# dohlee/diffab-pytorch

Hardware: AMD Instinct MI355X
Metric: CDR-residue denoise-steps/sec (K=128 patch) (higher is better)
Workload: dtype f32 (bf16x6 / fp16x3 split-precision products on the 16-bit matrix cores, fp32 accumulate; fp32-accurate, DESIGN section 4)

## Files before the change

### diffab-pytorch_amd/csrc/api.hip

```cpp
#include <atomic>
#include <cstring>
#include <mutex>
#include <vector>

#include "common.h"
#include "denoiser_internal.h"
#include "mlp_chain_tile.h"

namespace diffab {

static thread_local char g_err[512] = "";

void set_error(const char* fmt, ...) {
  va_list ap;
  va_start(ap, fmt);
  vsnprintf(g_err, sizeof(g_err), fmt, ap);
  va_end(ap);
}

namespace {
struct OrderState {
  std::recursive_mutex mu;
  hipStream_t last = nullptr;
  bool have = false;
// ... 21 lines not shown
}
StreamOrder::~StreamOrder() {
  if (dev_ < 0) return;
  OrderState& o = g_order[dev_ & 31];
  --o.depth;
  o.mu.unlock();
}
void set_stream_order(bool on) { g_order_on.store(on); }

struct KernelTimer {
  bool on = false;
  std::vector<hipEvent_t> ev;
  size_t used = 0;
};
static KernelTimer g_timer;

void timer_begin(hipStream_t st) {
  if (!g_timer.on) return;
  if (g_timer.used + 2 > g_timer.ev.size()) {
    for (int i = 0; i < 2; ++i) {
      hipEvent_t e;
      if (hipEventCreate(&e) != hipSuccess) return;
      g_timer.ev.push_back(e);
    }
  }
  (void)hipEventRecord(g_timer.ev[g_timer.used], st);
}
bool kernel_timer_enabled() { return g_timer.on; }
void timer_end(hipStream_t st) {
  if (!g_timer.on || g_timer.used + 2 > g_timer.ev.size()) return;
  (void)hipEventRecord(g_timer.ev[g_timer.used + 1], st);
  g_timer.used += 2;
}

static int check_dims(const diffab_dims* d, const char* who) {
  DIFFAB_REQUIRE(d != nullptr, DIFFAB_ERR_ARG, "%s: dims is null", who);
  DIFFAB_REQUIRE(d->B > 0 && d->K > 0 && d->D > 0 && d->C >= 0 && d->H > 0 && d->DS > 0 && d->PQ > 0 && d->PV > 0 && d->NL >= 0 && d->V > 0,
                 DIFFAB_ERR_ARG, "%s: non-positive dimension (B=%d K=%d D=%d C=%d H=%d DS=%d PQ=%d PV=%d NL=%d V=%d)", who, d->B, d->K, d->D,
                 d->C, d->H, d->DS, d->PQ, d->PV, d->NL, d->V);
  DIFFAB_REQUIRE(static_cast<int64_t>(d->B) * d->K < (1ll << 31), DIFFAB_ERR_UNSUPPORTED, "%s: B*K must be < 2^31", who);
  return DIFFAB_OK;
}

struct StepBuffers {
  float *cat2, *h1, *hA, *hB, *cat3, *t1, *t2, *vbuf, *logits, *ipa, *emb_tab, *beta_tab;
  char* planes;
  float* pair;
  size_t bytes;
};
static size_t mlp_planes_bytes() { return (rowgemm128_b6_scratch_bytes(128) + 255) & ~static_cast<size_t>(255); }

static StepBuffers carve_step(const diffab_dims* d, void* ws, int n_pair = 0) {
  Carver c(ws);
  const size_t rows = static_cast<size_t>(d->B) * d->K;
  StepBuffers b;
  b.cat2 = c.take<float>(rows * 2 * d->D);
  b.h1 = c.take<float>(rows * d->D);
  b.hA = c.take<float>(rows * d->D);
  b.hB = c.take<float>(rows * d->D);
  b.cat3 = c.take<float>(rows * (d->D + 3));
  b.t1 = c.take<float>(rows * d->D);
  b.t2 = c.take<float>(rows * d->D);
  b.vbuf = c.take<float>(rows * 3);
  b.logits = c.take<float>(rows * d->V);
  b.emb_tab = c.take<float>(static_cast<size_t>(25) * d->D);
  b.beta_tab = c.take<float>(static_cast<size_t>(3) * d->B * d->D);
  size_t ipa_floats = ipa_generic_workspace_floats(d);
  if (fast_path_supported(d)) ipa_floats = ipa_floats > ipa_fast_workspace_floats(d) ? ipa_floats : ipa_fast_workspace_floats(d);
  b.ipa = c.take<float>(ipa_floats);
  b.planes = fast_path_supported(d) ? c.take<char>(d->NL * ipa_layer_planes_bytes() + 11 * mlp_planes_bytes()) : nullptr;
  b.pair = pair_planes_supported(d) ? c.take<float>(pair_planes_floats(d, n_pair)) : nullptr;
  b.bytes = c.bytes();
  return b;
}

static bool ipa_layer_weights_ok(const diffab_dims* d, const diffab_ipa_layer_weights* w) {
  return w && w->gamma && w->wq_s && w->wk_s && w->wv_s && (w->w_bias || d->C == 0) && w->wq_p && w->wk_p && w->wv_p && w->w_out && w->b_out;
}

static int ipa_layer_dispatch(const diffab_dims* d, const diffab_ipa_layer_weights* w, const float* x, const float* e, const float* R,
                              const float* t, float* y, float* ws, uint32_t flags, hipStream_t st, float* sp_keep = nullptr,
                              float* d2_keep = nullptr, const void* planes = nullptr, const float* pair_planes = nullptr,
                              bool taped = false,
                              const unsigned char* tile_needed = nullptr, const int* ctx_of_row = nullptr, int n_ctx = 0) {
  DIFFAB_REQUIRE(ipa_layer_weights_ok(d, w), DIFFAB_ERR_ARG, "ipa layer: null weight pointer");
  if (!(flags & DIFFAB_FLAG_FORCE_GENERIC) && fast_path_supported(d))
    return ipa_layer_fast(d, w, x, e, R, t, y, ws, st, sp_keep, d2_keep, planes, pair_planes, (flags & DIFFAB_FLAG_FP32_GEMM) != 0,
                          taped, tile_needed, ctx_of_row, n_ctx);
  return ipa_layer_generic(d, w, x, e, R, t, y, ws, st, ctx_of_row);
}

static int check_denoiser_weights(const diffab_dims* d, const diffab_denoiser_weights* w) {
  DIFFAB_REQUIRE(w && w->seq_emb && w->res_w0 && w->res_b0 && w->res_w2 && w->res_b2 && (d->NL == 0 || w->layers), DIFFAB_ERR_ARG,
                 "denoiser: null weight pointer");
  DIFFAB_REQUIRE(d->C > 0, DIFFAB_ERR_ARG, "denoiser: C must be positive (the Denoiser's IPA layers use the pair bias, :478-492)");
  for (const diffab_mlp3_weights* h : {&w->coord, &w->orient, &w->seq})
    DIFFAB_REQUIRE(h->w0 && h->b0 && h->w2 && h->b2 && h->w4 && h->b4, DIFFAB_ERR_ARG, "denoiser head: null weight pointer");
  for (int l = 0; l < d->NL; ++l)
    DIFFAB_REQUIRE(ipa_layer_weights_ok(d, &w->layers[l]), DIFFAB_ERR_ARG, "denoiser: null weight pointer in IPA layer %d", l);
  return DIFFAB_OK;
}

static bool use_pair_planes(const diffab_dims* d, uint32_t flags, const float* pair_ctx, const StepBuffers& b) {
  const uint32_t other = DIFFAB_FLAG_FORCE_GENERIC | DIFFAB_FLAG_PAIR_F32;
  return (flags & DIFFAB_FLAG_PAIR_PLANES) && !(flags & other) && b.pair != nullptr && pair_planes_supported(d) &&
         (reinterpret_cast<uintptr_t>(pair_ctx) & 15) == 0;
}

static bool module_launch_fills_chip(const diffab_dims* d) {
  if (!ipa_module_persistent_supported(d)) return false;
  int dev = 0, ncu = 256;
  if (hipGetDevice(&dev) == hipSuccess) (void)hipDeviceGetAttribute(&ncu, hipDeviceAttributeMultiprocessorCount, dev);
  const int rounds = (d->B + ncu - 1) / ncu;
  return d->K == 128 && d->B >= ncu && static_cast<double>(d->B) >= 0.85 * rounds * ncu;
}

struct ForwardPlan {
  uint32_t flags;
  bool fold;
  bool b6;
  bool chain;
  bool persistent, fused_mlps;
  const float* pair_planes;
  const int* ctx_of_row;
  int n_ctx;
  const unsigned char* last_layer_tiles;
  float* res_emb;
};

static ForwardPlan plan_forward(const diffab_dims* d, uint32_t flags, const StepBuffers& b, const float* res_ctx, const float* pair_ctx,
                                float* res_emb, bool loop, const int* ctx_of_row = nullptr, int n_ctx = 0, unsigned char* tiles = nullptr) {
  const int rows = d->B * d->K, D = d->D;
  if (loop && !(flags & DIFFAB_FLAG_PAIR_F32)) flags |= DIFFAB_FLAG_PAIR_PLANES;
  ForwardPlan p{};
  p.flags = flags;
  p.fold = !(flags & DIFFAB_FLAG_FORCE_GENERIC) && fast_path_supported(d) && rowgemm128_ok(res_ctx, D, b.h1, D, rows, D);
  p.b6 = p.fold && use_b6_gemm(flags) && rowgemm128_b6_ok(res_ctx, D, b.h1, D, rows, D);
  p.chain = p.b6 && d->V <= 128;
  p.pair_planes = use_pair_planes(d, flags, pair_ctx, b) ? b.pair : nullptr;
  p.ctx_of_row = ctx_of_row;
  p.n_ctx = n_ctx;
  p.last_layer_tiles = tiles != nullptr && !(flags & DIFFAB_FLAG_ALL_ROWS) && p.fold && d->K % 16 == 0 && d->NL >= 2 ? tiles : nullptr;
  p.res_emb = res_emb;
  p.persistent = p.b6 && p.pair_planes != nullptr && ipa_module_persistent_supported(d) &&
                 ((flags & DIFFAB_FLAG_PERSISTENT_MODULE) || (loop && !(flags & DIFFAB_FLAG_MULTI_LAUNCH) && module_launch_fills_chip(d)));
  p.fused_mlps = p.persistent && p.chain && D == 128 && res_emb == nullptr;
  return p;
}

struct StepBias {
  const float* beta;
  const float* sched_beta;
  int t;
  const int* t_dev;
  float* beta_traj;
  int traj_rows;
};

static int prepare_forward(const diffab_dims* d, const diffab_denoiser_weights* w, const ForwardPlan& p, const StepBuffers& b,
                           const float* pair_ctx, const StepBias& bias, hipStream_t st) {
  if (p.fold)
    if (int rc = launch_fold_embed_table(d, w, b.emb_tab, st)) return rc;
  if (p.b6) {
    const int D = d->D;
    for (int l = 0; l < d->NL; ++l)
      if (int rc = ipa_layer_split_weights(&w->layers[l], b.planes + l * ipa_layer_planes_bytes(), st)) return rc;
    char* mlp = b.planes + d->NL * ipa_layer_planes_bytes();
    const diffab_mlp3_weights* hw[3] = {&w->coord, &w->orient, &w->seq};
    if (int rc = launch_wsplit128(w->res_w0, 2 * D, D, mlp, st)) return rc;
    if (int rc = launch_wsplit128(w->res_w2, D, D, mlp + mlp_planes_bytes(), st)) return rc;
    for (int hd = 0; hd < 3; ++hd) {
      if (int rc = launch_wsplit128(hw[hd]->w0, D + 3, D, mlp + (2 + 2 * hd) * mlp_planes_bytes(), st)) return rc;
      if (int rc = launch_wsplit128(hw[hd]->w2, D, D, mlp + (3 + 2 * hd) * mlp_planes_bytes(), st)) return rc;
      const int nout = hd == 2 ? d->V : 3;
      if (int rc = launch_wsplit128(hw[hd]->w4, D, D, mlp + (8 + hd) * mlp_planes_bytes(), st, nout)) return rc;
    }
  }
  if (p.pair_planes)
    if (int rc = launch_pair_split(d, pair_ctx, b.pair, st, p.n_ctx)) return rc;
  if (bias.beta_traj) {
    diffab_dims dt = *d;
    dt.B = bias.traj_rows;
    if (int rc = launch_fold_beta_table(&dt, w, bias.sched_beta, bias.beta_traj, st)) return rc;
  }
  return DIFFAB_OK;
}

static int denoise_step(const diffab_dims* d, const diffab_denoiser_weights* w, const ForwardPlan& p, const StepBias& bias,
                        const int64_t* seq_t, const float* x_t, const float* O_t, const float* res_ctx, const float* pair_ctx, float* out_eps,
                        float* out_O0, float* out_post, float* out_logits, const StepBuffers& b, hipStream_t st) {
  const int rows = d->B * d->K, D = d->D;
  if (p.fold && bias.beta_traj == nullptr)
    if (int rc = launch_fold_beta_table(d, w, bias.beta, b.beta_tab, st, bias.sched_beta, bias.t, bias.t_dev)) return rc;
  const char* mlp = p.b6 ? b.planes + d->NL * ipa_layer_planes_bytes() : nullptr;
  auto dense128 = [&](int slot, const float* X, const float* W, int ldw, const float* bvec, const int64_t* bias_idx, int bias_div, float* Y,
                      bool relu) -> int {
    if (p.b6) return launch_rowgemm128_b6p(X, D, mlp + slot * mlp_planes_bytes(), bvec, bias_idx, bias_div, Y, D, rows, D, relu, st);
    return launch_rowgemm128(X, D, W, ldw, bvec, bias_idx, bias_div, Y, D, rows, D, relu, st);
  };
  float* logits = out_logits ? out_logits : b.logits;
  MlpChainSet emb_set{}, head_set{};
  if (p.chain) {
    const void* pl[3] = {mlp, mlp + mlp_planes_bytes(), nullptr};
    const float* bs[3] = {b.emb_tab, w->res_b2, nullptr};
    float* ys[1] = {b.hA};
    const int nout1[1] = {D};
    if (int rc = make_mlp_chain_set(&emb_set, 1, pl, bs, seq_t, 0, 2, nout1, ys, nout1)) return rc;
    if (!p.fused_mlps)
      if (int rc = launch_mlp_chain_b6(res_ctx, D, pl, bs, seq_t, 0, 2, D, b.hA, D, rows, st)) return rc;
  } else if (p.fold) {
    if (int rc = dense128(0, res_ctx, w->res_w0, 2 * D, b.emb_tab, seq_t, 0, b.h1, true)) return rc;
    if (int rc = dense128(1, b.h1, w->res_w2, D, w->res_b2, nullptr, 0, b.hA, false)) return rc;
  } else {
    if (int rc = launch_embed_concat(res_ctx, w->seq_emb, seq_t, D, rows, b.cat2, st)) return rc;
    if (int rc = launch_linear(b.cat2, 2 * D, w->res_w0, w->res_b0, b.h1, D, rows, D, 2 * D, true, st)) return rc;
    if (int rc = launch_linear(b.h1, D, w->res_w2, w->res_b2, b.hA, D, rows, D, D, false, st)) return rc;
  }
  float *cur = b.hA, *nxt = b.hB;
  const diffab_mlp3_weights* hw[3] = {&w->coord, &w->orient, &w->seq};
  float* outs[3] = {out_eps, b.vbuf, logits};
  const int nout[3] = {3, 3, d->V};
  const void* hpl[9];
  const float* hbs[9];
  const int head_div = bias.beta_traj ? rows : d->K;
  if (p.chain) {
    for (int hd = 0; hd < 3; ++hd) {
      hpl[3 * hd] = mlp + (2 + 2 * hd) * mlp_planes_bytes();
      hpl[3 * hd + 1] = mlp + (3 + 2 * hd) * mlp_planes_bytes();
      hpl[3 * hd + 2] = mlp + (8 + hd) * mlp_planes_bytes();
      hbs[3 * hd] = bias.beta_traj ? bias.beta_traj + (static_cast<size_t>(hd) * bias.traj_rows + bias.t) * D
                                   : b.beta_tab + static_cast<size_t>(hd) * d->B * D;
      hbs[3 * hd + 1] = hw[hd]->b2;
      hbs[3 * hd + 2] = hw[hd]->b4;
    }
    if (int rc = make_mlp_chain_set(&head_set, 3, hpl, hbs, nullptr, head_div, 3, nout, outs, nout)) return rc;
  }
  if (p.persistent) {
    if (int rc = launch_ipa_module_persistent(d, b.hA, b.hB, O_t, x_t, b.ipa, b.planes, p.pair_planes, st, p.fused_mlps ? res_ctx : nullptr,
                                              &emb_set, &head_set, p.ctx_of_row, p.n_ctx, p.last_layer_tiles))
      return rc;
    cur = (d->NL & 1) ? b.hB : b.hA;
  }
  for (int l = 0; l < d->NL && !p.persistent; ++l) {
    const void* planes = p.b6 ? b.planes + l * ipa_layer_planes_bytes() : nullptr;
    if (int rc = ipa_layer_dispatch(d, &w->layers[l], cur, pair_ctx, O_t, x_t, nxt, b.ipa, p.flags, st, nullptr, nullptr, planes, p.pair_planes,
                                    false, l == d->NL - 1 ? p.last_layer_tiles : nullptr, p.ctx_of_row, p.n_ctx))
      return rc;
    float* tmp = cur; cur = nxt; nxt = tmp;
  }
  if (p.res_emb) DIFFAB_HIP_CHECK(hipMemcpyAsync(p.res_emb, cur, sizeof(float) * rows * D, hipMemcpyDeviceToDevice, st));
  if (p.chain) {
    if (!p.fused_mlps)
      if (int rc = launch_mlp_chains_b6(cur, D, 3, hpl, hbs, nullptr, head_div, 3, nout, outs, nout, rows, st)) return rc;
  } else if (p.fold) {
    for (int hd = 0; hd < 3; ++hd) {
      if (int rc = dense128(2 + 2 * hd, cur, hw[hd]->w0, D + 3, b.beta_tab + static_cast<size_t>(hd) * d->B * D, nullptr, d->K, b.t1, true))
        return rc;
      if (int rc = dense128(3 + 2 * hd, b.t1, hw[hd]->w2, D, hw[hd]->b2, nullptr, 0, b.t2, true)) return rc;
      if (int rc = launch_linear(b.t2, D, hw[hd]->w4, hw[hd]->b4, outs[hd], nout[hd], rows, nout[hd], D, false, st)) return rc;
    }
  } else {
    if (int rc = launch_beta_concat(cur, bias.beta, D, d->K, rows, b.cat3, st)) return rc;
    for (int hd = 0; hd < 3; ++hd) {
      if (int rc = launch_linear(b.cat3, D + 3, hw[hd]->w0, hw[hd]->b0, b.t1, D, rows, D, D + 3, true, st)) return rc;
      if (int rc = launch_linear(b.t1, D, hw[hd]->w2, hw[hd]->b2, b.t2, D, rows, D, D, true, st)) return rc;
      if (int rc = launch_linear(b.t2, D, hw[hd]->w4, hw[hd]->b4, outs[hd], nout[hd], rows, nout[hd], D, false, st)) return rc;
    }
  }
  if (out_O0 == nullptr) return DIFFAB_OK;
  return launch_heads_finish(b.vbuf, O_t, logits, d->V, rows, out_O0, out_post, st);
}

static uint32_t taped_flags(uint32_t flags) { return flags & ~(DIFFAB_FLAG_FORCE_GENERIC | DIFFAB_FLAG_PAIR_PLANES); }

static int denoise_step_taped(const diffab_dims* d, const diffab_denoiser_weights* w, const int64_t* seq_t, const float* x_t,
                              const float* O_t, const float* res_ctx, const float* pair_ctx, const float* beta, float* out_eps,
                              float* out_O0, float* out_post, const TrainTape& tp, uint32_t flags, hipStream_t st) {
  const int rows = d->B * d->K, D = d->D;
  if (int rc = launch_embed_concat(res_ctx, w->seq_emb, seq_t, D, rows, tp.cat2, st)) return rc;
  if (int rc = launch_linear(tp.cat2, 2 * D, w->res_w0, w->res_b0, tp.h1, D, rows, D, 2 * D, true, st)) return rc;
  if (int rc = launch_linear(tp.h1, D, w->res_w2, w->res_b2, tp.x[0], D, rows, D, D, false, st)) return rc;
  const bool b6 = tp.planes && use_b6_gemm(flags) && fast_path_supported(d);
  for (int l = 0; l < d->NL; ++l) {
    if (b6)
      if (int rc = ipa_layer_split_weights(&w->layers[l], tp.planes, st)) return rc;
    if (int rc = ipa_layer_dispatch(d, &w->layers[l], tp.x[l], pair_ctx, O_t, x_t, tp.x[l + 1], tp.ipa_ws[l], flags, st, tp.sp[l], tp.d2[l],
                                    b6 ? tp.planes : nullptr, nullptr, true))
      return rc;
  }
  if (int rc = launch_beta_concat(tp.x[d->NL], beta, D, d->K, rows, tp.cat3, st)) return rc;
  const diffab_mlp3_weights* hw[3] = {&w->coord, &w->orient, &w->seq};
  float* outs[3] = {out_eps, tp.vbuf, tp.logits};
  const int nout[3] = {3, 3, d->V};
  for (int hd = 0; hd < 3; ++hd) {
    if (int rc = launch_linear(tp.cat3, D + 3, hw[hd]->w0, hw[hd]->b0, tp.t1[hd], D, rows, D, D + 3, true, st)) return rc;
    if (int rc = launch_linear(tp.t1[hd], D, hw[hd]->w2, hw[hd]->b2, tp.t2[hd], D, rows, D, D, true, st)) return rc;
    if (int rc = launch_linear(tp.t2[hd], D, hw[hd]->w4, hw[hd]->b4, outs[hd], nout[hd], rows, nout[hd], D, false, st)) return rc;
  }
  return launch_heads_finish(tp.vbuf, O_t, tp.logits, d->V, rows, out_O0, out_post, st);
}

constexpr int kTrajRows = 1025;
struct SampleBuffers {
  float *beta, *eps, *O0, *post;
  int* t_dev;
  unsigned char* tiles;
  float* beta_traj;
  int* ctx_of_row;
  float* res_ctx;
  void* step;
  size_t bytes;
};

static SampleBuffers carve_sample(const diffab_dims* d, void* ws, int n_pair = 0, bool mapped = false) {
  Carver c(ws);
  const size_t rows = static_cast<size_t>(d->B) * d->K;
  SampleBuffers s;
  s.beta = c.take<float>(d->B);
  s.eps = c.take<float>(rows * 3);
  s.O0 = c.take<float>(rows * 9);
  s.post = c.take<float>(rows * d->V);
  s.t_dev = c.take<int>(64);
  s.tiles = c.take<unsigned char>(static_cast<size_t>(d->B) * ((d->K + 15) / 16));
  s.beta_traj = c.take<float>(static_cast<size_t>(3) * kTrajRows * d->D);
  s.ctx_of_row = mapped ? c.take<int>(d->B) : nullptr;
  s.res_ctx = mapped ? c.take<float>(rows * d->D) : nullptr;
  const size_t step_bytes = carve_step(d, nullptr, n_pair).bytes;
  s.step = c.take<char>(step_bytes);
  s.bytes = c.bytes();
  return s;
}

struct ScoreBuffers {
  int* t_list;
  float* beta;
  int* ctx_of_row;
  int64_t* seq_t;
  float *x_t, *O_t, *eps, *eps_hat;
  float* res_ctx;
  void* step;
  size_t bytes;
};
static ScoreBuffers carve_score(const diffab_dims* d, void* ws, int n_ctx) {
  Carver c(ws);
  const size_t rows = static_cast<size_t>(d->B) * d->K;
  ScoreBuffers s;
  s.t_list = c.take<int>(kTrajRows);
  s.beta = c.take<float>(d->B);
  s.ctx_of_row = c.take<int>(d->B);
  s.seq_t = c.take<int64_t>(rows);
  s.x_t = c.take<float>(rows * 3);
  s.O_t = c.take<float>(rows * 9);
  s.eps = c.take<float>(rows * 3);
  s.eps_hat = c.take<float>(rows * 3);
  s.res_ctx = c.take<float>(rows * d->D);
  s.step = c.take<char>(carve_step(d, nullptr, n_ctx).bytes);
  s.bytes = c.bytes();
  return s;
}

}

using namespace diffab;

extern "C" {

const char* diffab_version(void) { return "diffab_hip 0.1.0 (gfx950)"; }
const char* diffab_last_error(void) { return g_err; }

int diffab_device_ok(void) {
  int n = 0;
  if (hipGetDeviceCount(&n) != hipSuccess || n <= 0) return 0;
  hipDeviceProp_t p;
  int dev = 0;
  if (hipGetDevice(&dev) != hipSuccess || hipGetDeviceProperties(&p, dev) != hipSuccess) return 0;
  return std::strncmp(p.gcnArchName, "gfx950", 6) == 0 ? 1 : 0;
}

int diffab_debug_linear128(const float* X, const float* W, const float* bias, float* Y, int64_t M, int32_t Kd, int32_t mode, void* scratch,
                           size_t scratch_bytes, void* stream) {
  StreamOrder order_(stream);
  DIFFAB_REQUIRE(X && W && Y && M >= 1 && M < (1LL << 31) && Kd >= 32 && Kd % 32 == 0, DIFFAB_ERR_ARG, "debug_linear128: bad operands");
  hipStream_t st = as_stream(stream);
  if (mode == 0) return launch_linear(X, Kd, W, bias, Y, 128, static_cast<int>(M), 128, Kd, false, st);
  if (mode == 2) {
    const size_t pb = (rowgemm128_h3_planes_bytes(Kd) + 255) & ~static_cast<size_t>(255);
    DIFFAB_REQUIRE(Kd % 64 == 0, DIFFAB_ERR_ARG, "debug_linear128: mode 2 (fp16 x 3) needs Kd %% 64 == 0 (its chunks of 32 k are joined in pairs)");
    DIFFAB_REQUIRE(scratch && scratch_bytes >= pb + 512 && rowgemm128_b6_ok(X, Kd, Y, 128, static_cast<int>(M), Kd) &&
                       (reinterpret_cast<uintptr_t>(scratch) & 15) == 0,
                   DIFFAB_ERR_ARG, "debug_linear128: mode 2 needs 16-byte aligned operands and %zu bytes of scratch", pb + 512);
    float* wis = reinterpret_cast<float*>(static_cast<char*>(scratch) + pb);
    if (int rc = launch_wsplit128_h3(W, Kd, Kd, scratch, wis, st)) return rc;
    return launch_rowgemm128_h3p(X, Kd, scratch, wis, bias, nullptr, 0, Y, 128, static_cast<int>(M), Kd, false, st, nullptr);
  }
  DIFFAB_REQUIRE(mode == 1 && scratch && scratch_bytes >= rowgemm128_b6_scratch_bytes(Kd) && rowgemm128_b6_ok(X, Kd, Y, 128, static_cast<int>(M), Kd),
                 DIFFAB_ERR_ARG, "debug_linear128: mode 1 needs 16-byte aligned operands and %zu bytes of scratch", rowgemm128_b6_scratch_bytes(Kd));
  return launch_rowgemm128_b6(X, Kd, W, Kd, bias, nullptr, 0, Y, 128, static_cast<int>(M), Kd, false, scratch, st);
}

int diffab_debug_xstat128(const float* X, const float* W, float* Y, int64_t M, int32_t N, int32_t mode, void* scratch, size_t scratch_bytes,
                          void* stream) {
  StreamOrder order_(stream);
  DIFFAB_REQUIRE(X && W && Y && scratch && M >= 1 && M < (1LL << 31) && N >= 1 && (mode == 1 || mode == 2), DIFFAB_ERR_ARG,
                 "debug_xstat128: bad operands");
  const size_t need = mode == 1 ? xstat_b6_scratch_bytes(N) : xstat_h3_scratch_bytes(N);
  DIFFAB_REQUIRE(scratch_bytes >= need && (reinterpret_cast<uintptr_t>(scratch) & 15) == 0 && (reinterpret_cast<uintptr_t>(X) & 15) == 0,
                 DIFFAB_ERR_ARG, "debug_xstat128: needs 16-byte aligned X / scratch and %zu bytes of scratch", need);
  hipStream_t st = as_stream(stream);
  if (mode == 1) return launch_xstat_b6(X, W, 1, N, Y, N, static_cast<int>(M), N, scratch, st);
  return launch_xstat_h3(X, W, 1, N, Y, N, static_cast<int>(M), N, scratch, st);
}

int diffab_debug_gemm_tn(const float* A, const float* B, float* C, float* db, int64_t M, int32_t N1, int32_t N2, int32_t mode, void* stream) {
  StreamOrder order_(stream);
  DIFFAB_REQUIRE(A && B && C && M >= 1 && M < (1LL << 31) && N1 >= 1 && N2 >= 1 && (mode == 1 || mode == 2), DIFFAB_ERR_ARG,
                 "debug_gemm_tn: bad operands");
  hipStream_t st = as_stream(stream);
  if (mode == 1) return launch_gemm_tn_b6(A, N1, B, N2, C, N2, static_cast<int>(M), N1, N2, db, nullptr, nullptr, 0, st);
  return launch_gemm_tn_h3(A, N1, B, N2, C, N2, static_cast<int>(M), N1, N2, db, nullptr, nullptr, 0, st);
}

int diffab_set_stream_guard(int on) {
  set_stream_order(on != 0);
  return DIFFAB_OK;
}

int diffab_debug_set_module_stagger(int32_t ticks_10ns, int32_t classes) {
  set_module_stagger(ticks_10ns, classes);
  return DIFFAB_OK;
}

int diffab_debug_set_module_stamps(void* device_buffer) {
  set_module_stamps(device_buffer);
  return DIFFAB_OK;
}

int diffab_debug_row_tiles(const uint8_t* gen_mask, int32_t B, int32_t K, uint8_t* tiles, void* stream) {
  StreamOrder order_(stream);
  DIFFAB_REQUIRE(gen_mask && tiles && B >= 1 && K >= 16 && K % 16 == 0, DIFFAB_ERR_ARG, "debug_row_tiles: need B >= 1 and K a multiple of 16");
  return launch_tiles_needed(gen_mask, B, K, tiles, as_stream(stream));
}

int diffab_debug_set_attn_variant(int32_t v) { return set_attn_variant(v); }

int diffab_debug_set_attn_stamps(void* device_buffer) {
  set_attn_stamps(device_buffer);
  return DIFFAB_OK;
}

int diffab_kernel_timer_enable(int on) {
  g_timer.on = on != 0;
  g_timer.used = 0;
  return DIFFAB_OK;
}

int diffab_kernel_timer_read(int64_t* launches, double* total_ms) {
  DIFFAB_REQUIRE(launches && total_ms, DIFFAB_ERR_ARG, "kernel_timer_read: null pointer");
  double tot = 0.0;
  for (size_t i = 0; i + 1 < g_timer.used; i += 2) {
    DIFFAB_HIP_CHECK(hipEventSynchronize(g_timer.ev[i + 1]));
    float ms = 0.f;
    DIFFAB_HIP_CHECK(hipEventElapsedTime(&ms, g_timer.ev[i], g_timer.ev[i + 1]));
    tot += ms;
  }
  *launches = static_cast<int64_t>(g_timer.used / 2);
  *total_ms = tot;
  g_timer.used = 0;
  return DIFFAB_OK;
}

size_t diffab_denoise_workspace_bytes(const diffab_dims* d) {
  if (check_dims(d, "denoise_workspace_bytes")) return 0;
  return carve_step(d, nullptr).bytes;
}

size_t diffab_sample_workspace_bytes(const diffab_dims* d) {
  if (check_dims(d, "sample_workspace_bytes")) return 0;
  return carve_sample(d, nullptr).bytes;
}

size_t diffab_sample_shared_workspace_bytes(const diffab_dims* d, int32_t n_ctx) {
  if (check_dims(d, "sample_shared_workspace_bytes")) return 0;
  if (n_ctx < 1 || static_cast<int64_t>(n_ctx) * d->K >= (1ll << 31)) {
    set_error("sample_shared_workspace_bytes: need 1 <= n_ctx and n_ctx*K < 2^31 (n_ctx=%d)", n_ctx);
    return 0;
  }
  return carve_sample(d, nullptr, n_ctx, true).bytes;
}

int diffab_ipa_layer_fwd(const diffab_dims* d, const diffab_ipa_layer_weights* w, const float* x, const float* e, const float* R,
                         const float* t, float* y, void* workspace, size_t workspace_bytes, uint32_t flags, void* stream) {
  StreamOrder order_(stream);
  if (int rc = check_dims(d, "ipa_layer_fwd")) return rc;
  DIFFAB_REQUIRE(x && (e || d->C == 0) && R && t && y && workspace, DIFFAB_ERR_ARG, "ipa_layer_fwd: null pointer");
  const StepBuffers b = carve_step(d, workspace);
  DIFFAB_REQUIRE(workspace_bytes >= b.bytes, DIFFAB_ERR_WORKSPACE, "ipa_layer_fwd: workspace %zu < %zu bytes", workspace_bytes, b.bytes);
  const float* pair_planes = nullptr;
  if (use_pair_planes(d, flags, e, b)) {
    if (int rc = launch_pair_split(d, e, b.pair, as_stream(stream))) return rc;
    pair_planes = b.pair;
  }
  return ipa_layer_dispatch(d, w, x, e, R, t, y, b.ipa, flags, as_stream(stream), nullptr, nullptr, nullptr, pair_planes);
}

int diffab_denoise_step_fwd(const diffab_dims* d, const diffab_denoiser_weights* w, const int64_t* seq_t, const float* x_t, const float* O_t,
                            const float* res_ctx, const float* pair_ctx, const float* beta, float* out_eps, float* out_O0,
                            float* out_posterior, float* out_logits, float* out_res_emb, void* workspace, size_t workspace_bytes,
                            uint32_t flags, void* stream) {
  StreamOrder order_(stream);
  if (int rc = check_dims(d, "denoise_step_fwd")) return rc;
  if (int rc = check_denoiser_weights(d, w)) return rc;
  DIFFAB_REQUIRE(seq_t && x_t && O_t && res_ctx && pair_ctx && beta && out_eps && out_O0 && out_posterior && workspace, DIFFAB_ERR_ARG,
                 "denoise_step_fwd: null pointer");
  const StepBuffers b = carve_step(d, workspace);
  DIFFAB_REQUIRE(workspace_bytes >= b.bytes, DIFFAB_ERR_WORKSPACE, "denoise_step_fwd: workspace %zu < %zu bytes", workspace_bytes, b.bytes);
  hipStream_t st = as_stream(stream);
  const ForwardPlan p = plan_forward(d, flags, b, res_ctx, pair_ctx, out_res_emb, false);
  const StepBias bias{beta};
  if (int rc = prepare_forward(d, w, p, b, pair_ctx, bias, st)) return rc;
  return denoise_step(d, w, p, bias, seq_t, x_t, O_t, res_ctx, pair_ctx, out_eps, out_O0, out_posterior, out_logits, b, st);
}

static int check_attn_bwd_lds(const diffab_dims* d, const char* who) {
  DIFFAB_REQUIRE(attn_bwd_lds_ok(d), DIFFAB_ERR_UNSUPPORTED,
                 "%s: H*K = %d too large for the attention backward's LDS (%zu > %zu bytes; the forward alone reaches further)", who,
                 d->H * d->K, attn_bwd_lds_bytes(d), kAttnBwdLdsMax);
// ... 248 lines not shown
  std::vector<int32_t> plan_host;
  if (steps != nullptr) {
    const int T = s->T;
    DIFFAB_REQUIRE(steps->n_steps >= 1, DIFFAB_ERR_ARG, "sample_loop: steps n_steps = %d < 1", steps->n_steps);
    DIFFAB_REQUIRE(steps->steps && steps->beta_jump && steps->alpha_jump && steps->plan_dev, DIFFAB_ERR_ARG,
                   "sample_loop: steps needs steps, beta_jump, alpha_jump and plan_dev");
    DIFFAB_REQUIRE(s->alpha_bar, DIFFAB_ERR_ARG, "sample_loop: steps need the schedule's alpha_bar");
    DIFFAB_REQUIRE(steps->steps[0] == t_start, DIFFAB_ERR_ARG, "sample_loop: steps[0] = %d, t_start = %d", steps->steps[0], t_start);
    std::vector<char> listed(T + 1, 0);
    for (int j = 0; j < steps->n_steps; ++j) {
      const int t = steps->steps[j];
      DIFFAB_REQUIRE(t > t_stop && t <= T, DIFFAB_ERR_ARG, "sample_loop: steps[%d] = %d outside [t_stop + 1, T] = [%d, %d]", j, t, t_stop + 1, T);
      DIFFAB_REQUIRE(j == 0 || t < steps->steps[j - 1], DIFFAB_ERR_ARG, "sample_loop: steps are not strictly descending at %d (%d after %d)", j,
                     t, steps->steps[j - 1]);
      const float bj = steps->beta_jump[t], aj = steps->alpha_jump[t];
      DIFFAB_REQUIRE(bj > 0.0f && bj < 1.0f && aj > 0.0f && aj < 1.0f, DIFFAB_ERR_ARG,
                     "sample_loop: jump coefficients at step %d outside (0, 1): beta' = %g, alpha' = %g", t, bj, aj);
      listed[t] = 1;
    }
    if (rec != nullptr)
      for (int t = 0; t <= T; ++t)
        DIFFAB_REQUIRE(rec->slot_of_step[t] == -1 || listed[t], DIFFAB_ERR_ARG,
                       "sample_loop: record slot_of_step[%d] = %d, but the step list does not run step %d", t, rec->slot_of_step[t], t);
    plan_host.resize(3 * static_cast<size_t>(T + 1));
    for (int t = 0; t <= T; ++t) plan_host[t] = t > 0 ? t - 1 : 0;
    for (int j = 0; j < steps->n_steps; ++j) plan_host[steps->steps[j]] = j + 1 < steps->n_steps ? steps->steps[j + 1] : t_stop;
    std::memcpy(plan_host.data() + (T + 1), steps->beta_jump, sizeof(float) * (T + 1));
    std::memcpy(plan_host.data() + 2 * (T + 1), steps->alpha_jump, sizeof(float) * (T + 1));
    const int32_t* pd = static_cast<const int32_t*>(steps->plan_dev);
    pdev = StepPlanDev{pd, reinterpret_cast<const float*>(pd + (T + 1)), reinterpret_cast<const float*>(pd + 2 * (T + 1)), s->alpha_bar};
  }
  GuidanceDev gdev;
  if (guidance != nullptr) {
    if (int rc = check_guidance_terms(guidance, "sample_loop")) return rc;
    DIFFAB_REQUIRE(guidance->max_shift > 0.0f, DIFFAB_ERR_ARG, "sample_loop: guidance max_shift = %g must be > 0 (INFINITY: no cap)",
                   guidance->max_shift);
    DIFFAB_REQUIRE(guidance->t_max >= 0 && guidance->t_max <= s->T, DIFFAB_ERR_ARG, "sample_loop: guidance t_max = %d outside [0, T = %d]",
                   guidance->t_max, s->T);
    DIFFAB_REQUIRE(guidance->shift_dev != nullptr, DIFFAB_ERR_ARG, "sample_loop: guidance needs shift_dev");
    DIFFAB_REQUIRE(!(keep & DIFFAB_FLAG_KEEP_STRUCTURE), DIFFAB_ERR_ARG,
                   "sample_loop: guidance moves the structure, which DIFFAB_FLAG_KEEP_STRUCTURE does not sample");
    DIFFAB_REQUIRE(s->alpha_bar_sqrt, DIFFAB_ERR_ARG, "sample_loop: guidance needs the schedule's alpha_bar_sqrt");
    gdev.shift = guidance->shift_dev;
    gdev.chain = guidance->chain;
    gdev.residue_idx = guidance->residue_idx;
    gdev.residue_mask = guidance->residue_mask;
    gdev.w_clash = guidance->w_clash;
    gdev.clash_distance = guidance->clash_distance;
    gdev.w_bond = guidance->w_bond;
    gdev.bond_length = guidance->bond_length;
    gdev.max_shift = guidance->max_shift;
    gdev.t_max = guidance->t_max;
  }
  TemperatureDev tdev;
  if (temperature != nullptr) {
    DIFFAB_REQUIRE(!temperature->rot_scale || temperature->rot_row, DIFFAB_ERR_ARG,
                   "sample_loop: temperature rot_scale needs rot_row (its rows of the stacked reverse table)");
    DIFFAB_REQUIRE(!((temperature->trans_scale || temperature->rot_scale) && (keep & DIFFAB_FLAG_KEEP_STRUCTURE)), DIFFAB_ERR_ARG,
                   "sample_loop: noise scales act on the structure, which DIFFAB_FLAG_KEEP_STRUCTURE does not sample");
    DIFFAB_REQUIRE(!(temperature->seq_temp && (keep & DIFFAB_FLAG_KEEP_SEQUENCE)), DIFFAB_ERR_ARG,
                   "sample_loop: a sequence temperature acts on the sequence, which DIFFAB_FLAG_KEEP_SEQUENCE does not sample");
    tdev = TemperatureDev{temperature->trans_scale, temperature->rot_scale, temperature->seq_temp, temperature->rot_row};
  }
  const bool mapped = ctx_of_row != nullptr;
  DIFFAB_REQUIRE(mapped || n_ctx == d->B, DIFFAB_ERR_ARG, "sample_loop: without ctx_of_row n_ctx must equal B (%d != %d)", n_ctx, d->B);
  DIFFAB_REQUIRE(n_ctx >= 1 && static_cast<int64_t>(n_ctx) * d->K < (1ll << 31), DIFFAB_ERR_ARG, "sample_loop: need 1 <= n_ctx, n_ctx*K < 2^31");
  bool identity = n_ctx == d->B;
  for (int b = 0; mapped && b < d->B; ++b) {
    DIFFAB_REQUIRE(ctx_of_row[b] >= 0 && ctx_of_row[b] < n_ctx, DIFFAB_ERR_ARG, "sample_loop: ctx_of_row[%d] = %d outside [0, %d)", b,
                   ctx_of_row[b], n_ctx);
    identity = identity && ctx_of_row[b] == b;
  }
  const SampleBuffers sb = carve_sample(d, workspace, n_ctx, mapped);
  DIFFAB_REQUIRE(workspace_bytes >= sb.bytes, DIFFAB_ERR_WORKSPACE, "sample_loop: workspace %zu < %zu bytes", workspace_bytes, sb.bytes);
  hipStream_t st = as_stream(stream);
  const int* ctx_dev = nullptr;
  if (!identity) {
    DIFFAB_HIP_CHECK(hipMemcpyAsync(sb.ctx_of_row, ctx_of_row, sizeof(int32_t) * d->B, hipMemcpyHostToDevice, st));
    if (int rc = launch_gather_rows(res_ctx, sb.ctx_of_row, d->B, static_cast<int64_t>(d->K) * d->D, sb.res_ctx, st)) return rc;
    ctx_dev = sb.ctx_of_row;
    res_ctx = sb.res_ctx;
  }
  const StepBuffers b0 = carve_step(d, sb.step, n_ctx);
  const ForwardPlan plan = plan_forward(d, flags, b0, res_ctx, pair_ctx, nullptr, true, ctx_dev, n_ctx, sb.tiles);
  StepBias bias{sb.beta, plan.fold ? s->beta : nullptr, 0, nullptr, nullptr, s->T + 1};
  if (plan.chain && s->T + 1 <= kTrajRows && !(flags & DIFFAB_FLAG_GRAPH_SAMPLER)) bias.beta_traj = sb.beta_traj;
  if (int rc = prepare_forward(d, w, plan, b0, pair_ctx, bias, st)) return rc;
  if (plan.last_layer_tiles)
    if (int rc = launch_tiles_needed(gen_mask, d->B, d->K, sb.tiles, st)) return rc;
  if (rec != nullptr) {
    DIFFAB_HIP_CHECK(hipMemcpyAsync(rec->slot_dev, rec->slot_of_step, sizeof(int32_t) * (s->T + 1), hipMemcpyHostToDevice, st));
    if (int rc = launch_record_fixed(rdev, seq, x, O, gen_mask, d->B, d->K, d->V, st)) return rc;
  }
  if (steps != nullptr)
    DIFFAB_HIP_CHECK(hipMemcpyAsync(steps->plan_dev, plan_host.data(), sizeof(int32_t) * plan_host.size(), hipMemcpyHostToDevice, st));
  auto one_step = [&](int t, const int* t_dev) -> int {
    if (!plan.fold)
      if (int rc = launch_fill_beta(s, t, d->B, sb.beta, st, t_dev)) return rc;
    StepBias step = bias;
    step.t = t;
    step.t_dev = t_dev;
    if (int rc = denoise_step(d, w, plan, step, seq, x, O, res_ctx, pair_ctx, sb.eps, nullptr, nullptr, nullptr, b0, st)) return rc;
    return launch_reverse_update_philox(s, rev_tab, t, seq, x, O, sb.eps, sb.O0, sb.post, gen_mask, seed, first_patch, d->B, d->K, d->V, st,
                                        t_dev, b0.vbuf, b0.logits, keep, allowed, rdev, pdev, gdev, tdev);
  };
  const int n_steps = steps != nullptr ? steps->n_steps : t_start - t_stop;
  const bool graph = (flags & DIFFAB_FLAG_GRAPH_SAMPLER) && n_steps >= 3 && !kernel_timer_enabled();
  if (!graph) {
    if (steps != nullptr) {
      for (int j = 0; j < n_steps; ++j)
        if (int rc = one_step(steps->steps[j], nullptr)) return rc;
      return DIFFAB_OK;
    }
    for (int t = t_start; t > t_stop; --t)
      if (int rc = one_step(t, nullptr)) return rc;
    return DIFFAB_OK;
  }
  const int t_second = steps != nullptr ? steps->steps[1] : t_start - 1;
  if (int rc = one_step(t_start, nullptr)) return rc;
  if (int rc = launch_set_int(sb.t_dev, t_second, st)) return rc;
  hipStream_t side = nullptr;
  hipEvent_t ev = nullptr;
  hipGraph_t g = nullptr;
  hipGraphExec_t ge = nullptr;
  DIFFAB_HIP_CHECK(hipStreamCreateWithFlags(&side, hipStreamNonBlocking));
  hipError_t ei = hipEventCreateWithFlags(&ev, hipEventDisableTiming);
  if (ei == hipSuccess) ei = hipEventRecord(ev, st);
  if (ei == hipSuccess) ei = hipStreamWaitEvent(side, ev, 0);
  int rc = DIFFAB_OK;
  if (ei == hipSuccess) {
    hipStream_t caller = st;
    st = side;
    ei = hipStreamBeginCapture(side, hipStreamCaptureModeThreadLocal);
    if (ei == hipSuccess) {
      rc = one_step(t_second, sb.t_dev);
      if (rc == DIFFAB_OK) rc = steps != nullptr ? launch_advance_step(sb.t_dev, pdev.next, side) : launch_dec_int(sb.t_dev, side);
      ei = hipStreamEndCapture(side, &g);
    }
    st = caller;
  }
  if (ei == hipSuccess && rc == DIFFAB_OK) ei = hipGraphInstantiate(&ge, g, nullptr, nullptr, 0);
  if (ei == hipSuccess && rc == DIFFAB_OK)
    for (int j = 1; j < n_steps && ei == hipSuccess; ++j) ei = hipGraphLaunch(ge, side);
  if (ei == hipSuccess) ei = hipStreamSynchronize(side);
  if (ge) (void)hipGraphExecDestroy(ge);
  if (g) (void)hipGraphDestroy(g);
  if (ev) (void)hipEventDestroy(ev);
  (void)hipStreamDestroy(side);
  if (rc != DIFFAB_OK) return rc;
  if (ei != hipSuccess) {
    set_error("sample_loop: graph capture / replay failed: %s", hipGetErrorString(ei));
    return DIFFAB_ERR_HIP;
  }
  return DIFFAB_OK;
}

size_t diffab_score_workspace_bytes(const diffab_dims* d, int32_t n_ctx) {
  if (check_dims(d, "score_workspace_bytes")) return 0;
  if (n_ctx < 1 || static_cast<int64_t>(n_ctx) * d->K >= (1ll << 31)) {
    set_error("score_workspace_bytes: need 1 <= n_ctx and n_ctx*K < 2^31 (n_ctx=%d)", n_ctx);
    return 0;
  }
  return carve_score(d, nullptr, n_ctx).bytes;
}

int diffab_score_designs(const diffab_dims* d, const diffab_denoiser_weights* w, const diffab_sched* s, const diffab_igso3* fwd_tab,
                         const int64_t* seq, const float* x, const float* O, const uint8_t* gen_mask, const uint8_t* res_mask,
// ... 61 lines not shown
```

### diffab-pytorch_amd/csrc/denoiser_fast.hip

```cpp
#include <cstdlib>
#include <type_traits>

#include "common.h"
#include "denoiser_internal.h"
#include "rowgemm_b6_tile.h"
#include "ipa_attn_tile.h"

namespace diffab {


constexpr int LBM = 128, LBK = 32, LLD = LBK + 4;

struct LinearSegs {
  const float* W[6];
  int n_end[6];
  int nseg;
};

template <int BN, bool RELU, bool VEC>
__global__ __launch_bounds__(256) void linear_mfma_kernel(const float* __restrict__ X, int ldx, LinearSegs segs,
                                                          const float* __restrict__ bias, float* __restrict__ Y, int ldy, int M, int N,
                                                          int Kd) {
  __shared__ __attribute__((aligned(16))) float As[LBM * LLD];
  __shared__ __attribute__((aligned(16))) float Bs[BN * LLD];
// ... 189 lines not shown
#pragma unroll
      for (int s = 0; s < 4; ++s)
#pragma unroll
        for (int mt = 0; mt < MT; ++mt)
#pragma unroll
          for (int tt = 0; tt < 4; ++tt)
            acc[mt][tt] = __builtin_amdgcn_mfma_f32_16x16x4f32(a[mt][4 * part + kq][s], b[kq & 1][tt][s], acc[mt][tt], 0, 0, 0);
    }
  };

  load_w(0);
  load_a(aA, 0);
  store_w(0);
  __syncthreads();
  for (int ch = 0; ch < nchunk; ch += 2 * AW) {
    load_a(aB, ch / AW + 1);
#pragma unroll
    for (int p = 0; p < AW; ++p) {
      load_w(ch + p + 1);
      MEM_FENCE();
      compute(aA, p, p & 1);
      store_w((p + 1) & 1);
      __syncthreads();
    }
    load_a(aA, ch / AW + 2);
#pragma unroll
    for (int p = 0; p < AW; ++p) {
      load_w(ch + AW + p + 1);
      MEM_FENCE();
      compute(aB, p, (AW + p) & 1);
      store_w((AW + p + 1) & 1);
      __syncthreads();
    }
  }
  const int col = 64 * cw + 4 * l15;
  const bool table = bias_idx != nullptr || bias_div > 0;
  f32x4 bv = {0.f, 0.f, 0.f, 0.f};
  if (bias && !table) bv = *reinterpret_cast<const f32x4*>(bias + col);
#pragma unroll
  for (int mt = 0; mt < MT; ++mt)
#pragma unroll
    for (int r = 0; r < 4; ++r) {
      const int row = m0 + 16 * MT * rw + 16 * mt + 4 * g + r;
      if (row >= M) continue;
      if (table) {
        const int64_t bi = bias_idx ? bias_idx[row] : row / bias_div;
        bv = *reinterpret_cast<const f32x4*>(bias + bi * 128 + col);
      }
      f32x4 o = {acc[mt][0][r] + bv[0], acc[mt][1][r] + bv[1], acc[mt][2][r] + bv[2], acc[mt][3][r] + bv[3]};
      if (RELU) { o[0] = fmaxf(o[0], 0.f); o[1] = fmaxf(o[1], 0.f); o[2] = fmaxf(o[2], 0.f); o[3] = fmaxf(o[3], 0.f); }
      *reinterpret_cast<f32x4*>(Y + static_cast<int64_t>(row) * ldy + col) = o;
    }
}

bool rowgemm128_ok(const float* X, int ldx, const float* Y, int ldy, int M, int Kd) {
  return Kd % (2 * RG_KC) == 0 && ldx % 4 == 0 && ldy % 4 == 0 && aligned16(X) && aligned16(Y) && M >= RG_ROWS;
}
int launch_rowgemm128(const float* X, int ldx, const float* W, int ldw, const float* bias, const int64_t* bias_idx, int bias_div, float* Y,
                      int ldy, int M, int Kd, bool relu, hipStream_t st) {
  DIFFAB_REQUIRE(rowgemm128_ok(X, ldx, Y, ldy, M, Kd) && (!bias || aligned16(bias)), DIFFAB_ERR_ARG, "rowgemm128: unsupported operands");
  const dim3 grid((M + RG_ROWS - 1) / RG_ROWS);
#define RG_LAUNCH(R, AW_) \
  hipLaunchKernelGGL((rowgemm128_kernel<R, AW_>), grid, dim3(512), 0, st, X, ldx, W, ldw, bias, bias_idx, bias_div, Y, ldy, M, Kd)
  if (RG_DEEP_A && Kd % (4 * RG_KC) == 0) { if (relu) RG_LAUNCH(true, 2); else RG_LAUNCH(false, 2); }
  else                                    { if (relu) RG_LAUNCH(true, 1); else RG_LAUNCH(false, 1); }
#undef RG_LAUNCH
  DIFFAB_LAUNCH_CHECK();
  return DIFFAB_OK;
}

int launch_linear(const float* X, int ldx, const float* W, const float* bias, float* Y, int ldy, int M, int N, int Kd, bool relu,
                  hipStream_t st) {
  LinearSegs segs{};
  segs.W[0] = W;
  segs.n_end[0] = N;
  segs.nseg = 1;
  const bool vec = (ldx % 4 == 0) && (Kd % 4 == 0) && aligned16(X) && aligned16(W);
  if (N == 128 && vec && rowgemm128_ok(X, ldx, Y, ldy, M, Kd) && (!bias || aligned16(bias)))
    return launch_rowgemm128(X, ldx, W, Kd, bias, nullptr, 0, Y, ldy, M, Kd, relu, st);
  if (N > 64) return launch_linear_bn<128>(X, ldx, segs, bias, Y, ldy, M, N, Kd, relu, vec, st);
  return launch_linear_bn<64>(X, ldx, segs, bias, Y, ldy, M, N, Kd, relu, vec, st);
}

template <int NT, bool MULTI, bool PLANES = false, bool TAPE = false>
__global__ __launch_bounds__(512) void ipa_attn_fast_kernel(const float* __restrict__ proj, const float* __restrict__ e,
                                                            const float* __restrict__ R, const float* __restrict__ t,
                                                            const float* __restrict__ Wb, const float* __restrict__ gamma,
                                                            float* __restrict__ feat, int B, int NC_arg,
                                                            unsigned long long* __restrict__ stamps, const float* __restrict__ esc = nullptr,
                                                            float* __restrict__ tape_p = nullptr, float* __restrict__ tape_d2 = nullptr,
                                                            const unsigned char* __restrict__ tile_needed = nullptr,
                                                            const int* __restrict__ ctx_of_row = nullptr) {
  extern __shared__ __attribute__((aligned(16))) float S[];
  const int ntile = (MULTI ? NC_arg : 1) * NT;
  int b, tile;
  const unsigned bid = blockIdx.x;
  if ((B & 7) == 0) {
    const int xcd = bid & 7, slot = bid >> 3;
    b = (slot / ntile) * 8 + xcd;
    tile = slot % ntile;
  } else {
    b = bid / ntile;
    tile = bid % ntile;
  }
  if (tile_needed != nullptr && !tile_needed[b * ntile + tile]) return;
  ipa_attn_tile<NT, MULTI, PLANES, TAPE>(S, b, tile, bid, proj, e, R, t, Wb, gamma, feat, NC_arg, stamps, esc, tape_p, tape_d2, ctx_of_row);
}

static unsigned long long* g_attn_stamps = nullptr;
static bool g_pair_chain_off = false;
void set_pair_embed_fused(bool on);
int set_attn_variant(int v) {
  DIFFAB_REQUIRE((v & ~(4 | 64)) == 0, DIFFAB_ERR_ARG, "debug_set_attn_variant: %d has bits other than 4 and 64", v);
  set_pair_embed_fused(!(v & 4));
  g_pair_chain_off = (v & 64) != 0;
  return DIFFAB_OK;
}
bool pair_chain_bwd_enabled() { return !g_pair_chain_off; }
void set_attn_stamps(void* p) {
  g_attn_stamps = static_cast<unsigned long long*>(p);
}

__global__ void points_to_global_fast_kernel(float* __restrict__ proj, const float* __restrict__ R, const float* __restrict__ t, int rows) {
  const int gid = blockIdx.x * blockDim.x + threadIdx.x;
  if (gid >= rows * 192) return;
  const int r = gid / 192, p = gid % 192;
  float* qv = proj + static_cast<int64_t>(r) * ANP + OFF_GQ + p * 3;
  const float* Rr = R + static_cast<int64_t>(r) * 9;
  const float x = qv[0], y = qv[1], z = qv[2];
  qv[0] = (x * Rr[0] + y * Rr[3] + z * Rr[6]) + t[r * 3 + 0];
  qv[1] = (x * Rr[1] + y * Rr[4] + z * Rr[7]) + t[r * 3 + 1];
  qv[2] = (x * Rr[2] + y * Rr[5] + z * Rr[8]) + t[r * 3 + 2];
}

__global__ __launch_bounds__(64) void fold_embed_table_kernel(const float* __restrict__ emb, const float* __restrict__ W0,
                                                              const float* __restrict__ b0, int D, int n_types, float* __restrict__ tab) {
  const int s_ = blockIdx.x, n0 = blockIdx.y * 8, lane = threadIdx.x;
  if (s_ >= n_types) return;
  float acc[8];
#pragma unroll
  for (int i = 0; i < 8; ++i) {
    acc[i] = 0.f;
    const int n = n0 + i;
    if (n < D)
      for (int k = lane; k < D; k += 64) acc[i] += emb[s_ * D + k] * W0[n * 2 * D + D + k];
  }
#pragma unroll
  for (int i = 0; i < 8; ++i) {
    for (int o = 32; o > 0; o >>= 1) acc[i] += __shfl_xor(acc[i], o);
    if (lane == 0 && n0 + i < D) tab[s_ * D + n0 + i] = acc[i] + b0[n0 + i];
  }
}
__global__ void fold_beta_table_kernel(const float* __restrict__ beta, const float* __restrict__ Wa, const float* __restrict__ ba,
                                       const float* __restrict__ Wb_, const float* __restrict__ bb, const float* __restrict__ Wc,
                                       const float* __restrict__ bc, int D, int B, float* __restrict__ tab,
                                       const float* __restrict__ sched_beta, int t, const int* __restrict__ t_dev) {
  const int b = blockIdx.x, hd = blockIdx.y, n = threadIdx.x;
  if (b >= B || n >= D) return;
  const float* W = hd == 0 ? Wa : (hd == 1 ? Wb_ : Wc);
  const float* bias = hd == 0 ? ba : (hd == 1 ? bb : bc);
  const float be = sched_beta ? sched_beta[t_dev ? *t_dev : t] : beta[b];
  const float* wr = W + n * (D + 3) + D;
  tab[(static_cast<int64_t>(hd) * B + b) * D + n] = ((be * wr[0] + sinf(be) * wr[1]) + cosf(be) * wr[2]) + bias[n];
}
int launch_fold_embed_table(const diffab_dims* d, const diffab_denoiser_weights* w, float* emb_tab, hipStream_t st) {
  hipLaunchKernelGGL(fold_embed_table_kernel, dim3(25, (d->D + 7) / 8), dim3(64), 0, st, w->seq_emb, w->res_w0, w->res_b0, d->D, 25, emb_tab);
  DIFFAB_LAUNCH_CHECK();
  return DIFFAB_OK;
}
int launch_fold_beta_table(const diffab_dims* d, const diffab_denoiser_weights* w, const float* beta, float* beta_tab, hipStream_t st,
                           const float* sched_beta, int t, const int* t_dev) {
  hipLaunchKernelGGL(fold_beta_table_kernel, dim3(d->B, 3), dim3(d->D), 0, st, beta, w->coord.w0, w->coord.b0, w->orient.w0, w->orient.b0,
                     w->seq.w0, w->seq.b0, d->D, d->B, beta_tab, sched_beta, t, t_dev);
  DIFFAB_LAUNCH_CHECK();
  return DIFFAB_OK;
}

bool fast_path_supported(const diffab_dims* d) {
  return d->D == 128 && d->C == AC && d->H == AH && d->DS == ADS && d->PQ == AP && d->PV == AP && d->K % 64 == 0 && d->K >= 64 &&
         d->K <= 1024;
}

__global__ __launch_bounds__(256) void pair_rowscale_kernel(const float* __restrict__ e, int row_f4, float* __restrict__ rs) {
  const int64_t row = blockIdx.x;
  const f32x4* p = reinterpret_cast<const f32x4*>(e) + row * row_f4;
  float m = 0.f;
  for (int i = threadIdx.x; i < row_f4; i += 256) {
    const f32x4 v = p[i];
    m = fmaxf(fmaxf(m, fmaxf(fabsf(v[0]), fabsf(v[1]))), fmaxf(fabsf(v[2]), fabsf(v[3])));
  }
#pragma unroll
  for (int o = 1; o < 64; o <<= 1) m = fmaxf(m, __shfl_xor(m, o));
  __shared__ float wm[4];
  if ((threadIdx.x & 63) == 0) wm[threadIdx.x >> 6] = m;
  __syncthreads();
  if (threadIdx.x == 0) {
    const unsigned b = __float_as_uint(fmaxf(fmaxf(wm[0], wm[1]), fmaxf(wm[2], wm[3])));
    const int ex = static_cast<int>((b >> 23) & 255u);
    const bool ok = ex >= 8 && ex < 231 && b < 0x7f800000u;
    rs[2 * row] = ok ? __uint_as_float(static_cast<unsigned>(127 + 7 + 127 - ex) << 23) : 1.0f;
    rs[2 * row + 1] = ok ? __uint_as_float(static_cast<unsigned>(ex - 7) << 23) : 1.0f;
  }
}
__global__ void pair_split_kernel(const float* __restrict__ e, const float* __restrict__ rs, int K, int64_t n_groups,
                                  _Float16* __restrict__ out) {
  const int64_t gid = blockIdx.x * static_cast<int64_t>(blockDim.x) + threadIdx.x;
  if (gid >= n_groups) return;
  const int cg = static_cast<int>(gid & 7);
  const int64_t rj = gid >> 3;
  const int j = static_cast<int>(rj % K);
  const int64_t row = rj / K;
  const float s = rs[2 * row];
  const f32x4 v0 = reinterpret_cast<const f32x4*>(e)[gid * 2], v1 = reinterpret_cast<const f32x4*>(e)[gid * 2 + 1];
  f16x8 h1, h2;
#pragma unroll
  for (int c = 0; c < 8; ++c) {
    const float x = (c < 4 ? v0[c & 3] : v1[c & 3]) * s;
    const _Float16 a = static_cast<_Float16>(x);
    h1[c] = a;
    h2[c] = static_cast<_Float16>(x - static_cast<float>(a));
  }
  const int jt = j >> 4, l15 = j & 15, ks = cg >> 2, g = cg & 3;
  _Float16* base = out + (row * K) * 128 + static_cast<int64_t>(jt) * 2048 + ks * 512 + (l15 + 16 * g) * 8;
  *reinterpret_cast<f16x8*>(base) = h1;
  *reinterpret_cast<f16x8*>(base + 1024) = h2;
}
bool pair_planes_supported(const diffab_dims* d) { return fast_path_supported(d); }
static size_t pair_patches(const diffab_dims* d, int n_pair) { return static_cast<size_t>(n_pair > 0 ? n_pair : d->B); }
size_t pair_planes_floats(const diffab_dims* d, int n_pair) {
  const size_t np = pair_patches(d, n_pair);
  return pair_planes_supported(d) ? np * d->K * d->K * AC + 64 + 2 * np * d->K + 64 : 0;
}
const float* pair_row_scales(const diffab_dims* d, const float* planes, int n_pair) {
  return planes + 64 + pair_patches(d, n_pair) * d->K * d->K * AC;
}
int launch_pair_split(const diffab_dims* d, const float* e, float* planes, hipStream_t st, int n_pair) {
  DIFFAB_REQUIRE(pair_planes_supported(d) && e && planes && (reinterpret_cast<uintptr_t>(planes) & 15) == 0 &&
                     (reinterpret_cast<uintptr_t>(e) & 15) == 0,
                 DIFFAB_ERR_ARG, "pair_split: unsupported operands");
  const int64_t np = static_cast<int64_t>(pair_patches(d, n_pair));
  const int64_t n = np * d->K * d->K * AC;
  float* rs = const_cast<float*>(pair_row_scales(d, planes, n_pair));
  hipLaunchKernelGGL(pair_rowscale_kernel, dim3(static_cast<unsigned>(np * d->K)), dim3(256), 0, st, e, d->K * AC / 4, rs);
  hipLaunchKernelGGL(pair_split_kernel, dim3(static_cast<unsigned>((n / 8 + 255) / 256)), dim3(256), 0, st, e, rs, d->K, n / 8,
                     reinterpret_cast<_Float16*>(planes + 64));
  DIFFAB_LAUNCH_CHECK();
  return DIFFAB_OK;
}


bool use_b6_gemm(uint32_t flags) { return !(flags & DIFFAB_FLAG_FP32_GEMM); }
static size_t round256(size_t b) { return (b + 255) & ~static_cast<size_t>(255); }
constexpr size_t kLayerSmallFloats = AH * AC + 64 + 128;
size_t ipa_layer_small_offset() { return 0; }
size_t ipa_layer_h3_pj_offset() { return ipa_layer_small_offset() + round256(kLayerSmallFloats * sizeof(float)); }
size_t ipa_layer_h3_out_offset() { return ipa_layer_h3_pj_offset() + round256(proj_frames_h3_planes_bytes()); }
size_t ipa_layer_h3_wis_offset() { return ipa_layer_h3_out_offset() + round256(rowgemm128_h3_planes_bytes(AF)); }
size_t ipa_layer_planes_bytes() { return ipa_layer_h3_wis_offset() + round256((ANP + 128) * sizeof(float)); }
__global__ void layer_small_copy_kernel(const float* __restrict__ w_bias, const float* __restrict__ gamma, const float* __restrict__ b_out,
                                        float* __restrict__ out) {
  const int i = blockIdx.x * blockDim.x + threadIdx.x;
  if (i < AH * AC) out[i] = w_bias[i];
  else if (i < AH * AC + 64) out[i] = i - AH * AC < AH ? gamma[i - AH * AC] : 0.0f;
  else if (i < static_cast<int>(kLayerSmallFloats)) out[i] = b_out[i - AH * AC - 64];
}
int ipa_layer_split_weights(const diffab_ipa_layer_weights* w, void* planes, hipStream_t st) {
  DIFFAB_REQUIRE(w && w->wq_s && w->wk_s && w->wv_s && w->wq_p && w->wk_p && w->wv_p && w->w_out, DIFFAB_ERR_ARG, "ipa layer: null weight pointer");
  const float* W6[6] = {w->wq_s, w->wk_s, w->wv_s, w->wq_p, w->wk_p, w->wv_p};
  if (w->w_bias && w->gamma && w->b_out) {
    hipLaunchKernelGGL(layer_small_copy_kernel, dim3((kLayerSmallFloats + 255) / 256), dim3(256), 0, st, w->w_bias, w->gamma, w->b_out,
                       reinterpret_cast<float*>(static_cast<char*>(planes) + ipa_layer_small_offset()));
    DIFFAB_LAUNCH_CHECK();
  }
  char* pl = static_cast<char*>(planes);
  float* wis = reinterpret_cast<float*>(pl + ipa_layer_h3_wis_offset());
  if (int rc = launch_pjsplit_h3(W6, pl + ipa_layer_h3_pj_offset(), wis, st)) return rc;
  return launch_wsplit128_h3(w->w_out, AF, AF, pl + ipa_layer_h3_out_offset(), wis + ANP, st);
}
static size_t b6_scratch_floats() { return (ipa_layer_planes_bytes() + 256) / sizeof(float); }

static size_t ipa_ws_parts_offset(const diffab_dims* d) {
  const size_t rows = static_cast<size_t>(d->B) * d->K;
  const size_t o = rows * (ANP + AF) + 128 + (attention_split_supported(d) ? attention_split_workspace_floats(d) : 0) + b6_scratch_floats();
  return (o + 63) & ~static_cast<size_t>(63);
}
size_t ipa_fast_workspace_floats(const diffab_dims* d) { return ipa_ws_parts_offset(d) + rowgemm128_h3_parts_floats(d->B * d->K, AF) + 64; }

int ipa_layer_fast(const diffab_dims* d, const diffab_ipa_layer_weights* w, const float* x, const float* e, const float* R, const float* t,
                   float* y, float* ws, hipStream_t st, float* sp_keep, float* d2_keep, const void* planes, const float* pair_planes,
                   bool fp32_gemm, bool taped, const unsigned char* tile_needed, const int* ctx_of_row, int n_ctx) {
  const int rows = d->B * d->K, D = d->D;
  DIFFAB_REQUIRE(ctx_of_row == nullptr || sp_keep == nullptr, DIFFAB_ERR_ARG, "ipa_layer_fast: shared contexts are an inference form");
  float* proj = ws;
  float* feat = ws + static_cast<size_t>(rows) * ANP;
  const bool h3 = use_b6_gemm(fp32_gemm ? DIFFAB_FLAG_FP32_GEMM : 0u) && (planes != nullptr || sp_keep == nullptr);
  if (h3 && planes == nullptr) {
    float* tail = ws + static_cast<size_t>(rows) * (ANP + AF) + 128 + (attention_split_supported(d) ? attention_split_workspace_floats(d) : 0);
    void* own = reinterpret_cast<void*>((reinterpret_cast<uintptr_t>(tail) + 255) & ~static_cast<uintptr_t>(255));
    if (int rc = ipa_layer_split_weights(w, own, st)) return rc;
    planes = own;
  }
  const char* plc = static_cast<const char*>(planes);
  const float* wis = h3 ? reinterpret_cast<const float*>(plc + ipa_layer_h3_wis_offset()) : nullptr;
  auto to_out = [&]() -> int {
    if (h3 && rowgemm128_b6_ok(feat, AF, y, D, rows, AF))
      return launch_rowgemm128_h3p(feat, AF, plc + ipa_layer_h3_out_offset(), wis + ANP, w->b_out, nullptr, 0, y, D, rows, AF, false, st,
                                   taped ? nullptr : ws + ipa_ws_parts_offset(d));
    return launch_linear(feat, AF, w->w_out, w->b_out, y, D, rows, D, AF, false, st);
  };
  LinearSegs segs{};
  segs.W[0] = w->wq_s; segs.W[1] = w->wk_s; segs.W[2] = w->wv_s; segs.W[3] = w->wq_p; segs.W[4] = w->wk_p; segs.W[5] = w->wv_p;
  segs.n_end[0] = 256; segs.n_end[1] = 512; segs.n_end[2] = 768; segs.n_end[3] = 960; segs.n_end[4] = 1152; segs.n_end[5] = 1344;
  segs.nseg = 6;
  bool vec = aligned16(x);
  for (int s = 0; s < 6; ++s) vec = vec && aligned16(segs.W[s]);
  DIFFAB_REQUIRE(vec, DIFFAB_ERR_ARG, "ipa_layer_fast: x and the projection weights must be 16-byte aligned");
  if (h3) {
    if (int rc = launch_proj_frames_h3p(x, plc + ipa_layer_h3_pj_offset(), wis, R, t, proj, rows, st)) return rc;
  } else {
    if (int rc = launch_proj_frames_f32(x, segs.W, R, t, proj, rows, st)) return rc;
  }
  if (sp_keep != nullptr && attention_split_supported(d) && !(d->K == 128 && d2_keep != nullptr)) {
    if (int rc = launch_attention_split(d, proj, e, R, t, w->w_bias, w->gamma, feat, sp_keep, st, d2_keep)) return rc;
    return to_out();
  }
  const bool tape = sp_keep != nullptr && attention_split_supported(d);
  const int nt = (d->K % 128 == 0) ? 8 : 4;
  const int nc = d->K / (16 * nt);
  const size_t lds = ipa_attn_lds_bytes(nt);
  const dim3 grid(d->B * (d->K / TI));
  const bool use_planes = pair_planes != nullptr && pair_planes_supported(d);
  const float* e_arg = use_planes ? pair_planes + 64 : e;
  const float* esc = use_planes ? pair_row_scales(d, pair_planes, n_ctx) : nullptr;
#define ATTN_LAUNCH(NT_, MULTI_, PLANES_)                                                                                             \
  do {                                                                                                                                \
    DIFFAB_HIP_CHECK(hipFuncSetAttribute(reinterpret_cast<const void*>(ipa_attn_fast_kernel<NT_, MULTI_, PLANES_>),                   \
                                         hipFuncAttributeMaxDynamicSharedMemorySize, static_cast<int>(lds)));                         \
    timer_begin(st);                                                                                                                  \
    hipLaunchKernelGGL((ipa_attn_fast_kernel<NT_, MULTI_, PLANES_>), grid, dim3(512), lds, st, proj, e_arg, R, t, w->w_bias, w->gamma, \
                       feat, d->B, nc, g_attn_stamps, esc, nullptr, nullptr, tile_needed, ctx_of_row);                                \
    timer_end(st);                                                                                                                    \
  } while (0)
  if (tape) {
    DIFFAB_HIP_CHECK(hipFuncSetAttribute(reinterpret_cast<const void*>(ipa_attn_fast_kernel<8, false, false, true>),
                                         hipFuncAttributeMaxDynamicSharedMemorySize, static_cast<int>(lds)));
    hipLaunchKernelGGL((ipa_attn_fast_kernel<8, false, false, true>), grid, dim3(512), lds, st, proj, e, R, t, w->w_bias, w->gamma, feat,
                       d->B, nc, nullptr, nullptr, sp_keep, d2_keep);
  } else if (use_planes) {
    if (nt == 8 && nc == 1) ATTN_LAUNCH(8, false, true);
    else if (nt == 8) ATTN_LAUNCH(8, true, true);
    else if (nc == 1) ATTN_LAUNCH(4, false, true);
    else ATTN_LAUNCH(4, true, true);
  } else if (nt == 8 && nc == 1) ATTN_LAUNCH(8, false, false);
  else if (nt == 8) ATTN_LAUNCH(8, true, false);
  else if (nc == 1) ATTN_LAUNCH(4, false, false);
  else ATTN_LAUNCH(4, true, false);
#undef ATTN_LAUNCH
  DIFFAB_LAUNCH_CHECK();
  return to_out();
}

}
```

### diffab-pytorch_amd/csrc/denoiser_internal.h

```cpp
#pragma once
#include "common.h"

namespace diffab {

int launch_linear_generic(const float* X, int ldx, const float* W, const float* bias, float* Y, int ldy, int M, int N, int Kd, bool relu,
                          hipStream_t st);
size_t ipa_generic_workspace_floats(const diffab_dims* d);
int ipa_layer_generic(const diffab_dims* d, const diffab_ipa_layer_weights* w, const float* x, const float* e, const float* R, const float* t,
                      float* y, float* ws, hipStream_t st, const int* ctx_of_row = nullptr);
int launch_embed_concat(const float* res_ctx, const float* emb, const int64_t* seq, int D, int64_t rows, float* out, hipStream_t st);
int launch_beta_concat(const float* h, const float* beta, int D, int K, int64_t rows, float* out, hipStream_t st);
int launch_heads_finish(const float* v, const float* O_t, const float* logits, int V, int64_t rows, float* O0, float* post, hipStream_t st);
int launch_proj_frames_f32(const float* x, const float* const* W6, const float* R, const float* t, float* proj, int rows, hipStream_t st);
int launch_losses_bwd(const float* post, const float* tpost, const float* eps, const float* teps, const float* O0, const float* tO,
                      const float* O_t, const float* v, const uint8_t* gm, const uint8_t* rm, const float* count, const float* up, int V,
                      int64_t rows, float* d_logits, float* d_eps, float* d_v, hipStream_t st);
int launch_heads_cotangent(const float* post, const float* c_post, const float* c_eps, const float* c_O0, const float* O_t, const float* v,
                           int V, int64_t rows, float* d_logits, float* d_eps, float* d_v, float* d_Ot, hipStream_t st);
int launch_ipa_frames_bwd(const float* proj, const float* dproj, int NP, int pt_col0, int n_pts, const float* feat, const float* dfeat, int F,
                          int ol_col0, int on_col0, int n_vpts, const float* R, const float* t, float* dR, float* dt, int rows,
                          hipStream_t st);

bool fast_path_supported(const diffab_dims* d);
size_t ipa_fast_workspace_floats(const diffab_dims* d);
int ipa_layer_fast(const diffab_dims* d, const diffab_ipa_layer_weights* w, const float* x, const float* e, const float* R, const float* t,
                   float* y, float* ws, hipStream_t st,
                   float* sp_keep = nullptr, float* d2_keep = nullptr,
                   const void* planes = nullptr,
                   const float* pair_planes = nullptr,
                   bool fp32_gemm = false,
                   bool taped = false,
                   const unsigned char* tile_needed = nullptr,
                   const int* ctx_of_row = nullptr, int n_ctx = 0);
bool pair_planes_supported(const diffab_dims* d);
size_t pair_planes_floats(const diffab_dims* d, int n_pair = 0);
int launch_pair_split(const diffab_dims* d, const float* e, float* planes, hipStream_t st, int n_pair = 0);
const float* pair_row_scales(const diffab_dims* d, const float* planes, int n_pair = 0);
int launch_linear(const float* X, int ldx, const float* W, const float* bias, float* Y, int ldy, int M, int N, int Kd, bool relu,
                  hipStream_t st);

bool rowgemm128_ok(const float* X, int ldx, const float* Y, int ldy, int M, int Kd);
int launch_rowgemm128(const float* X, int ldx, const float* W, int ldw, const float* bias, const int64_t* bias_idx, int bias_div, float* Y,
                      int ldy, int M, int Kd, bool relu, hipStream_t st);
size_t rowgemm128_b6_scratch_bytes(int Kd);
bool rowgemm128_b6_ok(const float* X, int ldx, const float* Y, int ldy, int M, int Kd);
int launch_wsplit128(const float* W, int ldw, int Kd, void* planes, hipStream_t st, int nrows = 128);
int launch_mlp_chains_b6(const float* X, int ldx, int nchains, const void* const* planes, const float* const* bias, const int64_t* bias_idx0,
                         int bias_div0, int nlayers, const int* n_out, float* const* Y, const int* ldy, int M, hipStream_t st);
struct MlpChainSet;
int make_mlp_chain_set(MlpChainSet* out, int nchains, const void* const* planes, const float* const* bias, const int64_t* bias_idx0,
                       int bias_div0, int nlayers, const int* n_out, float* const* Y, const int* ldy);
int launch_mlp_chain_b6(const float* X, int ldx, const void* const* planes, const float* const* bias, const int64_t* bias_idx0, int bias_div0,
                        int nlayers, int n_out, float* Y, int ldy, int M, hipStream_t st);
int launch_wsplit128_strided(const float* W, int64_t sn, int64_t sk, int kseg, int k0, void* planes, hipStream_t st);
int launch_wsplit128_segs(const float* const* W, const int* k_end, int nseg, void* planes, hipStream_t st);
int launch_rowgemm128_b6p(const float* X, int ldx, const void* planes, const float* bias, const int64_t* bias_idx, int bias_div, float* Y,
                          int ldy, int M, int Kd, bool relu, hipStream_t st, float* parts = nullptr);
size_t rowgemm128_b6_parts_floats(int M, int Kd);
size_t rowgemm128_h3_parts_floats(int M, int Kd);
int launch_rowgemm128_b6(const float* X, int ldx, const float* W, int ldw, const float* bias, const int64_t* bias_idx, int bias_div, float* Y,
                         int ldy, int M, int Kd, bool relu, void* scratch, hipStream_t st);
bool use_b6_gemm(uint32_t flags = 0);
size_t xstat_b6_scratch_bytes(int N);
int launch_gemm_tn_h3(const float* A, int lda, const float* B, int ldb, float* C, int ldc, int M, int N1, int N2, float* db,
                      float* const* seg_ptrs, const int* seg_ends, int nseg, hipStream_t st);
size_t xstat_h3_scratch_bytes(int N);
int launch_xstat_h3(const float* X, const float* W, int64_t sn, int64_t sk, float* Y, int ldy, int rows, int N, void* scratch, hipStream_t st);
int launch_xstat_b6(const float* X, const float* W, int64_t sn, int64_t sk, float* Y, int ldy, int rows, int N, void* scratch, hipStream_t st);
bool gemm_tn_b6_ok(const float* A, int lda, const float* B, int ldb, int M, int N1, int N2);
int launch_gemm_tn_b6(const float* A, int lda, const float* B, int ldb, float* C, int ldc, int M, int N1, int N2, float* db,
                      float* const* seg_ptrs, const int* seg_ends, int nseg, hipStream_t st);
size_t ipa_layer_planes_bytes();
size_t ipa_layer_small_offset();
size_t ipa_layer_h3_pj_offset();
size_t ipa_layer_h3_out_offset();
size_t ipa_layer_h3_wis_offset();
size_t rowgemm128_h3_planes_bytes(int Kd);
size_t proj_frames_h3_planes_bytes();
int launch_wsplit128_h3(const float* W, int ldw, int Kd, void* planes, float* wis, hipStream_t st, int nrows = 128);
int launch_pjsplit_h3(const float* const* W6, void* planes, float* wis, hipStream_t st);
int launch_rowgemm128_h3p(const float* X, int ldx, const void* planes, const float* wis, const float* bias, const int64_t* bias_idx, int bias_div,
                          float* Y, int ldy, int M, int Kd, bool relu, hipStream_t st, float* parts = nullptr);
int launch_proj_frames_h3p(const float* x, const void* planes, const float* wis, const float* R, const float* t, float* proj, int rows,
                           hipStream_t st);
int ipa_layer_split_weights(const diffab_ipa_layer_weights* w, void* planes, hipStream_t st);
bool ipa_module_persistent_supported(const diffab_dims* d);
int launch_ipa_module_persistent(const diffab_dims* d, float* xa, float* xb, const float* R, const float* t, float* ws, const void* planes,
                                 const float* pair_planes, hipStream_t st, const float* emb_X = nullptr, const MlpChainSet* emb = nullptr,
                                 const MlpChainSet* heads = nullptr, const int* ctx_of_row = nullptr, int n_ctx = 0,
                                 const unsigned char* last_layer_tiles = nullptr);
void set_module_stagger(int ticks, int classes);
void set_module_stamps(void* device_buffer);
int launch_fold_embed_table(const diffab_dims* d, const diffab_denoiser_weights* w, float* emb_tab, hipStream_t st);
int launch_fold_beta_table(const diffab_dims* d, const diffab_denoiser_weights* w, const float* beta, float* beta_tab, hipStream_t st,
                           const float* sched_beta = nullptr, int t = 0, const int* t_dev = nullptr);

bool pair_embed_fused_supported(const diffab_ctx_dims* d);
size_t pair_embed_fused_prep_floats(const diffab_ctx_dims* d);
int launch_pair_embed_fused(const diffab_ctx_dims* d, const diffab_pair_emb_weights* w, const int64_t* seq_idx, const float* distmat,
                            const float* xyz, const float* pairwise_dihedrals, const int64_t* residue_idx, int32_t residue_idx_batch_stride,
                            const int64_t* chain_idx, const float* atom_mask, const uint8_t* sequence_context_mask, float* out, float* prep,
                            float* tape_h1, float* tape_df, float* tape_m1, float* tape_m2, int64_t row0, int64_t nrows, hipStream_t st,
                            const float** coef_sp_out = nullptr);
int launch_softplus_table(const float* coefw, int n, float* out, hipStream_t st);

bool attention_split_supported(const diffab_dims* d);
size_t attention_split_workspace_floats(const diffab_dims* d);
int launch_ipa_logits(const diffab_dims* d, const float* proj, const float* gamma, float* SP, hipStream_t st);
int launch_attention_probs(const diffab_dims* d, const float* proj, const float* e, const float* Wb, const float* gamma, float* P,
                           float* D2, hipStream_t st);
constexpr int kDeLayersMax = 6;
int launch_pair_de_layers(const diffab_dims* d, int nl, const float* const* P, const float* const* G, const float* const* doe,
                          const float* const* Wb, float* de, hipStream_t st);
int launch_pair_stream_bwd(const diffab_dims* d, const float* e, const float* P, float* G , const float* D2,
                           const float* dfeat, float* wb_part, const float* Wb, float* de ,
                           hipStream_t st);
int launch_attention_split(const diffab_dims* d, const float* proj, const float* e, const float* R, const float* t, const float* Wb,
                           const float* gamma, float* feat, float* SP, hipStream_t st, float* D2 = nullptr);

void set_stream_order(bool on);
int set_attn_variant(int v);
void set_attn_stamps(void* device_buffer);

void timer_begin(hipStream_t st);
void timer_end(hipStream_t st);
bool kernel_timer_enabled();

constexpr int kMaxLayers = 16;
struct TrainTape {
  float *cat2, *h1, *x[kMaxLayers + 1], *ipa_ws[kMaxLayers], *cat3, *t1[3], *t2[3], *vbuf, *logits;
  float* scratch;
  void* planes;
  float *sp[kMaxLayers], *d2[kMaxLayers];
};
size_t train_tape_floats(const diffab_dims* d);
TrainTape carve_tape(const diffab_dims* d, float* base);
constexpr size_t kAttnBwdLdsMax = 160 * 1024;
size_t attn_bwd_lds_bytes(const diffab_dims* d);
inline bool attn_bwd_lds_ok(const diffab_dims* d) { return attn_bwd_lds_bytes(d) <= kAttnBwdLdsMax; }
size_t train_bwd_workspace_floats(const diffab_dims* d);
int train_step_bwd(const diffab_dims* d, const diffab_denoiser_weights* w, const diffab_denoiser_weights* g, const TrainTape& tp,
                   const int64_t* seq_t, const float* x_t, const float* O_t, const float* pair_ctx, const float* eps_hat,
                   const float* O0_hat, const float* post_hat, const float* true_post, const float* true_eps, const float* true_O0,
                   const uint8_t* gm, const uint8_t* rm, const float* upstream3, float* d_res_ctx, float* d_pair_ctx, float* ws,
                   hipStream_t st);
int denoise_step_bwd(const diffab_dims* d, const diffab_denoiser_weights* w, const diffab_denoiser_weights* g, const TrainTape& tp,
                     const int64_t* seq_t, const float* x_t, const float* O_t, const float* pair_ctx, const float* post_hat,
                     const float* cot_eps, const float* cot_O0, const float* cot_post, float* d_res_ctx, float* d_pair_ctx, float* ws,
                     hipStream_t st, float* d_x_t = nullptr, float* d_O_t = nullptr);
int ipa_layer_bwd(const diffab_dims* d1, const diffab_ipa_layer_weights* lw, const diffab_ipa_layer_weights* lg, const TrainTape& tp,
                  const float* R, const float* t, const float* pair_ctx, const float* dy, float* dx, float* d_pair_ctx, float* ws,
                  hipStream_t st, float* d_R = nullptr, float* d_t = nullptr);
int bwd_linear(const float* dY, int ldy, const float* X, int ldx, const float* W, float* dW, float* db, float* dX, int lddx, int M, int N,
               int Kd, bool acc_dx, hipStream_t st);
int bwd_relu_mask(float* dY, const float* act, int64_t n, hipStream_t st);
int bwd_linear_masked(const float* dY, int ldy, const float* X, int ldx, const float* W, float* dW, float* db, float* dX, int lddx, int M,
                      int N, int Kd, const float* relu_act, hipStream_t st);
size_t pair_chain_bwd_prep_floats();
size_t pair_chain_bwd_part_floats();
int launch_pair_dist_bwd_fused(const int64_t* seq, const uint8_t* seq_m, const float* distmat, const float* xyz, const float* din, const float* dh1,
                               const float* W, int ld_w, int K, int A, int n_aa, int unk, int64_t row0, int64_t nrows, int ld, float* g_sp,
                               float* prep, hipStream_t st);
bool pair_dist_bwd_mfma_supported(int K, int A, int64_t row0, int64_t nrows, int ld, int n_aa);
int launch_pair_dist_bwd_mfma(const int64_t* seq, const uint8_t* seq_m, const float* distmat, const float* xyz, const float* din, const float* ddin,
                              int K, int A, int n_aa, int unk, int64_t row0, int64_t nrows, int ld, float* g_sp, hipStream_t st);
bool pair_table_mfma_supported(int C, int K, int64_t row0, int64_t nrows, int n_aa, int max_dist);
int launch_pair_table_mfma(const float* g, const int64_t* seq, const uint8_t* seq_m, const int64_t* resid, int resid_bstride, const int64_t* chain,
                           int K, int max_dist, int n_aa, int unk, int64_t row0, int64_t nrows, float* G1, float* part, hipStream_t st);
struct PartsSegs { int nseg; int off[8]; int n[8]; int cols[8]; int ld[8]; float* out[8]; };
int launch_parts_reduce(const float* parts, int nparts, int64_t stride, const PartsSegs& sg, hipStream_t st);
bool pair_chain_bwd_supported(int C, int K, int64_t row0, int64_t nrows);
bool pair_chain_bwd_enabled();
int launch_pair_chain_bwd(const float* d_out, const float* amask, int K, int A, int ca, int64_t row0, int64_t nrows, const float* const* X,
// ... 83 lines not shown
```

### diffab-pytorch_amd/csrc/ipa_attn_tile.h

```cpp
#pragma once
#include <hip/hip_runtime.h>
#include <cmath>
#include <cstdint>

namespace diffab {

typedef float f32x4 __attribute__((ext_vector_type(4)));
typedef float f32x16 __attribute__((ext_vector_type(16)));
typedef float f32x2 __attribute__((ext_vector_type(2)));

#ifndef MEM_FENCE
#define MEM_FENCE() asm volatile("" ::: "memory")
#endif

constexpr int AH = 8, ADS = 32, AP = 8, AC = 64;
constexpr int ANP = 3 * AH * ADS + 3 * AH * AP * 3;
constexpr int AF = AH * ADS + AH * AC + AH * AP * 3 + AH * AP;
constexpr int OFF_QS = 0, OFF_KS = 256, OFF_VS = 512, OFF_GQ = 768, OFF_GK = 960, OFF_GV = 1152;
constexpr int FOFF_OS = 0, FOFF_OE = 256, FOFF_OL = 768, FOFF_ON = 960;
constexpr int TI = 16;


#define FAST_EXP(x) __expf(x)

typedef _Float16 f16x8 __attribute__((ext_vector_type(8)));
typedef short s16x4_t __attribute__((ext_vector_type(4)));
typedef short s16x8_t __attribute__((ext_vector_type(8)));
template <int SD>
struct AttnP1Pre {
  f32x4 st[SD][4];
  f32x4 qa[2];
  f32x4 gqr[2];
};
struct AttnLaneOff { int s, p0, p1; };
__device__ __forceinline__ AttnLaneOff attn_lane_off(const int lane) {
  const int g0 = lane, g1 = lane + 64 < 96 ? lane + 64 : 95;
  return AttnLaneOff{(lane >> 3) * ANP + 4 * (lane & 7), (g0 / 6) * ANP + 4 * (g0 % 6), (g1 / 6) * ANP + 4 * (g1 % 6)};
}
__device__ __forceinline__ void attn_tile_request(f32x4 (&dst)[4], const float* __restrict__ proj, const int64_t row0, const int off_s,
                                                  const int off_p, const AttnLaneOff lo, const int h) {
  const float* us = proj + row0 * ANP + (off_s + h * ADS);
  const float* up = proj + row0 * ANP + (off_p + h * 24);
  dst[0] = *reinterpret_cast<const f32x4*>(us + lo.s);
  dst[1] = *reinterpret_cast<const f32x4*>(us + 8 * ANP + lo.s);
  dst[2] = *reinterpret_cast<const f32x4*>(up + lo.p0);
  dst[3] = *reinterpret_cast<const f32x4*>(up + lo.p1);
}
template <int SD>
__device__ __forceinline__ void attn_p1_request(AttnP1Pre<SD>& pre, const int piece, const float* __restrict__ proj, const int64_t prow0,
                                                const int64_t krow0, const int i0, const int lane, const AttnLaneOff lo, const int h) {
  if (piece < SD) {
    attn_tile_request(pre.st[piece], proj, krow0 + 16 * piece, OFF_KS, OFF_GK, lo, h);
    return;
  }
  const int l15 = lane & 15, q = lane >> 4;
  const float* uq = proj + (prow0 + i0) * ANP + h * ADS;
  pre.qa[0] = *reinterpret_cast<const f32x4*>(uq + OFF_QS + l15 * ANP + 4 * q);
  pre.qa[1] = *reinterpret_cast<const f32x4*>(uq + OFF_QS + 16 + l15 * ANP + 4 * q);
  const float* ug = proj + (prow0 + i0) * ANP + (OFF_GQ + h * 24);
  pre.gqr[0] = *reinterpret_cast<const f32x4*>(ug + lo.p0);
  pre.gqr[1] = *reinterpret_cast<const f32x4*>(ug + lo.p1);
}

template <bool PLANES, typename FP>
__device__ __forceinline__ void attn_shift_pair_rows(FP& e, FP& esc, const int* __restrict__ ctx_of_row, const int b, const int K) {
  if (ctx_of_row == nullptr) return;
  int c;
  asm volatile("s_load_dword %0, %1, 0x0\n\ts_waitcnt lgkmcnt(0)" : "=s"(c) : "s"(ctx_of_row + b) : "memory");
  const int64_t shift = static_cast<int64_t>(c - b) * K;
  e += shift * K * AC;
  if constexpr (PLANES) esc += 2 * shift;
}

template <int NT, bool MULTI, bool PLANES = false, bool TAPE = false>
__device__ __forceinline__ void ipa_attn_tile(float* __restrict__ S, const int b, const int tile, const unsigned stamp_id,
                                              const float* __restrict__ proj, const float* __restrict__ e,
                                              const float* __restrict__ R, const float* __restrict__ t,
                                              const float* __restrict__ Wb, const float* __restrict__ gamma,
                                              float* __restrict__ feat, int NC_arg,
                                              unsigned long long* __restrict__ stamps, const float* __restrict__ esc = nullptr,
                                              float* __restrict__ tape_p = nullptr, float* __restrict__ tape_d2 = nullptr,
                                              const int* __restrict__ ctx_of_row = nullptr) {
  static_assert(!PLANES || NT % 2 == 0, "the o_e product takes key tiles in pairs");
  static_assert(!TAPE || (!MULTI && !PLANES), "the tape form is the single-chunk fp32-pair kernel");
  const int NC = MULTI ? NC_arg : 1;
  constexpr int KC = NT * 16;
  const int K = NC * KC;
  auto stamp = [&](int k) {
    if (stamps != nullptr) {
      __builtin_amdgcn_sched_barrier(0);
#ifdef AT_STAMP_REALTIME
      const unsigned long long tnow = __builtin_amdgcn_s_memrealtime();
#else
      const unsigned long long tnow = __builtin_amdgcn_s_memtime();
#endif
      if ((threadIdx.x & 63) == 0) stamps[(static_cast<size_t>(stamp_id) * 8 + (threadIdx.x >> 6)) * 8 + k] = tnow;
      __builtin_amdgcn_sched_barrier(0);
    }
  };
  stamp(0);
  const int i0 = tile * TI;
  const int tid = threadIdx.x, lane0 = tid & 63, wv = __builtin_amdgcn_readfirstlane(tid >> 6);
  constexpr int HS = KC + 8, IS = AH * (KC + 8) + 8;
  const int64_t prow0 = static_cast<int64_t>(b) * K;
  attn_shift_pair_rows<PLANES>(e, esc, ctx_of_row, b, K);
  const float scale_t = 0.57735026918962576f;

  constexpr int KLD = 40, GLD = 28;
  constexpr int P1_TILE = 16 * KLD + 16 * GLD;
  constexpr int ELD = 72;
  constexpr int SCR_FLOATS = 2 * 16 * ELD;
  constexpr int E_LAG = MULTI ? 2 : 0;
  constexpr int E_EARLY = MULTI ? 1 : 2;
  float* scr = S + TI * IS + wv * SCR_FLOATS;
  float* st_fac = S + TI * IS + 8 * SCR_FLOATS;
  float* st_inv = st_fac + TI * AH;
  float* wb_lds = st_inv + TI * AH;
  float* gq_lds = wb_lds + (PLANES ? 0 : 4 * 64 * 4) + wv * (TI * 24);
  if (wv == 0 && !PLANES) {
    const int l15_ = lane0 & 15, q_ = lane0 >> 4;
#pragma unroll
    for (int sg = 0; sg < 4; ++sg) {
      f32x4 v = *reinterpret_cast<const f32x4*>(Wb + (l15_ & 7) * AC + 16 * sg + 4 * q_);
#pragma unroll
      for (int s_ = 0; s_ < 4; ++s_) v[s_] = l15_ < 8 ? v[s_] : 0.0f;
      *reinterpret_cast<f32x4*>(wb_lds + (sg * 64 + lane0) * 4) = v;
    }
  }

  const float* erow[2];
  float Mrun[2], Lrun[2];
#pragma unroll
  for (int ii = 0; ii < 2; ++ii) {
    erow[ii] = e + ((prow0 + i0 + 2 * wv + ii) * K) * AC;
    Mrun[ii] = -INFINITY;
    Lrun[ii] = 0.f;
  }
  float inv_s2[2];
#pragma unroll
  for (int ii = 0; ii < 2; ++ii) inv_s2[ii] = 1.0f;
  if constexpr (PLANES) {
    const float* ep = esc + 2 * (prow0 + i0 + 2 * __builtin_amdgcn_readfirstlane(static_cast<int>(threadIdx.x >> 6)));
#pragma unroll
    for (int ii = 0; ii < 2; ++ii) inv_s2[ii] = ep[2 * ii + 1];
  }

#pragma unroll 1
  for (int c = 0; c < NC; ++c) {
    const bool last = c == NC - 1;
    const int64_t krow0 = prow0 + c * KC;
    int lane = lane0;
    asm volatile("" : "+v"(lane));
    const int l15 = lane & 15, q = lane >> 4;
    f32x4 ev[2][NT][4];
    f32x4 wv4[2][2];
    auto load_e_tile = [&](int ii, int cc_, int jt) {
      if constexpr (PLANES) {
        const f32x4* ep = reinterpret_cast<const f32x4*>(erow[ii]) + (cc_ * NT + jt) * 256 + lane;
#pragma unroll
        for (int r = 0; r < 4; ++r) ev[ii][jt][r] = __builtin_nontemporal_load(ep + r * 64);
      } else {
        const f32x4* ep = reinterpret_cast<const f32x4*>(erow[ii] + (cc_ * KC + jt * 16 + 4 * q) * AC + 4 * l15);
#pragma unroll
        for (int r = 0; r < 4; ++r) ev[ii][jt][r] = __builtin_nontemporal_load(ep + r * (AC / 4));
      }
    };
    {
      const int h = wv;
      const float scale_s = 0.17677669529663687f;
      const float coef_p = -0.5f * 0.16666666666666666f * gamma[h];
      const int ks_dst = (lane >> 3) * KLD + 4 * (lane & 7);
      const int g0 = lane, g1 = lane + 64;
      const int gk_dst0 = 16 * KLD + (g0 / 6) * GLD + 4 * (g0 % 6), gk_dst1 = 16 * KLD + (g1 / 6) * GLD + 4 * (g1 % 6);
      constexpr int SD = MULTI ? 3 : 4;
      static_assert(E_EARLY <= SD, "the early pair tiles are requested in the last E_EARLY iterations, which must not request key tiles any more");
      AttnP1Pre<SD> pre;
      f32x4 (&st)[SD][4] = pre.st;
      const AttnLaneOff lo = attn_lane_off(lane);
      auto load_keys = [&](int sb, int jt) { attn_tile_request(st[sb], proj, krow0 + 16 * jt, OFF_KS, OFF_GK, lo, h); };
      auto stage_keys = [&](int sb, int lb) {
        float* t_ = scr + lb * P1_TILE;
        *reinterpret_cast<f32x4*>(t_ + ks_dst) = st[sb][0];
        *reinterpret_cast<f32x4*>(t_ + ks_dst + 8 * KLD) = st[sb][1];
        *reinterpret_cast<f32x4*>(t_ + gk_dst0) = st[sb][2];
        if (g1 < 96) *reinterpret_cast<f32x4*>(t_ + gk_dst1) = st[sb][3];
      };
      attn_p1_request<SD>(pre, SD, proj, prow0, krow0, i0, lane, lo, h);
#pragma unroll
      for (int piece = 0; piece < SD && piece < NT; ++piece) attn_p1_request<SD>(pre, piece, proj, prow0, krow0, i0, lane, lo, h);
      f32x4 (&qa)[2] = pre.qa;
      MEM_FENCE();
      *reinterpret_cast<f32x4*>(gq_lds + 4 * g0) = pre.gqr[0];
      if (g1 < 96) *reinterpret_cast<f32x4*>(gq_lds + 4 * g1) = pre.gqr[1];
      f32x4 gq[4][6];
#pragma unroll
      for (int r = 0; r < 4; ++r)
#pragma unroll
        for (int cc = 0; cc < 6; ++cc) gq[r][cc] = *reinterpret_cast<const f32x4*>(gq_lds + (4 * q + r) * 24 + 4 * cc);
      struct KeyFrag { f32x4 kb0, kb1, gk[6]; };
      auto read_frags = [&](int jt) {
        KeyFrag f;
        const float* t_ = scr + (jt & 1) * P1_TILE;
        f.kb0 = *reinterpret_cast<const f32x4*>(t_ + l15 * KLD + 4 * q);
        f.kb1 = *reinterpret_cast<const f32x4*>(t_ + l15 * KLD + 16 + 4 * q);
#pragma unroll
        for (int cc = 0; cc < 6; ++cc) f.gk[cc] = *reinterpret_cast<const f32x4*>(t_ + 16 * KLD + l15 * GLD + 4 * cc);
        return f;
      };
      stage_keys(0, 0);
      KeyFrag cur = read_frags(0);
      if (NT > 1) stage_keys(1 % SD, 1);
#pragma unroll
      for (int jt = 0; jt < NT; ++jt) {
        if (jt + 2 < NT) stage_keys((jt + 2) % SD, jt & 1);
        KeyFrag nxt = cur;
        if (jt + 1 < NT) nxt = read_frags(jt + 1);
        if (jt + SD < NT) {
          load_keys(jt % SD, jt + SD);
        } else if (jt + E_EARLY >= NT) {
          if constexpr (PLANES) {
            if (jt + E_EARLY == NT) {
              const int hh = lane & 7, qq = lane >> 4;
#pragma unroll
              for (int ks = 0; ks < 2; ++ks)
#pragma unroll
                for (int hf = 0; hf < 2; ++hf) wv4[ks][hf] = *reinterpret_cast<const f32x4*>(Wb + hh * AC + 32 * ks + 8 * qq + 4 * hf);
            }
          }
          load_e_tile(0, c, jt + E_EARLY - NT);
        }
        MEM_FENCE();
        const f32x4 kb0 = cur.kb0, kb1 = cur.kb1;
        f32x4 gk[6];
#pragma unroll
        for (int cc = 0; cc < 6; ++cc) gk[cc] = cur.gk[cc];
        cur = nxt;
        f32x4 acc = {0.f, 0.f, 0.f, 0.f};
#pragma unroll
        for (int s = 0; s < 4; ++s) acc = __builtin_amdgcn_mfma_f32_16x16x4f32(qa[0][s], kb0[s], acc, 0, 0, 0);
#pragma unroll
        for (int s = 0; s < 4; ++s) acc = __builtin_amdgcn_mfma_f32_16x16x4f32(qa[1][s], kb1[s], acc, 0, 0, 0);
#pragma unroll
        for (int r = 0; r < 4; ++r) {
          f32x2 d2v = {0.f, 0.f};
#pragma unroll
          for (int cc = 0; cc < 6; ++cc) {
            f32x2 dlo, dhi;
            asm("v_pk_add_f32 %0, %1, %2 neg_lo:[0,1] neg_hi:[0,1]"
                : "=v"(dlo)
                : "v"(__builtin_shufflevector(gq[r][cc], gq[r][cc], 0, 1)), "v"(__builtin_shufflevector(gk[cc], gk[cc], 0, 1)));
            asm("v_pk_add_f32 %0, %1, %2 neg_lo:[0,1] neg_hi:[0,1]"
                : "=v"(dhi)
                : "v"(__builtin_shufflevector(gq[r][cc], gq[r][cc], 2, 3)), "v"(__builtin_shufflevector(gk[cc], gk[cc], 2, 3)));
            d2v = __builtin_elementwise_fma(dlo, dlo, d2v);
            d2v = __builtin_elementwise_fma(dhi, dhi, d2v);
          }
          const float d2 = d2v[0] + d2v[1];
          S[(4 * q + r) * IS + h * HS + jt * 16 + l15] = scale_t * (acc[r] * scale_s + coef_p * d2);
          if constexpr (TAPE) tape_d2[((static_cast<int64_t>(b) * AH + h) * K + i0 + 4 * q + r) * K + jt * 16 + l15] = d2;
        }
        if (c == 0 && jt == 0) stamp(6);
        if (c == 0 && jt == 3) stamp(7);
      }
    }
    if (c == 0) stamp(1);
    {
      const int h = l15 & 7;
      constexpr int E_DEPTH_FP32 = 3;
      constexpr int RT = NT / 2;
      constexpr int E_DEPTH0 = PLANES ? RT : (E_DEPTH_FP32 < NT ? (E_DEPTH_FP32 > E_EARLY ? E_DEPTH_FP32 : E_EARLY) : NT);
      if constexpr (!PLANES) {
#pragma unroll
        for (int jt = E_EARLY; jt < E_DEPTH0; ++jt) load_e_tile(0, c, jt);
      }
      f32x4 wb[4];
      f16x8 wp[2][2];
      float bscale = scale_t, oscale = 1.0f;
      if constexpr (PLANES) {
        float wmax = 0.f;
#pragma unroll
        for (int ks = 0; ks < 2; ++ks)
#pragma unroll
          for (int hf = 0; hf < 2; ++hf)
#pragma unroll
            for (int s = 0; s < 4; ++s) wmax = fmaxf(wmax, fabsf(wv4[ks][hf][s]));
#pragma unroll
        for (int o = 1; o < 64; o <<= 1) wmax = fmaxf(wmax, __shfl_xor(wmax, o));
        const int ew = static_cast<int>((__float_as_uint(wmax) >> 23) & 255u);
        const float sw = (ew == 0 || ew > 230) ? 1.0f : __uint_as_float(static_cast<unsigned>(127 + 7 + 127 - ew) << 23);
        const float isw = (ew == 0 || ew > 230) ? 1.0f : __uint_as_float(static_cast<unsigned>(ew - 7) << 23);
#pragma unroll
        for (int ks = 0; ks < 2; ++ks)
#pragma unroll
          for (int c8 = 0; c8 < 8; ++c8) {
            const float x = l15 < 8 ? wv4[ks][c8 >> 2][c8 & 3] * sw : 0.0f;
            const _Float16 h1 = static_cast<_Float16>(x);
            wp[0][ks][c8] = h1;
            wp[1][ks][c8] = static_cast<_Float16>(x - static_cast<float>(h1));
          }
        bscale = scale_t * isw;
        oscale = 1.0f / 256.0f;
        asm volatile("" ::"v"(wp[0][0]), "v"(wp[1][0]), "v"(wp[0][1]), "v"(wp[1][1]));
#pragma unroll
        for (int jt = E_EARLY; jt < E_DEPTH0; ++jt) load_e_tile(0, c, jt);
      } else if constexpr (!MULTI) {
#pragma unroll
        for (int sg = 0; sg < 4; ++sg) {
          wb[sg] = *reinterpret_cast<const f32x4*>(Wb + h * AC + 16 * sg + 4 * q);
#pragma unroll
          for (int s = 0; s < 4; ++s) wb[sg][s] = l15 < 8 ? wb[sg][s] : 0.0f;
        }
      }
      MEM_FENCE();
      __syncthreads();
      if (c == 0) stamp(2);
      auto stage_e = [&](int ii, int jt) {
        float* t_ = scr + (jt & 1) * (16 * ELD) + 4 * q * ELD + 4 * l15;
#pragma unroll
        for (int r = 0; r < 4; ++r) *reinterpret_cast<f32x4*>(t_ + r * ELD) = ev[ii][jt][r];
      };

      if constexpr (PLANES) {
        char* trt = reinterpret_cast<char*>(scr);
        const int wr_off = l15 * 128 + 8 * ((2 * q) ^ (4 * ((l15 >> 1) & 3)) ^ (2 * (l15 & 1)));
        const int rrow = 4 * q + (l15 >> 2);
        const int rd_off = rrow * 128 + 8 * ((l15 & 3) ^ (4 * ((rrow >> 1) & 3)) ^ (2 * (rrow & 1)));
#pragma unroll
        for (int ii = 0; ii < 2; ++ii) {
          const int il = 2 * wv + ii;
          float* Srow = S + il * IS + h * HS;
          const float inv_s = inv_s2[ii];
          const float bscale_r = bscale * inv_s, oscale_r = oscale * inv_s;
          float m_run = -INFINITY, l_run = 0.f, m_hist[NT / 2];
          f32x4 oe[4];
#pragma unroll
          for (int ct = 0; ct < 4; ++ct) oe[ct] = f32x4{0.f, 0.f, 0.f, 0.f};
#pragma unroll
          for (int T = 0; T < NT / 2; ++T) {
            f32x4 acc[2][2];
#pragma unroll
            for (int tl = 0; tl < 2; ++tl)
#pragma unroll
              for (int ks = 0; ks < 2; ++ks) {
                const f16x8 a1 = __builtin_bit_cast(f16x8, ev[ii][2 * T + tl][ks]), a2 = __builtin_bit_cast(f16x8, ev[ii][2 * T + tl][2 + ks]);
                f32x4 a_ = {0.f, 0.f, 0.f, 0.f};
                a_ = __builtin_amdgcn_mfma_f32_16x16x32_f16(a2, wp[0][ks], a_, 0, 0, 0);
                a_ = __builtin_amdgcn_mfma_f32_16x16x32_f16(a1, wp[1][ks], a_, 0, 0, 0);
                a_ = __builtin_amdgcn_mfma_f32_16x16x32_f16(a1, wp[0][ks], a_, 0, 0, 0);
                acc[tl][ks] = a_;
              }
            float v[8], smax = -INFINITY;
#pragma unroll
            for (int tl = 0; tl < 2; ++tl) {
              const f32x4 sv = *reinterpret_cast<const f32x4*>(Srow + (2 * T + tl) * 16 + 4 * q);
#pragma unroll
              for (int r = 0; r < 4; ++r) {
                v[4 * tl + r] = sv[r] + bscale_r * (acc[tl][0][r] + acc[tl][1][r]);
                smax = fmaxf(smax, v[4 * tl + r]);
              }
            }
            smax = fmaxf(smax, __shfl_xor(smax, 16));
            smax = fmaxf(smax, __shfl_xor(smax, 32));
            const float m_new = fmaxf(m_run, smax);
            const float alpha = T == 0 ? 0.0f : FAST_EXP(m_run - m_new);
            m_run = m_new;
            m_hist[T] = m_new;
            float psum = 0.f;
#pragma unroll
            for (int tt = 0; tt < 8; ++tt) {
              v[tt] = FAST_EXP(v[tt] - m_new);
              psum += v[tt];
            }
            l_run = l_run * alpha + psum;
            if (T > 0) {
#pragma unroll
              for (int ct = 0; ct < 4; ++ct)
#pragma unroll
                for (int r = 0; r < 4; ++r) oe[ct][r] *= alpha;
            }
            f16x8 p1, p2;
#pragma unroll
            for (int tt = 0; tt < 8; ++tt) {
              const float x = 256.0f * v[tt];
              const _Float16 hh = static_cast<_Float16>(x);
              p1[tt] = hh;
              p2[tt] = static_cast<_Float16>(x - static_cast<float>(hh));
            }
#pragma unroll
            for (int tl = 0; tl < 2; ++tl) {
              if (l15 < 8) *reinterpret_cast<f32x4*>(Srow + (2 * T + tl) * 16 + 4 * q) = f32x4{v[4 * tl], v[4 * tl + 1], v[4 * tl + 2], v[4 * tl + 3]};
#pragma unroll
              for (int pl = 0; pl < 2; ++pl)
#pragma unroll
                for (int ks = 0; ks < 2; ++ks)
                  *reinterpret_cast<f32x4*>(trt + (tl * 2 + pl) * 2048 + (wr_off ^ (64 * ks))) = ev[ii][2 * T + tl][2 * pl + ks];
            }
            {
              constexpr int dummy_ = 0;
              (void)dummy_;
              const int nx = ii * NT + 2 * T + RT;
              if (nx < 2 * NT) {
                load_e_tile(nx / NT, c, nx % NT);
                load_e_tile((nx + 1) / NT, c, (nx + 1) % NT);
                MEM_FENCE();
              }
            }
            f16x8 a[2][4];
#pragma unroll
            for (int pl = 0; pl < 2; ++pl)
#pragma unroll
              for (int ct = 0; ct < 4; ++ct) {
                const int ro = rd_off ^ (32 * ct);
                const s16x4_t lo = __builtin_amdgcn_ds_read_tr16_b64_v4i16((s16x4_t __attribute__((address_space(3)))*)(trt + (0 * 2 + pl) * 2048 + ro));
                const s16x4_t hi = __builtin_amdgcn_ds_read_tr16_b64_v4i16((s16x4_t __attribute__((address_space(3)))*)(trt + (1 * 2 + pl) * 2048 + ro));
                const s16x8_t v8 = {lo[0], lo[1], lo[2], lo[3], hi[0], hi[1], hi[2], hi[3]};
                a[pl][ct] = __builtin_bit_cast(f16x8, v8);
              }
#pragma unroll
            for (int ct = 0; ct < 4; ++ct) oe[ct] = __builtin_amdgcn_mfma_f32_16x16x32_f16(a[1][ct], p1, oe[ct], 0, 0, 0);
#pragma unroll
            for (int ct = 0; ct < 4; ++ct) oe[ct] = __builtin_amdgcn_mfma_f32_16x16x32_f16(a[0][ct], p2, oe[ct], 0, 0, 0);
#pragma unroll
            for (int ct = 0; ct < 4; ++ct) oe[ct] = __builtin_amdgcn_mfma_f32_16x16x32_f16(a[0][ct], p1, oe[ct], 0, 0, 0);
          }
          l_run += __shfl_xor(l_run, 16);
          l_run += __shfl_xor(l_run, 32);
          const float Mnew = MULTI ? fmaxf(Mrun[ii], m_run) : m_run;
          const float fac = (!MULTI || c == 0) ? 0.0f : expf(Mrun[ii] - Mnew);
          const float cf = MULTI ? expf(m_run - Mnew) : 1.0f;
          Mrun[ii] = Mnew;
          Lrun[ii] = Lrun[ii] * fac + l_run * cf;
          const float inv = last ? 1.0f / Lrun[ii] : 1.0f;
#pragma unroll
          for (int T = 0; T < NT / 2 - (MULTI ? 0 : 1); ++T) {
            const float f = FAST_EXP(m_hist[T] - Mnew);
            if (l15 < 8) {
#pragma unroll
              for (int tl = 0; tl < 2; ++tl) {
                f32x4* sp = reinterpret_cast<f32x4*>(Srow + (2 * T + tl) * 16 + 4 * q);
                f32x4 pv = *sp;
#pragma unroll
                for (int r = 0; r < 4; ++r) pv[r] *= f;
                *sp = pv;
              }
            }
          }
          if (l15 < 8) {
            float* fo = feat + (prow0 + i0 + il) * AF + FOFF_OE + h * AC + 4 * q;
            const float sc = cf * oscale_r;
#pragma unroll
            for (int ct = 0; ct < 4; ++ct) {
              f32x4 o = oe[ct];
#pragma unroll
              for (int r = 0; r < 4; ++r) o[r] *= sc;
              if (MULTI && c > 0) {
                const f32x4 old = *reinterpret_cast<const f32x4*>(fo + 16 * ct);
#pragma unroll
                for (int r = 0; r < 4; ++r) o[r] += old[r] * fac;
              }
#pragma unroll
              for (int r = 0; r < 4; ++r) o[r] *= inv;
              *reinterpret_cast<f32x4*>(fo + 16 * ct) = o;
            }
            if (q == 0) {
              st_fac[il * AH + h] = fac;
              st_inv[il * AH + h] = inv;
            }
          }
        }
      } else {
#pragma unroll
      for (int ii = 0; ii < 2; ++ii) {
        const int il = 2 * wv + ii;
        float* Srow = S + il * IS + h * HS;
        float lg[NT][4];
        float mx = -INFINITY;
        stage_e(ii, 0);
#pragma unroll
        for (int jt = 0; jt < NT; ++jt) {
          f32x4 acc = {0.f, 0.f, 0.f, 0.f}, acc2 = {0.f, 0.f, 0.f, 0.f};
          {
            if (jt + 1 < NT) stage_e(ii, jt + 1);
            const float* t_ = scr + (jt & 1) * (16 * ELD) + l15 * ELD + 4 * q;
#pragma unroll
            for (int sg = 0; sg < 4; ++sg) {
              const f32x4 ea = *reinterpret_cast<const f32x4*>(t_ + 16 * sg);
              const f32x4 wbf = MULTI ? *reinterpret_cast<const f32x4*>(wb_lds + (sg * 64 + lane) * 4) : wb[sg];
#pragma unroll
              for (int s = 0; s < 4; ++s) {
                if (sg & 1) acc2 = __builtin_amdgcn_mfma_f32_16x16x4f32(ea[s], wbf[s], acc2, 0, 0, 0);
                else acc = __builtin_amdgcn_mfma_f32_16x16x4f32(ea[s], wbf[s], acc, 0, 0, 0);
              }
            }
          }
          if (ii == 0 && jt + E_DEPTH0 < NT) {
            load_e_tile(0, c, jt + E_DEPTH0);
            MEM_FENCE();
          }
          const f32x4 sv = *reinterpret_cast<const f32x4*>(Srow + jt * 16 + 4 * q);
// ... 191 lines not shown
```

### diffab-pytorch_amd/csrc/ipa_persistent.hip

```cpp
#include "common.h"
#include "denoiser_internal.h"
#define AT_STAMP_REALTIME 1
#include "ipa_attn_tile.h"
#include "proj_frames_h3_tile.h"
#include "rowgemm_h3_tile.h"
#include "mlp_chain_tile.h"

namespace diffab {

namespace {
constexpr size_t cmax(size_t a, size_t b) { return a > b ? a : b; }
constexpr size_t kModuleLdsBytes = cmax(cmax(ipa_attn_lds_bytes(8), static_cast<size_t>(kChainLdsBytes)),
                                        cmax(static_cast<size_t>(pjh3::PJ_LDS_BYTES), static_cast<size_t>(h3tile::lds_bytes<128>())));
constexpr size_t kXImageOffset = cmax(static_cast<size_t>(pjh3::PJ_LDS_BYTES), static_cast<size_t>(h3tile::lds_bytes<128>())) / 4;
static_assert(kXImageOffset * 4 + h3tile::y_lds_bytes<128>() <= kModuleLdsBytes, "module LDS: no room for the x image of the dense phases");
static_assert(kModuleLdsBytes <= 160 * 1024, "module LDS: one work-group per CU within gfx950's 160 KiB");
static_assert(kXImageOffset % 4 == 0, "x image: 16-byte aligned rows");

struct ModuleArgs {
  float* xa;
  float* xb;
  float* proj;
  float* feat;
  const float* pair;
  const float* esc;
  const int* ctx_of_row;
  const unsigned char* last_layer_tiles;
  const float* R;
  const float* t;
  const char* planes;
  size_t layer_stride, pj_off, out_off, wis_off, small_off;
  unsigned long long* stamps;
  const float* emb_X;
  MlpChainSet emb, heads;
  int B, NL;
  int stagger_ticks, stagger_classes;
};
}

__device__ __forceinline__ bool module_tile_needed(const unsigned char* __restrict__ map, const int idx) {
  unsigned w;
  asm volatile("s_load_dword %0, %1, 0x0\n\ts_waitcnt lgkmcnt(0)" : "=s"(w) : "s"(map + (idx & ~3)) : "memory");
  return ((w >> (8 * (idx & 3))) & 0xffu) != 0;
}

template <int KRES>
__global__ __launch_bounds__(512) void ipa_module_persistent_kernel(const ModuleArgs a) {
  extern __shared__ __attribute__((aligned(16))) float lds[];
  constexpr int K = KRES, NTILE = K / TI, DT = K / 128;
  static_assert(KRES == 128 || KRES == 256, "patch-resident module: K = 128 or 256");
  const int M = a.B * K;
  if (a.stagger_ticks > 0 && a.stagger_classes > 1) {
    const unsigned long long t0 = __builtin_amdgcn_s_memrealtime();
    const unsigned long long wait = static_cast<unsigned long long>((blockIdx.x >> 3) % a.stagger_classes) * a.stagger_ticks;
    while (__builtin_amdgcn_s_memrealtime() - t0 < wait) __builtin_amdgcn_s_sleep(32);
  }
  unsigned long long* pstamps = a.stamps ? a.stamps + static_cast<size_t>(a.B) * a.NL * NTILE * 64 : nullptr;
  auto pstamp = [&](int b, int l, int k) {
    if (pstamps != nullptr && threadIdx.x == 0) pstamps[(static_cast<size_t>(b) * a.NL + l) * 4 + k] = __builtin_amdgcn_s_memrealtime();
  };
#pragma unroll 1
  for (int b = blockIdx.x; b < a.B; b += gridDim.x) {
    if (a.emb_X != nullptr) {
#pragma unroll 1
      for (int dt = 0; dt < DT; ++dt) {
        int tid = threadIdx.x;
        asm volatile("" : "+v"(tid));
        chaintile::mlp_chain_tile(reinterpret_cast<__bf16*>(lds), tid, b * DT + dt, a.emb_X, 128, a.emb.c[0].planes[0], a.emb.c[0].planes[1],
                                  nullptr, a.emb.c[0].bias[0], a.emb.c[0].bias[1], nullptr, a.emb.c[0].bias_idx0, a.emb.c[0].bias_div0, 2, 128,
                                  a.xa, 128, M);
        asm volatile("s_waitcnt vmcnt(0)" ::: "memory");
        __syncthreads();
      }
    }
#pragma unroll 1
    for (int l = 0; l < a.NL; ++l) {
      const char* lp = a.planes + static_cast<size_t>(l) * a.layer_stride;
      const float* small = reinterpret_cast<const float*>(lp + a.small_off);
      const float* xin = (l & 1) ? a.xb : a.xa;
      float* xout = (l & 1) ? a.xa : a.xb;
      pstamp(b, l, 0);
#pragma unroll 1
      for (int dt = 0; dt < DT; ++dt) {
        int tid = threadIdx.x;
        asm volatile("" : "+v"(tid));
        if (KRES == 128) {
          if (l == 0) {
            float* xl = lds + kXImageOffset;
            for (int i = tid; i < 128 * 32; i += 512) {
              const int row = i >> 5, c4 = 4 * (i & 31);
              *reinterpret_cast<float4*>(xl + row * h3tile::Y_LDS_LD + c4) =
                  *reinterpret_cast<const float4*>(xin + (static_cast<int64_t>(b) * 128 + row) * 128 + c4);
            }
            __syncthreads();
          }
          pjh3::proj_frames_h3_tile<true, false, true, true>(reinterpret_cast<_Float16*>(lds), tid, b, 0, 1, nullptr,
                                                             reinterpret_cast<const _Float16*>(lp + a.pj_off),
                                                             reinterpret_cast<const float*>(lp + a.wis_off), a.R, a.t, a.proj, M, 0, 0, 0,
                                                             lds + kXImageOffset);
        } else {
          pjh3::proj_frames_h3_tile<true, false>(reinterpret_cast<_Float16*>(lds), tid, b * DT + dt, 0, 1, xin,
                                                 reinterpret_cast<const _Float16*>(lp + a.pj_off), reinterpret_cast<const float*>(lp + a.wis_off),
                                                 a.R, a.t, a.proj, M);
        }
        if (dt + 1 < DT) {
          asm volatile("s_waitcnt vmcnt(0)" ::: "memory");
          __syncthreads();
        }
      }
      asm volatile("s_waitcnt vmcnt(0)" ::: "memory");
      __syncthreads();
      pstamp(b, l, 1);
      const unsigned char* needed = l + 1 == a.NL ? a.last_layer_tiles : nullptr;
#pragma unroll 1
      for (int tile = 0; tile < NTILE; ++tile) {
        if (needed != nullptr && !module_tile_needed(needed, b * NTILE + tile)) continue;
        ipa_attn_tile<8, (KRES > 128), true>(lds, b, tile, static_cast<unsigned>((b * a.NL + l) * NTILE + tile), a.proj, a.pair, a.R, a.t, small,
                                             small + 512, a.feat, K / 128, a.stamps, a.esc, nullptr, nullptr, a.ctx_of_row);
        asm volatile("s_waitcnt vmcnt(0)" ::: "memory");
        __syncthreads();
      }
      pstamp(b, l, 2);
#pragma unroll 1
      for (int dt = 0; dt < DT; ++dt) {
        int tid = threadIdx.x;
        asm volatile("" : "+v"(tid));
        if (KRES == 128)
          h3tile::rowgemm128_h3_tile<false, 128, false, true>(reinterpret_cast<_Float16*>(lds), tid, b, a.feat, AF,
                                                              reinterpret_cast<const _Float16*>(lp + a.out_off),
                                                              reinterpret_cast<const float*>(lp + a.wis_off) + ANP, small + 576, nullptr, 0,
                                                              l + 1 == a.NL ? xout : nullptr, 128, M, AF, 0, nullptr, lds + kXImageOffset);
        else
          h3tile::rowgemm128_h3_tile<false, 128>(reinterpret_cast<_Float16*>(lds), tid, b * DT + dt, a.feat, AF,
                                                 reinterpret_cast<const _Float16*>(lp + a.out_off),
                                                 reinterpret_cast<const float*>(lp + a.wis_off) + ANP, small + 576, nullptr, 0, xout, 128, M, AF);
        if (dt + 1 < DT) {
          asm volatile("s_waitcnt vmcnt(0)" ::: "memory");
          __syncthreads();
        }
      }
      asm volatile("s_waitcnt vmcnt(0)" ::: "memory");
      __syncthreads();
      pstamp(b, l, 3);
    }
    if (a.emb_X != nullptr) {
      const float* xfin = (a.NL & 1) ? a.xb : a.xa;
#pragma unroll 1
      for (int hdt = 0; hdt < 3 * DT; ++hdt) {
        const int hd = hdt / DT, dt = hdt % DT;
        int tid = threadIdx.x;
        asm volatile("" : "+v"(tid));
#define HSEL(f) (hd == 0 ? a.heads.c[0].f : hd == 1 ? a.heads.c[1].f : a.heads.c[2].f)
        chaintile::mlp_chain_tile(reinterpret_cast<__bf16*>(lds), tid, b * DT + dt, xfin, 128, HSEL(planes[0]), HSEL(planes[1]), HSEL(planes[2]),
                                  HSEL(bias[0]), HSEL(bias[1]), HSEL(bias[2]), HSEL(bias_idx0), HSEL(bias_div0), 3, HSEL(n_out),
                                  hd == 0 ? a.heads.Y[0] : hd == 1 ? a.heads.Y[1] : a.heads.Y[2],
                                  hd == 0 ? a.heads.ldy[0] : hd == 1 ? a.heads.ldy[1] : a.heads.ldy[2], M);
#undef HSEL
        asm volatile("s_waitcnt vmcnt(0)" ::: "memory");
        __syncthreads();
      }
    }
  }
}

namespace {
int g_stagger_ticks = 1000, g_stagger_classes = 8;
unsigned long long* g_module_stamps = nullptr;
}
void set_module_stagger(int ticks, int classes) {
  g_stagger_ticks = ticks;
  g_stagger_classes = classes;
}
void set_module_stamps(void* p) { g_module_stamps = static_cast<unsigned long long*>(p); }

bool ipa_module_persistent_supported(const diffab_dims* d) {
  return fast_path_supported(d) && (d->K == 128 || d->K == 256) && d->NL >= 1;
}

int launch_ipa_module_persistent(const diffab_dims* d, float* xa, float* xb, const float* R, const float* t, float* ws, const void* planes,
                                 const float* pair_planes, hipStream_t st, const float* emb_X, const MlpChainSet* emb,
                                 const MlpChainSet* heads, const int* ctx_of_row, int n_ctx, const unsigned char* last_layer_tiles) {
  DIFFAB_REQUIRE(ipa_module_persistent_supported(d) && xa && xb && R && t && ws && planes && pair_planes, DIFFAB_ERR_ARG,
                 "ipa_module_persistent: unsupported operands");
  DIFFAB_REQUIRE((reinterpret_cast<uintptr_t>(last_layer_tiles) & 3) == 0, DIFFAB_ERR_ARG,
                 "ipa_module_persistent: the row-tile map must be 4-byte aligned");
  const size_t rows = static_cast<size_t>(d->B) * d->K;
  ModuleArgs a{};
  a.xa = xa;
  a.xb = xb;
  a.proj = ws;
  a.feat = ws + rows * ANP;
  a.pair = pair_planes + 64;
  a.esc = pair_row_scales(d, pair_planes, n_ctx);
  a.ctx_of_row = ctx_of_row;
  a.last_layer_tiles = last_layer_tiles;
  a.R = R;
  a.t = t;
  a.planes = static_cast<const char*>(planes);
  a.layer_stride = ipa_layer_planes_bytes();
  a.pj_off = ipa_layer_h3_pj_offset();
  a.out_off = ipa_layer_h3_out_offset();
  a.wis_off = ipa_layer_h3_wis_offset();
  a.small_off = ipa_layer_small_offset();
  a.stamps = g_module_stamps;
  if (emb_X != nullptr) {
    DIFFAB_REQUIRE(emb && heads && d->D == 128 && (reinterpret_cast<uintptr_t>(emb_X) & 15) == 0, DIFFAB_ERR_ARG,
                   "ipa_module_persistent: the fused MLP phases need both chain sets");
    a.emb_X = emb_X;
    a.emb = *emb;
    a.heads = *heads;
  }
  a.B = d->B;
  a.NL = d->NL;
  a.stagger_ticks = g_stagger_ticks;
  a.stagger_classes = g_stagger_classes;
  int dev = 0, ncu = 256;
  if (hipGetDevice(&dev) == hipSuccess) (void)hipDeviceGetAttribute(&ncu, hipDeviceAttributeMultiprocessorCount, dev);
  const int grid = d->B < ncu ? d->B : ncu;
#define MODULE_LAUNCH(K_)                                                                                                       \
  do {                                                                                                                            \
    DIFFAB_HIP_CHECK(hipFuncSetAttribute(reinterpret_cast<const void*>(ipa_module_persistent_kernel<K_>),                         \
                                         hipFuncAttributeMaxDynamicSharedMemorySize, static_cast<int>(kModuleLdsBytes)));        \
    timer_begin(st);                                                                                                              \
    hipLaunchKernelGGL((ipa_module_persistent_kernel<K_>), dim3(grid), dim3(512), kModuleLdsBytes, st, a);                        \
    timer_end(st);                                                                                                                \
  } while (0)
  if (d->K == 128) MODULE_LAUNCH(128);
  else MODULE_LAUNCH(256);
#undef MODULE_LAUNCH
  DIFFAB_LAUNCH_CHECK();
  return DIFFAB_OK;
}

}
```

### diffab-pytorch_amd/diffab_pytorch/_hip.py

```python
from __future__ import annotations

import ctypes as C
import os
from typing import Dict, Optional, Sequence

import torch

_HERE = os.path.dirname(os.path.abspath(__file__))
LIB_PATH = os.environ.get("DIFFAB_HIP_LIB") or os.path.join(os.path.dirname(_HERE), "lib", "libdiffab_hip.so")

FLAG_FORCE_GENERIC = 1
FLAG_PAIR_F32 = 64
FLAG_FP32_GEMM = 128
FLAG_PAIR_PLANES = 32
FLAG_GRAPH_SAMPLER = 16
FLAG_PERSISTENT_MODULE = 512
FLAG_MULTI_LAUNCH = 1024
FLAG_SKIP_UNUSED_ROWS = 256
FLAG_ALL_ROWS = 8192
FLAG_KEEP_STRUCTURE = 2048
FLAG_KEEP_SEQUENCE = 4096


class HipUnavailable(RuntimeError):
    pass


class DiffabHipError(RuntimeError):
    pass


class Dims(C.Structure):
    _fields_ = [(n, C.c_int32) for n in ("B", "K", "D", "C", "H", "DS", "PQ", "PV", "NL", "V")]


_fp = C.c_void_p


class IpaLayerWeights(C.Structure):
    _fields_ = [(n, _fp) for n in ("gamma", "wq_s", "wk_s", "wv_s", "w_bias", "wq_p", "wk_p", "wv_p", "w_out", "b_out")]


class Mlp3Weights(C.Structure):
    _fields_ = [(n, _fp) for n in ("w0", "b0", "w2", "b2", "w4", "b4")]


class DenoiserWeights(C.Structure):
    _fields_ = [
        ("seq_emb", _fp), ("res_w0", _fp), ("res_b0", _fp), ("res_w2", _fp), ("res_b2", _fp),
        ("layers", C.POINTER(IpaLayerWeights)),
        ("coord", Mlp3Weights), ("orient", Mlp3Weights), ("seq", Mlp3Weights),
    ]


class CtxDims(C.Structure):
    _fields_ = [(n, C.c_int32) for n in ("B", "K", "A", "D", "C", "max_dist")]


class ResidueEmbWeights(C.Structure):
    _fields_ = [(n, _fp) for n in ("aa_emb", "chain_emb", "w0", "b0", "w2", "b2", "w4", "b4", "w6", "b6")]


class PairEmbWeights(C.Structure):
    _fields_ = [(n, _fp) for n in ("aa_pair_emb", "relpos_emb", "pair2distcoef", "dw0", "db0", "dw2", "db2", "mw0", "mb0", "mw2", "mb2",
                                   "mw4", "mb4")]


class Sched(C.Structure):
    _fields_ = [("T", C.c_int32), ("alpha", _fp), ("alpha_bar", _fp), ("alpha_bar_sqrt", _fp),
                ("one_minus_alpha_bar_sqrt", _fp), ("beta", _fp)]


class Igso3(C.Structure):
    _fields_ = [("n_sigmas", C.c_int32), ("n_bins", C.c_int32), ("sigmas", _fp), ("cdf", _fp), ("sigma_threshold", C.c_float)]


class ScoreNoised(C.Structure):
    _fields_ = [(n, _fp) for n in ("seq_t", "x_t", "O_t", "eps")]


class SampleRecord(C.Structure):
    _fields_ = [("n_slots", C.c_int32), ("slot_of_step", C.POINTER(C.c_int32)), ("slot_dev", _fp)] + \
        [(n, _fp) for n in ("seq", "x", "O", "pred_x", "pred_O", "seq_probs")]


class SampleSteps(C.Structure):
    _fields_ = [("n_steps", C.c_int32), ("steps", C.POINTER(C.c_int32)), ("beta_jump", C.POINTER(C.c_float)),
                ("alpha_jump", C.POINTER(C.c_float)), ("plan_dev", _fp)]


class SampleGuidance(C.Structure):
    _fields_ = [(n, C.c_float) for n in ("w_clash", "clash_distance", "w_bond", "bond_length", "max_shift")] + \
        [("t_max", C.c_int32)] + [(n, _fp) for n in ("chain", "residue_idx", "residue_mask", "shift_dev")]


class SampleTemperature(C.Structure):
    _fields_ = [(n, _fp) for n in ("trans_scale", "rot_scale", "seq_temp", "rot_row")]


_i32, _i64, _u32, _u64, _sz = C.c_int32, C.c_int64, C.c_uint32, C.c_uint64, C.c_size_t
_PD, _PS, _PI = C.POINTER(Dims), C.POINTER(Sched), C.POINTER(Igso3)
SYMBOLS = {
    "diffab_version": (C.c_char_p, []),
    "diffab_last_error": (C.c_char_p, []),
    "diffab_device_ok": (C.c_int, []),
    "diffab_kernel_timer_enable": (C.c_int, [C.c_int]),
    "diffab_debug_set_attn_stamps": (C.c_int, [_fp]),
    "diffab_debug_set_attn_variant": (C.c_int, [_i32]),
    "diffab_debug_set_module_stagger": (C.c_int, [_i32, _i32]),
    "diffab_debug_set_module_stamps": (C.c_int, [_fp]),
    "diffab_debug_row_tiles": (C.c_int, [_fp, _i32, _i32, _fp, _fp]),
    "diffab_set_stream_guard": (C.c_int, [C.c_int]),
    "diffab_debug_linear128": (C.c_int, [_fp, _fp, _fp, _fp, C.c_int64, C.c_int32, C.c_int32, _fp, C.c_size_t, _fp]),
    "diffab_debug_gemm_tn": (C.c_int, [_fp, _fp, _fp, _fp, C.c_int64, C.c_int32, C.c_int32, C.c_int32, _fp]),
    "diffab_debug_xstat128": (C.c_int, [_fp, _fp, _fp, C.c_int64, C.c_int32, C.c_int32, _fp, C.c_size_t, _fp]),
    "diffab_kernel_timer_read": (C.c_int, [C.POINTER(C.c_int64), C.POINTER(C.c_double)]),
    "diffab_so3_log": (C.c_int, [_fp, _fp, _i64, _fp]),
    "diffab_so3_exp": (C.c_int, [_fp, _fp, _i64, _fp]),
    "diffab_so3_matrix_to_rotvec": (C.c_int, [_fp, _fp, _i64, _fp]),
    "diffab_so3_rotvec_to_matrix": (C.c_int, [_fp, _fp, _i64, _fp]),
    "diffab_so3_scale_rot": (C.c_int, [_fp, _fp, _fp, _i64, _i64, _fp]),
    "diffab_igso3_table_build": (C.c_int, [_fp, _i32, _i32, _i32, _fp, _fp]),
    "diffab_igso3_table_build_accurate": (C.c_int, [_fp, _i32, _i32, _i32, _fp, _fp]),
    "diffab_igso3_cdf_build": (C.c_int, [_fp, _i32, _i32, _fp, _fp]),
    "diffab_igso3_sample": (C.c_int, [_PI, _fp, _i32, _i32, _fp, _fp, _fp, _fp, _fp, _fp]),
    "diffab_igso3_bins_without_replacement": (C.c_int, [_fp, _i32, _i32, _fp, _i32, _i32, _fp, _fp, _fp, C.c_float, _fp]),
    "diffab_igso3_sample_bins": (C.c_int, [_PI, _fp, _i32, _i32, _fp, _fp, _fp, _fp, _fp, _fp]),
    "diffab_weighted_multinomial": (C.c_int, [_fp, _fp, _fp, _fp, _i64, _i64, _fp, _fp]),
    "diffab_seq_forward_prob": (C.c_int, [_PS, C.c_int, _fp, _fp, _fp, _i32, _i32, _fp, _fp]),
    "diffab_seq_posterior": (C.c_int, [_PS, _fp, _fp, _fp, _fp, _i32, _i32, _fp, _fp]),
    "diffab_categorical_sample": (C.c_int, [_fp, _fp, _i64, _i32, _fp, _fp]),
    "diffab_coord_forward": (C.c_int, [_PS, _fp, _fp, _fp, _fp, _i32, _i32, _fp, _fp]),
    "diffab_orient_forward": (C.c_int, [_PS, _fp, _fp, _fp, _fp, _i32, _i32, _fp, _fp]),
    "diffab_philox_fill": (C.c_int, [_u64, _i64, _i32, _i32, _i32, _i32, C.c_int, _fp, _fp]),
    "diffab_denoise_workspace_bytes": (_sz, [_PD]),
    "diffab_sample_workspace_bytes": (_sz, [_PD]),
    "diffab_sample_shared_workspace_bytes": (_sz, [_PD, _i32]),
    "diffab_ipa_layer_fwd": (C.c_int, [_PD, C.POINTER(IpaLayerWeights), _fp, _fp, _fp, _fp, _fp, _fp, _sz, _u32, _fp]),
    "diffab_denoise_step_fwd": (C.c_int, [_PD, C.POINTER(DenoiserWeights), _fp, _fp, _fp, _fp, _fp, _fp, _fp, _fp, _fp, _fp, _fp,
                                          _fp, _sz, _u32, _fp]),
    "diffab_losses_fwd": (C.c_int, [_fp, _fp, _fp, _fp, _fp, _fp, _fp, _fp, _i32, _i32, _i32, _fp, _fp]),
    "diffab_train_tape_bytes": (_sz, [_PD]),
    "diffab_train_workspace_bytes": (_sz, [_PD]),
    "diffab_train_step_fwd": (C.c_int, [_PD, C.POINTER(DenoiserWeights)] + [_fp] * 16 + [_sz, _u32, _fp]),
    "diffab_train_step_bwd": (C.c_int, [_PD, C.POINTER(DenoiserWeights), C.POINTER(DenoiserWeights)] + [_fp] * 16 + [_sz, _fp, _sz, _fp]),
    "diffab_residue_embedding_workspace_bytes": (_sz, [C.POINTER(CtxDims)]),
    "diffab_residue_embedding_fwd": (C.c_int, [C.POINTER(CtxDims), C.POINTER(ResidueEmbWeights)] + [_fp] * 10 + [_sz, _fp]),
    "diffab_pair_embedding_workspace_bytes": (_sz, [C.POINTER(CtxDims)]),
    "diffab_pair_embedding_fwd": (C.c_int, [C.POINTER(CtxDims), C.POINTER(PairEmbWeights), _fp, _fp, _fp, _fp, _i32, _fp, _fp, _fp, _fp,
                                            _fp, _sz, _fp]),
    "diffab_pair_embedding_xyz_fwd": (C.c_int, [C.POINTER(CtxDims), C.POINTER(PairEmbWeights), _fp, _fp, _fp, _fp, _i32, _fp, _fp, _fp, _fp,
                                                _fp, _sz, _fp]),
    "diffab_residue_embedding_bwd_workspace_bytes": (_sz, [C.POINTER(CtxDims)]),
    "diffab_residue_embedding_bwd": (C.c_int, [C.POINTER(CtxDims), C.POINTER(ResidueEmbWeights), C.POINTER(ResidueEmbWeights)] + [_fp] * 10
                                     + [_sz, _fp]),
    "diffab_pair_embedding_bwd_workspace_bytes": (_sz, [C.POINTER(CtxDims)]),
    "diffab_pair_embedding_bwd": (C.c_int, [C.POINTER(CtxDims), C.POINTER(PairEmbWeights), C.POINTER(PairEmbWeights), _fp, _fp, _fp, _fp, _fp,
                                            _i32, _fp, _fp, _fp, _fp, _fp, _sz, _fp]),
    "diffab_pair_embedding_tape_bytes": (_sz, [C.POINTER(CtxDims)]),
    "diffab_pair_embedding_fwd_taped": (C.c_int, [C.POINTER(CtxDims), C.POINTER(PairEmbWeights), _fp, _fp, _fp, _fp, _fp, _i32, _fp, _fp, _fp,
                                                  _fp, _fp, _sz, _fp, _sz, _fp]),
    "diffab_pair_embedding_bwd_taped": (C.c_int, [C.POINTER(CtxDims), C.POINTER(PairEmbWeights), C.POINTER(PairEmbWeights), _fp, _fp, _fp, _fp,
                                                  _fp, _i32, _fp, _fp, _fp, _fp, _fp, _sz, _fp, _sz, _fp]),
    "diffab_featurize_xyz": (C.c_int, [_fp, _fp, _fp, _i32, _i32, _i32, _fp, _fp, _fp, _fp, _fp]),
    "diffab_patch_select": (C.c_int, [_fp, _i32, _fp, _fp, _fp, _fp, _fp, _i32, _i32, _i32, _i32, _i32, _fp, _fp, _fp, _fp]),
    "diffab_patch_gather": (C.c_int, [_fp, _fp, C.POINTER(_i32), _i32, _i32, _i32, _i32, _i64, _fp, _fp]),
    "diffab_patch_scatter": (C.c_int, [_fp, _fp, _fp, _i32, _i32, _i32, _i64, _fp, _fp]),
    "diffab_metrics_vs_native": (C.c_int, [_fp] * 7 + [_i32] * 5 + [_fp] * 7),
    "diffab_metrics_pairwise": (C.c_int, [_fp] * 4 + [_i32] * 5 + [_fp, _fp, _fp, _sz, _fp]),
    "diffab_metrics_select_diverse": (C.c_int, [_fp, _fp, _fp, _i32, _i32, _i32, _fp, _fp, _fp, _fp]),
    "diffab_orientation_loss": (C.c_int, [_fp, _fp, _i64, _fp, _fp, _fp]),
    "diffab_orientation_loss_bwd": (C.c_int, [_fp, _fp, _i64, _fp, _fp, _fp, _fp, _fp]),
    "diffab_frames_apply": (C.c_int, [_fp, _fp, _fp, _fp, _i32, _i32, _i32, _i32, _fp]),
    "diffab_frames_invert": (C.c_int, [_fp, _fp, _fp, _fp, _i32, _i32, _i32, _i32, _fp]),
    "diffab_frames_bwd": (C.c_int, [_fp, _fp, _fp, _fp, _i32, _fp, _fp, _i32, _i32, _i32, _i32, _fp]),
    "diffab_angular_encoding": (C.c_int, [_fp, _i64, _i32, _fp, _fp]),
    "diffab_angular_encoding_bwd": (C.c_int, [_fp, _fp, _i64, _i32, _fp, _fp]),
    "diffab_denoise_step_fwd_taped": (C.c_int, [_PD, C.POINTER(DenoiserWeights)] + [_fp] * 10 + [_sz, _u32, _fp]),
    "diffab_denoise_step_bwd": (C.c_int, [_PD, C.POINTER(DenoiserWeights), C.POINTER(DenoiserWeights)] + [_fp] * 13 + [_sz, _fp, _sz, _fp]),
    "diffab_ipa_layer_tape_bytes": (_sz, [_PD]),
    "diffab_ipa_layer_bwd_workspace_bytes": (_sz, [_PD]),
    "diffab_ipa_layer_fwd_taped": (C.c_int, [_PD, C.POINTER(IpaLayerWeights), _fp, _fp, _fp, _fp, _fp, _fp, _sz, _u32, _fp]),
    "diffab_ipa_layer_bwd": (C.c_int, [_PD, C.POINTER(IpaLayerWeights), C.POINTER(IpaLayerWeights), _fp, _fp, _fp, _fp, _fp, _fp, _fp, _fp, _fp,
                                       _sz, _fp, _sz, _fp]),
    "diffab_reverse_update": (C.c_int, [_PS, _i32, _fp, _fp, _fp, _fp, _fp, _fp, _fp, _fp, _fp, _fp, _i32, _i32, _i32, _fp]),
    "diffab_sample_loop": (C.c_int, [_PD, C.POINTER(DenoiserWeights), _PS, _PI, _fp, _fp, _fp, _fp, _fp, _fp, _u64, _i64, _i32,
                                     _i32, _fp, _sz, _u32, _fp]),
    "diffab_sample_loop_shared": (C.c_int, [_PD, C.POINTER(DenoiserWeights), _PS, _PI, _fp, _fp, _fp, _fp, _fp, _i32, C.POINTER(_i32), _fp,
                                            _u64, _i64, _i32, _i32, _fp, _sz, _u32, _fp]),
    "diffab_sample_init": (C.c_int, [_fp, _fp, _fp, _fp, _u64, _i64, _i32, _i32, _i32, _fp]),
    "diffab_sample_init_ex": (C.c_int, [_fp, _fp, _fp, _fp, _u64, _i64, _i32, _i32, _i32, _u32, _fp]),
    "diffab_sample_init_noised": (C.c_int, [_PS, _PI, _fp, _fp, _fp, _fp, _u64, _i64, _i32, _i32, _i32, _u32, _fp]),
    "diffab_sample_loop_aa": (C.c_int, [_PD, C.POINTER(DenoiserWeights), _PS, _PI, _fp, _fp, _fp, _fp, _fp, _i32, C.POINTER(_i32), _fp,
                                        _u64, _i64, _i32, _i32, _fp, _sz, _u32, _fp, _fp]),
# ... 134 lines not shown
```

### include/diffab_hip.h

```cpp
#ifndef DIFFAB_HIP_H
#define DIFFAB_HIP_H

#include <stddef.h>
#include <stdint.h>

#ifdef __cplusplus
extern "C" {
#endif

#define DIFFAB_OK 0
#define DIFFAB_ERR_ARG (-1)
#define DIFFAB_ERR_UNSUPPORTED (-2)
#define DIFFAB_ERR_HIP (-3)
#define DIFFAB_ERR_WORKSPACE (-4)

#define DIFFAB_FLAG_FORCE_GENERIC 1u

#define DIFFAB_FLAG_PAIR_PLANES 32u

#define DIFFAB_FLAG_PAIR_F32 64u
#define DIFFAB_FLAG_FP32_GEMM 128u

#define DIFFAB_FLAG_GRAPH_SAMPLER 16u
#define DIFFAB_FLAG_PERSISTENT_MODULE 512u
#define DIFFAB_FLAG_MULTI_LAUNCH 1024u
#define DIFFAB_FLAG_ALL_ROWS 8192u
#define DIFFAB_FLAG_SKIP_UNUSED_ROWS 256u
#define DIFFAB_FLAG_KEEP_STRUCTURE 2048u
#define DIFFAB_FLAG_KEEP_SEQUENCE 4096u

typedef struct {
  int32_t B;
  int32_t K;
  int32_t D;
  int32_t C;
  int32_t H;
  int32_t DS;
  int32_t PQ;
  int32_t PV;
  int32_t NL;
  int32_t V;
} diffab_dims;

typedef struct {
  const float* gamma;
  const float* wq_s;
  const float* wk_s;
  const float* wv_s;
  const float* w_bias;
  const float* wq_p;
  const float* wk_p;
  const float* wv_p;
  const float* w_out;
  const float* b_out;
} diffab_ipa_layer_weights;

typedef struct {
  const float *w0, *b0;
  const float *w2, *b2;
  const float *w4, *b4;
} diffab_mlp3_weights;

typedef struct {
  const float* seq_emb;
  const float *res_w0, *res_b0;
  const float *res_w2, *res_b2;
  const diffab_ipa_layer_weights* layers;
  diffab_mlp3_weights coord;
  diffab_mlp3_weights orient;
  diffab_mlp3_weights seq;
} diffab_denoiser_weights;

typedef struct {
  int32_t T;
  const float* alpha;
  const float* alpha_bar;
  const float* alpha_bar_sqrt;
  const float* one_minus_alpha_bar_sqrt;
  const float* beta;
} diffab_sched;

typedef struct {
  int32_t n_sigmas;
  int32_t n_bins;
  const float* sigmas;
  const float* cdf;
  float sigma_threshold;
} diffab_igso3;

const char* diffab_version(void);
const char* diffab_last_error(void);
int diffab_device_ok(void);

int diffab_kernel_timer_enable(int on);
int diffab_debug_set_attn_stamps(void* device_buffer);
int diffab_debug_set_attn_variant(int32_t v);
int diffab_debug_set_module_stagger(int32_t ticks_10ns, int32_t classes);
int diffab_debug_set_module_stamps(void* device_buffer);
int diffab_debug_row_tiles(const uint8_t* gen_mask, int32_t B, int32_t K, uint8_t* tiles, void* stream);
int diffab_set_stream_guard(int on);
int diffab_debug_linear128(const float* X, const float* W, const float* bias, float* Y, int64_t M, int32_t Kd, int32_t mode, void* scratch,
                           size_t scratch_bytes, void* stream);
int diffab_debug_xstat128(const float* X, const float* W, float* Y, int64_t M, int32_t N, int32_t mode, void* scratch, size_t scratch_bytes,
                          void* stream);
int diffab_debug_gemm_tn(const float* A, const float* B, float* C, float* db, int64_t M, int32_t N1, int32_t N2, int32_t mode, void* stream);
int diffab_kernel_timer_read(int64_t* launches, double* total_ms);
int diffab_so3_log(const float* R, float* S, int64_t n, void* stream);
int diffab_so3_exp(const float* S, float* R, int64_t n, void* stream);
int diffab_so3_matrix_to_rotvec(const float* R, float* v, int64_t n, void* stream);
int diffab_so3_rotvec_to_matrix(const float* v, float* R, int64_t n, void* stream);
int diffab_so3_scale_rot(const float* R, const float* k, float* out, int64_t n, int64_t per_k, void* stream);

int diffab_igso3_table_build(const float* sigmas, int32_t n_sigmas, int32_t n_bins, int32_t num_iters, float* pdf, void* stream);
int diffab_igso3_table_build_accurate(const float* sigmas, int32_t n_sigmas, int32_t n_bins, int32_t num_iters, float* pdf,
                                      void* stream);
int diffab_igso3_cdf_build(const float* pdf, int32_t n_sigmas, int32_t n_bins, float* cdf, void* stream);
int diffab_igso3_sample(const diffab_igso3* tab, const int64_t* sigma_idx, int32_t B, int32_t K, const float* axis_raw,
                        const float* u_bin, const float* u_in, const float* z, float* rotvec, void* stream);

int diffab_igso3_bins_without_replacement(const float* pdf, int32_t n_sigmas, int32_t n_bins, const int64_t* sigma_idx, int32_t B,
                                          int32_t K, const float* race, int32_t* bins, const float* sigmas, float sigma_threshold,
                                          void* stream);
int diffab_igso3_sample_bins(const diffab_igso3* tab, const int64_t* sigma_idx, int32_t B, int32_t K, const float* axis_raw,
                             const int32_t* bins, const float* u_in, const float* z, float* rotvec, void* stream);

int diffab_weighted_multinomial(const float* p1, const float* p2, const float* w1, const float* w2, int64_t n, int64_t per_b,
                                float* out, void* stream);
int diffab_seq_forward_prob(const diffab_sched* s, int mode, const int64_t* seq, const int64_t* t, const uint8_t* mask,
                            int32_t B, int32_t K, float* prob , void* stream);
int diffab_seq_posterior(const diffab_sched* s, const int64_t* seq_t, const int64_t* seq_0, const int64_t* t,
                         const uint8_t* mask, int32_t B, int32_t K, float* post , void* stream);
int diffab_categorical_sample(const float* prob, const float* u, int64_t n_rows, int32_t V, int64_t* out, void* stream);
int diffab_coord_forward(const diffab_sched* s, const float* x0, const int64_t* t, const uint8_t* mask, const float* eps,
                         int32_t B, int32_t K, float* xt, void* stream);
int diffab_orient_forward(const diffab_sched* s, const float* O0, const uint8_t* mask, const int64_t* t,
                          const float* rotvec, int32_t B, int32_t K, float* Ot, void* stream);

int diffab_philox_fill(uint64_t seed, int64_t first_patch, int32_t B, int32_t K, int32_t step, int32_t stream_id, int kind,
                       float* out, void* stream);

size_t diffab_denoise_workspace_bytes(const diffab_dims* d);
size_t diffab_sample_workspace_bytes(const diffab_dims* d);
size_t diffab_sample_shared_workspace_bytes(const diffab_dims* d, int32_t n_ctx);
int diffab_ipa_layer_fwd(const diffab_dims* d, const diffab_ipa_layer_weights* w, const float* x ,
                         const float* e , const float* R , const float* t ,
                         float* y , void* workspace, size_t workspace_bytes, uint32_t flags, void* stream);
int diffab_denoise_step_fwd(const diffab_dims* d, const diffab_denoiser_weights* w, const int64_t* seq_t, const float* x_t,
                            const float* O_t, const float* res_ctx, const float* pair_ctx, const float* beta ,
                            float* out_eps, float* out_O0, float* out_posterior, float* out_logits, float* out_res_emb,
                            void* workspace, size_t workspace_bytes, uint32_t flags, void* stream);

int diffab_losses_fwd(const float* pred_post, const float* true_post, const float* pred_eps, const float* true_eps,
                      const float* pred_O0, const float* true_O0, const uint8_t* gen_mask, const uint8_t* res_mask,
                      int32_t B, int32_t K, int32_t V, float* losses3, void* stream);

size_t diffab_train_tape_bytes(const diffab_dims* d);
size_t diffab_train_workspace_bytes(const diffab_dims* d);
int diffab_train_step_fwd(const diffab_dims* d, const diffab_denoiser_weights* w, const int64_t* seq_t, const float* x_t,
                          const float* O_t, const float* res_ctx, const float* pair_ctx, const float* beta, const float* true_post,
                          const float* true_eps, const float* true_O0, const uint8_t* gen_mask, const uint8_t* res_mask,
                          float* out_eps, float* out_O0, float* out_posterior, float* losses3, void* tape, size_t tape_bytes,
                          uint32_t flags, void* stream);
int diffab_train_step_bwd(const diffab_dims* d, const diffab_denoiser_weights* w, const diffab_denoiser_weights* grads,
                          const int64_t* seq_t, const float* x_t, const float* O_t, const float* pair_ctx, const float* out_eps,
                          const float* out_O0, const float* out_posterior, const float* true_post, const float* true_eps,
                          const float* true_O0, const uint8_t* gen_mask, const uint8_t* res_mask, const float* upstream3,
                          float* d_res_ctx, float* d_pair_ctx, const void* tape, size_t tape_bytes, void* workspace,
                          size_t workspace_bytes, void* stream);

int diffab_orientation_loss(const float* pred, const float* target, int64_t n, float* elems, float* sum1, void* stream);
int diffab_orientation_loss_bwd(const float* pred, const float* target, int64_t n, const float* g_elems, const float* g_total,
                                float* d_pred, float* d_target, void* stream);

int diffab_frames_apply(const float* x, const float* R, const float* t, float* out, int32_t B, int32_t N, int32_t L, int32_t P, void* stream);
int diffab_frames_invert(const float* x, const float* R, const float* t, float* out, int32_t B, int32_t N, int32_t L, int32_t P, void* stream);
int diffab_frames_bwd(const float* x, const float* R, const float* t, const float* g_out, int32_t invert, float* dR, float* dt, int32_t B,
                      int32_t N, int32_t L, int32_t P, void* stream);
int diffab_angular_encoding(const float* x, int64_t n, int32_t num_funcs, float* out, void* stream);
int diffab_angular_encoding_bwd(const float* enc, const float* g_out, int64_t n, int32_t num_funcs, float* dx, void* stream);

int diffab_denoise_step_fwd_taped(const diffab_dims* d, const diffab_denoiser_weights* w, const int64_t* seq_t, const float* x_t,
                                  const float* O_t, const float* res_ctx, const float* pair_ctx, const float* beta, float* out_eps,
                                  float* out_O0, float* out_posterior, void* tape, size_t tape_bytes, uint32_t flags, void* stream);
int diffab_denoise_step_bwd(const diffab_dims* d, const diffab_denoiser_weights* w, const diffab_denoiser_weights* grads,
                            const int64_t* seq_t, const float* x_t, const float* O_t, const float* pair_ctx, const float* out_posterior,
                            const float* d_eps, const float* d_O0, const float* d_posterior, float* d_res_ctx, float* d_pair_ctx,
                            float* d_x_t, float* d_O_t, const void* tape, size_t tape_bytes, void* workspace, size_t workspace_bytes,
                            void* stream);
size_t diffab_ipa_layer_tape_bytes(const diffab_dims* d);
size_t diffab_ipa_layer_bwd_workspace_bytes(const diffab_dims* d);
int diffab_ipa_layer_fwd_taped(const diffab_dims* d, const diffab_ipa_layer_weights* w, const float* x, const float* e, const float* R,
                               const float* t, float* y, void* tape, size_t tape_bytes, uint32_t flags, void* stream);
int diffab_ipa_layer_bwd(const diffab_dims* d, const diffab_ipa_layer_weights* w, const diffab_ipa_layer_weights* grads, const float* e,
                         const float* R, const float* t, const float* dy, float* dx, float* d_e, float* d_R, float* d_t, const void* tape,
                         size_t tape_bytes, void* workspace, size_t workspace_bytes, void* stream);

typedef struct {
  int32_t B, K;
  int32_t A;
  int32_t D;
  int32_t C;
  int32_t max_dist;
} diffab_ctx_dims;

typedef struct {
  const float *aa_emb, *chain_emb;
  const float *w0, *b0, *w2, *b2, *w4, *b4, *w6, *b6;
} diffab_residue_emb_weights;

typedef struct {
  const float *aa_pair_emb, *relpos_emb, *pair2distcoef;
  const float *dw0, *db0, *dw2, *db2;
  const float *mw0, *mb0, *mw2, *mb2, *mw4, *mb4;
} diffab_pair_emb_weights;

size_t diffab_residue_embedding_workspace_bytes(const diffab_ctx_dims* d);
int diffab_residue_embedding_fwd(const diffab_ctx_dims* d, const diffab_residue_emb_weights* w, const int64_t* seq_idx,
                                 const float* xyz , const float* orientations, const float* dihedrals ,
                                 const int64_t* chain_idx, const float* atom_mask, const uint8_t* structure_context_mask,
                                 const uint8_t* sequence_context_mask, float* out, void* workspace, size_t workspace_bytes,
                                 void* stream);
size_t diffab_pair_embedding_workspace_bytes(const diffab_ctx_dims* d);
int diffab_pair_embedding_fwd(const diffab_ctx_dims* d, const diffab_pair_emb_weights* w, const int64_t* seq_idx,
                              const float* distmat , const float* pairwise_dihedrals ,
                              const int64_t* residue_idx, int32_t residue_idx_batch_stride, const int64_t* chain_idx,
// ... 175 lines not shown
```

Baseline: 14.70 million.

## Hoist per-layer pair bias out of the sampling loop into a precomputed table

Adds a one-time pair_hoist kernel that splits the pair context into fp16 planes and precomputes the pair-bias logits for every IPA layer once per sampling run. The attention tile then reads these precomputed biases instead of recomputing the pair-feature × to_pair_bias product every denoise step. The pair context and weights are fixed across steps, so this is legitimate reuse within a call. In exchange it adds a large workspace of NL×K×K×H floats, extra global reads per step, and a new templated attention variant.

```diff
diff --git a/diffab-pytorch_amd/csrc/api.hip b/diffab-pytorch_amd/csrc/api.hip
--- a/diffab-pytorch_amd/csrc/api.hip
+++ b/diffab-pytorch_amd/csrc/api.hip
@@ -127,11 +127,12 @@
                               const float* t, float* y, float* ws, uint32_t flags, hipStream_t st, float* sp_keep = nullptr,
                               float* d2_keep = nullptr, const void* planes = nullptr, const float* pair_planes = nullptr,
                               bool taped = false,
-                              const unsigned char* tile_needed = nullptr, const int* ctx_of_row = nullptr, int n_ctx = 0) {
+                              const unsigned char* tile_needed = nullptr, const int* ctx_of_row = nullptr, int n_ctx = 0,
+                              const float* pair_bias = nullptr, const float* pair_bias_isw = nullptr) {
   DIFFAB_REQUIRE(ipa_layer_weights_ok(d, w), DIFFAB_ERR_ARG, "ipa layer: null weight pointer");
   if (!(flags & DIFFAB_FLAG_FORCE_GENERIC) && fast_path_supported(d))
     return ipa_layer_fast(d, w, x, e, R, t, y, ws, st, sp_keep, d2_keep, planes, pair_planes, (flags & DIFFAB_FLAG_FP32_GEMM) != 0,
-                          taped, tile_needed, ctx_of_row, n_ctx);
+                          taped, tile_needed, ctx_of_row, n_ctx, pair_bias, pair_bias_isw);
   return ipa_layer_generic(d, w, x, e, R, t, y, ws, st, ctx_of_row);
 }
 
@@ -167,6 +168,7 @@
   bool chain;
   bool persistent, fused_mlps;
   const float* pair_planes;
+  float* pair_bias;
   const int* ctx_of_row;
   int n_ctx;
   const unsigned char* last_layer_tiles;
@@ -174,7 +176,8 @@
 };
 
 static ForwardPlan plan_forward(const diffab_dims* d, uint32_t flags, const StepBuffers& b, const float* res_ctx, const float* pair_ctx,
-                                float* res_emb, bool loop, const int* ctx_of_row = nullptr, int n_ctx = 0, unsigned char* tiles = nullptr) {
+                                float* res_emb, bool loop, const int* ctx_of_row = nullptr, int n_ctx = 0, unsigned char* tiles = nullptr,
+                                float* pair_bias = nullptr) {
   const int rows = d->B * d->K, D = d->D;
   if (loop && !(flags & DIFFAB_FLAG_PAIR_F32)) flags |= DIFFAB_FLAG_PAIR_PLANES;
   ForwardPlan p{};
@@ -183,6 +186,8 @@
   p.b6 = p.fold && use_b6_gemm(flags) && rowgemm128_b6_ok(res_ctx, D, b.h1, D, rows, D);
   p.chain = p.b6 && d->V <= 128;
   p.pair_planes = use_pair_planes(d, flags, pair_ctx, b) ? b.pair : nullptr;
+  p.pair_bias = p.pair_planes != nullptr && pair_bias != nullptr && pair_hoist_supported(d) && !(flags & DIFFAB_FLAG_INLINE_PAIR_BIAS)
+                    ? pair_bias : nullptr;
   p.ctx_of_row = ctx_of_row;
   p.n_ctx = n_ctx;
   p.last_layer_tiles = tiles != nullptr && !(flags & DIFFAB_FLAG_ALL_ROWS) && p.fold && d->K % 16 == 0 && d->NL >= 2 ? tiles : nullptr;
@@ -221,8 +226,11 @@
       if (int rc = launch_wsplit128(hw[hd]->w4, D, D, mlp + (8 + hd) * mlp_planes_bytes(), st, nout)) return rc;
     }
   }
-  if (p.pair_planes)
+  if (p.pair_bias) {
+    if (int rc = launch_pair_hoist(d, pair_ctx, w->layers, b.pair, p.pair_bias, st, p.n_ctx)) return rc;
+  } else if (p.pair_planes) {
     if (int rc = launch_pair_split(d, pair_ctx, b.pair, st, p.n_ctx)) return rc;
+  }
   if (bias.beta_traj) {
     diffab_dims dt = *d;
     dt.B = bias.traj_rows;
@@ -282,14 +290,15 @@
   }
   if (p.persistent) {
     if (int rc = launch_ipa_module_persistent(d, b.hA, b.hB, O_t, x_t, b.ipa, b.planes, p.pair_planes, st, p.fused_mlps ? res_ctx : nullptr,
-                                              &emb_set, &head_set, p.ctx_of_row, p.n_ctx, p.last_layer_tiles))
+                                              &emb_set, &head_set, p.ctx_of_row, p.n_ctx, p.last_layer_tiles, p.pair_bias))
       return rc;
     cur = (d->NL & 1) ? b.hB : b.hA;
   }
   for (int l = 0; l < d->NL && !p.persistent; ++l) {
     const void* planes = p.b6 ? b.planes + l * ipa_layer_planes_bytes() : nullptr;
     if (int rc = ipa_layer_dispatch(d, &w->layers[l], cur, pair_ctx, O_t, x_t, nxt, b.ipa, p.flags, st, nullptr, nullptr, planes, p.pair_planes,
-                                    false, l == d->NL - 1 ? p.last_layer_tiles : nullptr, p.ctx_of_row, p.n_ctx))
+                                    false, l == d->NL - 1 ? p.last_layer_tiles : nullptr, p.ctx_of_row, p.n_ctx,
+                                    p.pair_bias ? pair_bias_layer(d, p.pair_bias, l, p.n_ctx) : nullptr, p.pair_bias ? p.pair_bias + l : nullptr))
       return rc;
     float* tmp = cur; cur = nxt; nxt = tmp;
   }
@@ -353,6 +362,7 @@
   float* beta_traj;
   int* ctx_of_row;
   float* res_ctx;
+  float* pair_bias;
   void* step;
   size_t bytes;
 };
@@ -372,6 +382,7 @@
   s.res_ctx = mapped ? c.take<float>(rows * d->D) : nullptr;
   const size_t step_bytes = carve_step(d, nullptr, n_pair).bytes;
   s.step = c.take<char>(step_bytes);
+  s.pair_bias = pair_hoist_supported(d) ? c.take<float>(pair_bias_floats(d, n_pair)) : nullptr;
   s.bytes = c.bytes();
   return s;
 }
@@ -487,6 +498,21 @@
 }
 
 int diffab_debug_set_attn_variant(int32_t v) { return set_attn_variant(v); }
+
+size_t diffab_debug_pair_hoist_floats(const diffab_dims* d, int32_t which) {
+  if (check_dims(d, "debug_pair_hoist_floats") || !pair_hoist_supported(d)) return 0;
+  return which == 0 ? pair_planes_floats(d) : pair_bias_floats(d);
+}
+
+int diffab_debug_pair_hoist(const diffab_dims* d, const float* pair_ctx, const diffab_denoiser_weights* w, float* planes_inline,
+                            float* planes_hoisted, float* bias, void* stream) {
+  StreamOrder order_(stream);
+  if (int rc = check_dims(d, "debug_pair_hoist")) return rc;
+  DIFFAB_REQUIRE(pair_hoist_supported(d) && pair_ctx && w && w->layers && planes_inline && planes_hoisted && bias, DIFFAB_ERR_ARG,
+                 "debug_pair_hoist: needs K = 128 on the MFMA geometry and every buffer");
+  if (int rc = launch_pair_split(d, pair_ctx, planes_inline, as_stream(stream))) return rc;
+  return launch_pair_hoist(d, pair_ctx, w->layers, planes_hoisted, bias, as_stream(stream));
+}
 
 int diffab_debug_set_attn_stamps(void* device_buffer) {
   set_attn_stamps(device_buffer);
@@ -901,7 +927,7 @@
     res_ctx = sb.res_ctx;
   }
   const StepBuffers b0 = carve_step(d, sb.step, n_ctx);
-  const ForwardPlan plan = plan_forward(d, flags, b0, res_ctx, pair_ctx, nullptr, true, ctx_dev, n_ctx, sb.tiles);
+  const ForwardPlan plan = plan_forward(d, flags, b0, res_ctx, pair_ctx, nullptr, true, ctx_dev, n_ctx, sb.tiles, sb.pair_bias);
   StepBias bias{sb.beta, plan.fold ? s->beta : nullptr, 0, nullptr, nullptr, s->T + 1};
   if (plan.chain && s->T + 1 <= kTrajRows && !(flags & DIFFAB_FLAG_GRAPH_SAMPLER)) bias.beta_traj = sb.beta_traj;
   if (int rc = prepare_forward(d, w, plan, b0, pair_ctx, bias, st)) return rc;
diff --git a/diffab-pytorch_amd/csrc/denoiser_fast.hip b/diffab-pytorch_amd/csrc/denoiser_fast.hip
--- a/diffab-pytorch_amd/csrc/denoiser_fast.hip
+++ b/diffab-pytorch_amd/csrc/denoiser_fast.hip
@@ -295,7 +295,7 @@
   return launch_linear_bn<64>(X, ldx, segs, bias, Y, ldy, M, N, Kd, relu, vec, st);
 }
 
-template <int NT, bool MULTI, bool PLANES = false, bool TAPE = false>
+template <int NT, bool MULTI, bool PLANES = false, bool TAPE = false, bool HOISTED = false>
 __global__ __launch_bounds__(512) void ipa_attn_fast_kernel(const float* __restrict__ proj, const float* __restrict__ e,
                                                             const float* __restrict__ R, const float* __restrict__ t,
                                                             const float* __restrict__ Wb, const float* __restrict__ gamma,
@@ -303,7 +303,9 @@
                                                             unsigned long long* __restrict__ stamps, const float* __restrict__ esc = nullptr,
                                                             float* __restrict__ tape_p = nullptr, float* __restrict__ tape_d2 = nullptr,
                                                             const unsigned char* __restrict__ tile_needed = nullptr,
-                                                            const int* __restrict__ ctx_of_row = nullptr) {
+                                                            const int* __restrict__ ctx_of_row = nullptr,
+                                                            const float* __restrict__ pbias = nullptr,
+                                                            const float* __restrict__ pbias_isw = nullptr) {
   extern __shared__ __attribute__((aligned(16))) float S[];
   const int ntile = (MULTI ? NC_arg : 1) * NT;
   int b, tile;
@@ -317,7 +319,8 @@
     tile = bid % ntile;
   }
   if (tile_needed != nullptr && !tile_needed[b * ntile + tile]) return;
-  ipa_attn_tile<NT, MULTI, PLANES, TAPE>(S, b, tile, bid, proj, e, R, t, Wb, gamma, feat, NC_arg, stamps, esc, tape_p, tape_d2, ctx_of_row);
+  ipa_attn_tile<NT, MULTI, PLANES, TAPE, HOISTED>(S, b, tile, bid, proj, e, R, t, Wb, gamma, feat, NC_arg, stamps, esc, tape_p, tape_d2,
+                                                  ctx_of_row, pbias, pbias_isw);
 }
 
 static unsigned long long* g_attn_stamps = nullptr;
@@ -438,6 +441,100 @@
   *reinterpret_cast<f16x8*>(base) = h1;
   *reinterpret_cast<f16x8*>(base + 1024) = h2;
 }
+constexpr int kMaxHoistLayers = 16;
+struct PairHoistLayers { const float* wb[kMaxHoistLayers]; };
+__global__ __launch_bounds__(256) void pair_hoist_kernel(const float* __restrict__ e, const float* __restrict__ rs, _Float16* __restrict__ planes,
+                                                         float* __restrict__ hdr, float* __restrict__ bias, const PairHoistLayers L, int NL,
+                                                         int64_t layer_stride) {
+  constexpr int K = 128, TLD = 72;
+  __shared__ __attribute__((aligned(16))) _Float16 tr[4][2][32][TLD];
+  const int64_t row = blockIdx.x;
+  const int lane = threadIdx.x & 63, T = threadIdx.x >> 6, l15 = lane & 15, q = lane >> 4;
+  const float s = rs[2 * row];
+  const float* er = e + (row * K + 32 * T) * AC;
+  f16x8 a1[2][2], a2[2][2];
+#pragma unroll
+  for (int tl = 0; tl < 2; ++tl)
+#pragma unroll
+    for (int ks = 0; ks < 2; ++ks) {
+      const float* p = er + (16 * tl + l15) * AC + 32 * ks + 8 * q;
+      const f32x4 v0 = *reinterpret_cast<const f32x4*>(p), v1 = *reinterpret_cast<const f32x4*>(p + 4);
+      f16x8 h1, h2;
+#pragma unroll
+      for (int c = 0; c < 8; ++c) {
+        const float x = (c < 4 ? v0[c & 3] : v1[c & 3]) * s;
+        const _Float16 a = static_cast<_Float16>(x);
+        h1[c] = a;
+        h2[c] = static_cast<_Float16>(x - static_cast<float>(a));
+      }
+      a1[tl][ks] = h1;
+      a2[tl][ks] = h2;
+      *reinterpret_cast<f16x8*>(&tr[T][0][16 * tl + l15][32 * ks + 8 * q]) = h1;
+      *reinterpret_cast<f16x8*>(&tr[T][1][16 * tl + l15][32 * ks + 8 * q]) = h2;
+    }
+  __syncthreads();
+  _Float16* out = planes + (row * K + 32 * T) * (2 * AC);
+#pragma unroll
+  for (int pl = 0; pl < 2; ++pl)
+#pragma unroll
+    for (int ct = 0; ct < 4; ++ct) {
+      f16x8 f;
+#pragma unroll
+      for (int tt = 0; tt < 8; ++tt) f[tt] = tr[T][pl][16 * (tt >> 2) + 4 * q + (tt & 3)][16 * ct + l15];
+      *reinterpret_cast<f16x8*>(out + ((pl * 4 + ct) * 64 + lane) * 8) = f;
+    }
+  float* brow = bias + row * (K * AH) + T * 256 + (q * 16 + l15) * 4;
+#pragma unroll 1
+  for (int l = 0; l < NL; ++l) {
+    const float* Wb = L.wb[l];
+    f32x4 wv4[2][2];
+#pragma unroll
+    for (int ks = 0; ks < 2; ++ks)
+#pragma unroll
+      for (int hf = 0; hf < 2; ++hf) wv4[ks][hf] = *reinterpret_cast<const f32x4*>(Wb + (lane & 7) * AC + 32 * ks + 8 * q + 4 * hf);
+    f16x8 wp[2][2];
+    float isw;
+    attn_bias_weight_planes(wv4, l15, wp, isw);
+    if (row == 0 && threadIdx.x == 0) hdr[l] = isw;
+#pragma unroll
+    for (int tl = 0; tl < 2; ++tl) {
+      const f32x4 acc0 = attn_bias_product(a1[tl][0], a2[tl][0], wp[0][0], wp[1][0]);
+      const f32x4 acc1 = attn_bias_product(a1[tl][1], a2[tl][1], wp[0][1], wp[1][1]);
+      f32x4 sum;
+#pragma unroll
+      for (int r = 0; r < 4; ++r) sum[r] = acc0[r] + acc1[r];
+      if (l15 < 8) *reinterpret_cast<f32x4*>(brow + l * layer_stride + 32 * tl) = sum;
+    }
+  }
+}
+bool pair_hoist_supported(const diffab_dims* d) { return fast_path_supported(d) && d->K == 128 && d->NL >= 1 && d->NL <= kMaxHoistLayers; }
+static size_t pair_bias_layer_floats(const diffab_dims* d, int n_pair) {
+  return (n_pair > 0 ? static_cast<size_t>(n_pair) : static_cast<size_t>(d->B)) * d->K * d->K * AH;
+}
+size_t pair_bias_floats(const diffab_dims* d, int n_pair) {
+  return pair_hoist_supported(d) ? 64 + d->NL * pair_bias_layer_floats(d, n_pair) : 0;
+}
+const float* pair_bias_layer(const diffab_dims* d, const float* bias, int l, int n_pair) { return bias + 64 + l * pair_bias_layer_floats(d, n_pair); }
+int launch_pair_hoist(const diffab_dims* d, const float* e, const diffab_ipa_layer_weights* layers, float* planes, float* bias, hipStream_t st,
+                      int n_pair) {
+  DIFFAB_REQUIRE(pair_hoist_supported(d) && e && layers && planes && bias && (reinterpret_cast<uintptr_t>(planes) & 15) == 0 &&
+                     (reinterpret_cast<uintptr_t>(e) & 15) == 0 && (reinterpret_cast<uintptr_t>(bias) & 15) == 0,
+                 DIFFAB_ERR_ARG, "pair_hoist: unsupported operands");
+  PairHoistLayers L{};
+  for (int l = 0; l < d->NL; ++l) {
+    DIFFAB_REQUIRE(layers[l].w_bias && (reinterpret_cast<uintptr_t>(layers[l].w_bias) & 15) == 0, DIFFAB_ERR_ARG,
+                   "pair_hoist: layer %d needs a 16-byte aligned to_pair_bias weight", l);
+    L.wb[l] = layers[l].w_bias;
+  }
+  const int64_t np = static_cast<int64_t>(n_pair > 0 ? n_pair : d->B);
+  float* rs = const_cast<float*>(pair_row_scales(d, planes, n_pair));
+  hipLaunchKernelGGL(pair_rowscale_kernel, dim3(static_cast<unsigned>(np * d->K)), dim3(256), 0, st, e, d->K * AC / 4, rs);
+  hipLaunchKernelGGL(pair_hoist_kernel, dim3(static_cast<unsigned>(np * d->K)), dim3(256), 0, st, e, rs, reinterpret_cast<_Float16*>(planes + 64),
+                     bias, bias + 64, L, d->NL, static_cast<int64_t>(pair_bias_layer_floats(d, n_pair)));
+  DIFFAB_LAUNCH_CHECK();
+  return DIFFAB_OK;
+}
+
 bool pair_planes_supported(const diffab_dims* d) { return fast_path_supported(d); }
 static size_t pair_patches(const diffab_dims* d, int n_pair) { return static_cast<size_t>(n_pair > 0 ? n_pair : d->B); }
 size_t pair_planes_floats(const diffab_dims* d, int n_pair) {
@@ -501,7 +598,8 @@
 
 int ipa_layer_fast(const diffab_dims* d, const diffab_ipa_layer_weights* w, const float* x, const float* e, const float* R, const float* t,
                    float* y, float* ws, hipStream_t st, float* sp_keep, float* d2_keep, const void* planes, const float* pair_planes,
-                   bool fp32_gemm, bool taped, const unsigned char* tile_needed, const int* ctx_of_row, int n_ctx) {
+                   bool fp32_gemm, bool taped, const unsigned char* tile_needed, const int* ctx_of_row, int n_ctx, const float* pair_bias,
+                   const float* pair_bias_isw) {
   const int rows = d->B * d->K, D = d->D;
   DIFFAB_REQUIRE(ctx_of_row == nullptr || sp_keep == nullptr, DIFFAB_ERR_ARG, "ipa_layer_fast: shared contexts are an inference form");
   float* proj = ws;
@@ -559,6 +657,14 @@
                                          hipFuncAttributeMaxDynamicSharedMemorySize, static_cast<int>(lds)));
     hipLaunchKernelGGL((ipa_attn_fast_kernel<8, false, false, true>), grid, dim3(512), lds, st, proj, e, R, t, w->w_bias, w->gamma, feat,
                        d->B, nc, nullptr, nullptr, sp_keep, d2_keep);
+  } else if (use_planes && pair_bias != nullptr) {
+    DIFFAB_REQUIRE(nt == 8 && nc == 1 && pair_bias_isw != nullptr, DIFFAB_ERR_ARG, "ipa_layer_fast: the hoisted pair bias is a K = 128 form");
+    DIFFAB_HIP_CHECK(hipFuncSetAttribute(reinterpret_cast<const void*>(ipa_attn_fast_kernel<8, false, true, false, true>),
+                                         hipFuncAttributeMaxDynamicSharedMemorySize, static_cast<int>(lds)));
+    timer_begin(st);
+    hipLaunchKernelGGL((ipa_attn_fast_kernel<8, false, true, false, true>), grid, dim3(512), lds, st, proj, e_arg, R, t, w->w_bias, w->gamma, feat,
+                       d->B, nc, g_attn_stamps, esc, nullptr, nullptr, tile_needed, ctx_of_row, pair_bias, pair_bias_isw);
+    timer_end(st);
   } else if (use_planes) {
     if (nt == 8 && nc == 1) ATTN_LAUNCH(8, false, true);
     else if (nt == 8) ATTN_LAUNCH(8, true, true);
diff --git a/diffab-pytorch_amd/csrc/denoiser_internal.h b/diffab-pytorch_amd/csrc/denoiser_internal.h
--- a/diffab-pytorch_amd/csrc/denoiser_internal.h
+++ b/diffab-pytorch_amd/csrc/denoiser_internal.h
@@ -31,11 +31,17 @@
                    bool fp32_gemm = false,
                    bool taped = false,
                    const unsigned char* tile_needed = nullptr,
-                   const int* ctx_of_row = nullptr, int n_ctx = 0);
+                   const int* ctx_of_row = nullptr, int n_ctx = 0,
+                   const float* pair_bias = nullptr, const float* pair_bias_isw = nullptr);
 bool pair_planes_supported(const diffab_dims* d);
 size_t pair_planes_floats(const diffab_dims* d, int n_pair = 0);
 int launch_pair_split(const diffab_dims* d, const float* e, float* planes, hipStream_t st, int n_pair = 0);
 const float* pair_row_scales(const diffab_dims* d, const float* planes, int n_pair = 0);
+bool pair_hoist_supported(const diffab_dims* d);
+size_t pair_bias_floats(const diffab_dims* d, int n_pair = 0);
+const float* pair_bias_layer(const diffab_dims* d, const float* bias, int l, int n_pair = 0);
+int launch_pair_hoist(const diffab_dims* d, const float* e, const diffab_ipa_layer_weights* layers, float* planes, float* bias, hipStream_t st,
+                      int n_pair = 0);
 int launch_linear(const float* X, int ldx, const float* W, const float* bias, float* Y, int ldy, int M, int N, int Kd, bool relu,
                   hipStream_t st);
 
@@ -88,7 +94,8 @@
 int launch_ipa_module_persistent(const diffab_dims* d, float* xa, float* xb, const float* R, const float* t, float* ws, const void* planes,
                                  const float* pair_planes, hipStream_t st, const float* emb_X = nullptr, const MlpChainSet* emb = nullptr,
                                  const MlpChainSet* heads = nullptr, const int* ctx_of_row = nullptr, int n_ctx = 0,
-                                 const unsigned char* last_layer_tiles = nullptr);
+                                 const unsigned char* last_layer_tiles = nullptr,
+                                 const float* pair_bias = nullptr);
 void set_module_stagger(int ticks, int classes);
 void set_module_stamps(void* device_buffer);
 int launch_fold_embed_table(const diffab_dims* d, const diffab_denoiser_weights* w, float* emb_tab, hipStream_t st);
diff --git a/diffab-pytorch_amd/csrc/ipa_attn_tile.h b/diffab-pytorch_amd/csrc/ipa_attn_tile.h
--- a/diffab-pytorch_amd/csrc/ipa_attn_tile.h
+++ b/diffab-pytorch_amd/csrc/ipa_attn_tile.h
@@ -63,16 +63,49 @@
 }
 
 template <bool PLANES, typename FP>
-__device__ __forceinline__ void attn_shift_pair_rows(FP& e, FP& esc, const int* __restrict__ ctx_of_row, const int b, const int K) {
+__device__ __forceinline__ void attn_shift_pair_rows(FP& e, FP& esc, const int* __restrict__ ctx_of_row, const int b, const int K,
+                                                     FP* pbias = nullptr) {
   if (ctx_of_row == nullptr) return;
   int c;
   asm volatile("s_load_dword %0, %1, 0x0\n\ts_waitcnt lgkmcnt(0)" : "=s"(c) : "s"(ctx_of_row + b) : "memory");
   const int64_t shift = static_cast<int64_t>(c - b) * K;
   e += shift * K * AC;
   if constexpr (PLANES) esc += 2 * shift;
-}
-
-template <int NT, bool MULTI, bool PLANES = false, bool TAPE = false>
+  if (pbias != nullptr) *pbias += shift * K * AH;
+}
+
+__device__ __forceinline__ void attn_bias_weight_planes(const f32x4 (&wv4)[2][2], const int l15, f16x8 (&wp)[2][2], float& isw_out) {
+  float wmax = 0.f;
+#pragma unroll
+  for (int ks = 0; ks < 2; ++ks)
+#pragma unroll
+    for (int hf = 0; hf < 2; ++hf)
+#pragma unroll
+      for (int s = 0; s < 4; ++s) wmax = fmaxf(wmax, fabsf(wv4[ks][hf][s]));
+#pragma unroll
+  for (int o = 1; o < 64; o <<= 1) wmax = fmaxf(wmax, __shfl_xor(wmax, o));
+  const int ew = static_cast<int>((__float_as_uint(wmax) >> 23) & 255u);
+  const float sw = (ew == 0 || ew > 230) ? 1.0f : __uint_as_float(static_cast<unsigned>(127 + 7 + 127 - ew) << 23);
+  isw_out = (ew == 0 || ew > 230) ? 1.0f : __uint_as_float(static_cast<unsigned>(ew - 7) << 23);
+#pragma unroll
+  for (int ks = 0; ks < 2; ++ks)
+#pragma unroll
+    for (int c8 = 0; c8 < 8; ++c8) {
+      const float x = l15 < 8 ? wv4[ks][c8 >> 2][c8 & 3] * sw : 0.0f;
+      const _Float16 h1 = static_cast<_Float16>(x);
+      wp[0][ks][c8] = h1;
+      wp[1][ks][c8] = static_cast<_Float16>(x - static_cast<float>(h1));
+    }
+}
+__device__ __forceinline__ f32x4 attn_bias_product(const f16x8 a1, const f16x8 a2, const f16x8 wp0, const f16x8 wp1) {
+  f32x4 a_ = {0.f, 0.f, 0.f, 0.f};
+  a_ = __builtin_amdgcn_mfma_f32_16x16x32_f16(a2, wp0, a_, 0, 0, 0);
+  a_ = __builtin_amdgcn_mfma_f32_16x16x32_f16(a1, wp1, a_, 0, 0, 0);
+  a_ = __builtin_amdgcn_mfma_f32_16x16x32_f16(a1, wp0, a_, 0, 0, 0);
+  return a_;
+}
+
+template <int NT, bool MULTI, bool PLANES = false, bool TAPE = false, bool HOISTED = false>
 __device__ __forceinline__ void ipa_attn_tile(float* __restrict__ S, const int b, const int tile, const unsigned stamp_id,
                                               const float* __restrict__ proj, const float* __restrict__ e,
                                               const float* __restrict__ R, const float* __restrict__ t,
@@ -80,8 +113,10 @@
                                               float* __restrict__ feat, int NC_arg,
                                               unsigned long long* __restrict__ stamps, const float* __restrict__ esc = nullptr,
                                               float* __restrict__ tape_p = nullptr, float* __restrict__ tape_d2 = nullptr,
-                                              const int* __restrict__ ctx_of_row = nullptr) {
+                                              const int* __restrict__ ctx_of_row = nullptr, const float* __restrict__ pbias = nullptr,
+                                              const float* __restrict__ pbias_isw = nullptr) {
   static_assert(!PLANES || NT % 2 == 0, "the o_e product takes key tiles in pairs");
+  static_assert(!HOISTED || (PLANES && !MULTI), "the hoisted-bias form is the single-chunk planes kernel");
   static_assert(!TAPE || (!MULTI && !PLANES), "the tape form is the single-chunk fp32-pair kernel");
   const int NC = MULTI ? NC_arg : 1;
   constexpr int KC = NT * 16;
@@ -103,7 +138,8 @@
   const int tid = threadIdx.x, lane0 = tid & 63, wv = __builtin_amdgcn_readfirstlane(tid >> 6);
   constexpr int HS = KC + 8, IS = AH * (KC + 8) + 8;
   const int64_t prow0 = static_cast<int64_t>(b) * K;
-  attn_shift_pair_rows<PLANES>(e, esc, ctx_of_row, b, K);
+  if constexpr (HOISTED) attn_shift_pair_rows<PLANES>(e, esc, ctx_of_row, b, K, &pbias);
+  else attn_shift_pair_rows<PLANES>(e, esc, ctx_of_row, b, K);
   const float scale_t = 0.57735026918962576f;
 
   constexpr int KLD = 40, GLD = 28;
@@ -144,6 +180,13 @@
 #pragma unroll
     for (int ii = 0; ii < 2; ++ii) inv_s2[ii] = ep[2 * ii + 1];
   }
+  const float* brow[2] = {nullptr, nullptr};
+  float hoist_isw = 1.0f;
+  if constexpr (HOISTED) {
+#pragma unroll
+    for (int ii = 0; ii < 2; ++ii) brow[ii] = pbias + (prow0 + i0 + 2 * wv + ii) * (K * AH);
+    hoist_isw = pbias_isw[0];
+  }
 
 #pragma unroll 1
   for (int c = 0; c < NC; ++c) {
@@ -154,6 +197,10 @@
     const int l15 = lane & 15, q = lane >> 4;
     f32x4 ev[2][NT][4];
     f32x4 wv4[2][2];
+    f32x4 bq[2][NT / 2];
+    auto load_bias = [&](int ii, int T) {
+      if constexpr (HOISTED) bq[ii][T] = __builtin_nontemporal_load(reinterpret_cast<const f32x4*>(brow[ii]) + T * 64 + lane);
+    };
     auto load_e_tile = [&](int ii, int cc_, int jt) {
       if constexpr (PLANES) {
         const f32x4* ep = reinterpret_cast<const f32x4*>(erow[ii]) + (cc_ * NT + jt) * 256 + lane;
@@ -218,7 +265,9 @@
         if (jt + SD < NT) {
           load_keys(jt % SD, jt + SD);
         } else if (jt + E_EARLY >= NT) {
-          if constexpr (PLANES) {
+          if constexpr (HOISTED) {
+            if (jt + E_EARLY == NT) load_bias(0, 0);
+          } else if constexpr (PLANES) {
             if (jt + E_EARLY == NT) {
               const int hh = lane & 7, qq = lane >> 4;
 #pragma unroll
@@ -276,28 +325,18 @@
       f32x4 wb[4];
       f16x8 wp[2][2];
       float bscale = scale_t, oscale = 1.0f;
-      if constexpr (PLANES) {
-        float wmax = 0.f;
-#pragma unroll
-        for (int ks = 0; ks < 2; ++ks)
-#pragma unroll
-          for (int hf = 0; hf < 2; ++hf)
-#pragma unroll
-            for (int s = 0; s < 4; ++s) wmax = fmaxf(wmax, fabsf(wv4[ks][hf][s]));
-#pragma unroll
-        for (int o = 1; o < 64; o <<= 1) wmax = fmaxf(wmax, __shfl_xor(wmax, o));
-        const int ew = static_cast<int>((__float_as_uint(wmax) >> 23) & 255u);
-        const float sw = (ew == 0 || ew > 230) ? 1.0f : __uint_as_float(static_cast<unsigned>(127 + 7 + 127 - ew) << 23);
-        const float isw = (ew == 0 || ew > 230) ? 1.0f : __uint_as_float(static_cast<unsigned>(ew - 7) << 23);
-#pragma unroll
-        for (int ks = 0; ks < 2; ++ks)
-#pragma unroll
-          for (int c8 = 0; c8 < 8; ++c8) {
-            const float x = l15 < 8 ? wv4[ks][c8 >> 2][c8 & 3] * sw : 0.0f;
-            const _Float16 h1 = static_cast<_Float16>(x);
-            wp[0][ks][c8] = h1;
-            wp[1][ks][c8] = static_cast<_Float16>(x - static_cast<float>(h1));
-          }
+      if constexpr (HOISTED) {
+        (void)wv4;
+        bscale = scale_t * hoist_isw;
+        oscale = 1.0f / 256.0f;
+#pragma unroll
+        for (int jt = E_EARLY; jt < E_DEPTH0; ++jt) {
+          if (jt % 2 == 0) load_bias(0, jt / 2);
+          load_e_tile(0, c, jt);
+        }
+      } else if constexpr (PLANES) {
+        float isw;
+        attn_bias_weight_planes(wv4, l15, wp, isw);
         bscale = scale_t * isw;
         oscale = 1.0f / 256.0f;
         asm volatile("" ::"v"(wp[0][0]), "v"(wp[1][0]), "v"(wp[0][1]), "v"(wp[1][1]));
@@ -338,24 +377,29 @@
 #pragma unroll
           for (int T = 0; T < NT / 2; ++T) {
             f32x4 acc[2][2];
-#pragma unroll
-            for (int tl = 0; tl < 2; ++tl)
-#pragma unroll
-              for (int ks = 0; ks < 2; ++ks) {
-                const f16x8 a1 = __builtin_bit_cast(f16x8, ev[ii][2 * T + tl][ks]), a2 = __builtin_bit_cast(f16x8, ev[ii][2 * T + tl][2 + ks]);
-                f32x4 a_ = {0.f, 0.f, 0.f, 0.f};
-                a_ = __builtin_amdgcn_mfma_f32_16x16x32_f16(a2, wp[0][ks], a_, 0, 0, 0);
-                a_ = __builtin_amdgcn_mfma_f32_16x16x32_f16(a1, wp[1][ks], a_, 0, 0, 0);
-                a_ = __builtin_amdgcn_mfma_f32_16x16x32_f16(a1, wp[0][ks], a_, 0, 0, 0);
-                acc[tl][ks] = a_;
-              }
+            f32x4 bsum[2];
+            if constexpr (HOISTED) {
+              bsum[0] = bq[ii][T];
+#pragma unroll
+              for (int r = 0; r < 4; ++r)
+                bsum[1][r] = __int_as_float(__builtin_amdgcn_update_dpp(0, __float_as_int(bsum[0][r]), 0x128 , 0xf, 0xf, false));
+            } else {
+#pragma unroll
+              for (int tl = 0; tl < 2; ++tl)
+#pragma unroll
+                for (int ks = 0; ks < 2; ++ks) {
+                  const f16x8 a1 = __builtin_bit_cast(f16x8, ev[ii][2 * T + tl][ks]), a2 = __builtin_bit_cast(f16x8, ev[ii][2 * T + tl][2 + ks]);
+                  acc[tl][ks] = attn_bias_product(a1, a2, wp[0][ks], wp[1][ks]);
+                }
+            }
             float v[8], smax = -INFINITY;
 #pragma unroll
             for (int tl = 0; tl < 2; ++tl) {
               const f32x4 sv = *reinterpret_cast<const f32x4*>(Srow + (2 * T + tl) * 16 + 4 * q);
 #pragma unroll
               for (int r = 0; r < 4; ++r) {
-                v[4 * tl + r] = sv[r] + bscale_r * (acc[tl][0][r] + acc[tl][1][r]);
+                if constexpr (HOISTED) v[4 * tl + r] = __builtin_fmaf(bscale_r, bsum[tl][r], sv[r]);
+                else v[4 * tl + r] = sv[r] + bscale_r * (acc[tl][0][r] + acc[tl][1][r]);
                 smax = fmaxf(smax, v[4 * tl + r]);
               }
             }
@@ -389,17 +433,20 @@
 #pragma unroll
             for (int tl = 0; tl < 2; ++tl) {
               if (l15 < 8) *reinterpret_cast<f32x4*>(Srow + (2 * T + tl) * 16 + 4 * q) = f32x4{v[4 * tl], v[4 * tl + 1], v[4 * tl + 2], v[4 * tl + 3]};
-#pragma unroll
-              for (int pl = 0; pl < 2; ++pl)
-#pragma unroll
-                for (int ks = 0; ks < 2; ++ks)
-                  *reinterpret_cast<f32x4*>(trt + (tl * 2 + pl) * 2048 + (wr_off ^ (64 * ks))) = ev[ii][2 * T + tl][2 * pl + ks];
+              if constexpr (!HOISTED) {
+#pragma unroll
+                for (int pl = 0; pl < 2; ++pl)
+#pragma unroll
+                  for (int ks = 0; ks < 2; ++ks)
+                    *reinterpret_cast<f32x4*>(trt + (tl * 2 + pl) * 2048 + (wr_off ^ (64 * ks))) = ev[ii][2 * T + tl][2 * pl + ks];
+              }
             }
             {
               constexpr int dummy_ = 0;
               (void)dummy_;
               const int nx = ii * NT + 2 * T + RT;
               if (nx < 2 * NT) {
+                load_bias(nx / NT, (nx % NT) / 2);
                 load_e_tile(nx / NT, c, nx % NT);
                 load_e_tile((nx + 1) / NT, c, (nx + 1) % NT);
                 MEM_FENCE();
@@ -410,11 +457,15 @@
             for (int pl = 0; pl < 2; ++pl)
 #pragma unroll
               for (int ct = 0; ct < 4; ++ct) {
-                const int ro = rd_off ^ (32 * ct);
-                const s16x4_t lo = __builtin_amdgcn_ds_read_tr16_b64_v4i16((s16x4_t __attribute__((address_space(3)))*)(trt + (0 * 2 + pl) * 2048 + ro));
-                const s16x4_t hi = __builtin_amdgcn_ds_read_tr16_b64_v4i16((s16x4_t __attribute__((address_space(3)))*)(trt + (1 * 2 + pl) * 2048 + ro));
-                const s16x8_t v8 = {lo[0], lo[1], lo[2], lo[3], hi[0], hi[1], hi[2], hi[3]};
-                a[pl][ct] = __builtin_bit_cast(f16x8, v8);
+                if constexpr (HOISTED) {
+                  a[pl][ct] = __builtin_bit_cast(f16x8, ev[ii][2 * T + pl][ct]);
+                } else {
+                  const int ro = rd_off ^ (32 * ct);
+                  const s16x4_t lo = __builtin_amdgcn_ds_read_tr16_b64_v4i16((s16x4_t __attribute__((address_space(3)))*)(trt + (0 * 2 + pl) * 2048 + ro));
+                  const s16x4_t hi = __builtin_amdgcn_ds_read_tr16_b64_v4i16((s16x4_t __attribute__((address_space(3)))*)(trt + (1 * 2 + pl) * 2048 + ro));
+                  const s16x8_t v8 = {lo[0], lo[1], lo[2], lo[3], hi[0], hi[1], hi[2], hi[3]};
+                  a[pl][ct] = __builtin_bit_cast(f16x8, v8);
+                }
               }
 #pragma unroll
             for (int ct = 0; ct < 4; ++ct) oe[ct] = __builtin_amdgcn_mfma_f32_16x16x32_f16(a[1][ct], p1, oe[ct], 0, 0, 0);
diff --git a/diffab-pytorch_amd/csrc/ipa_persistent.hip b/diffab-pytorch_amd/csrc/ipa_persistent.hip
--- a/diffab-pytorch_amd/csrc/ipa_persistent.hip
+++ b/diffab-pytorch_amd/csrc/ipa_persistent.hip
@@ -24,6 +24,8 @@
   float* feat;
   const float* pair;
   const float* esc;
+  const float* pbias;
+  size_t pbias_stride;
   const int* ctx_of_row;
   const unsigned char* last_layer_tiles;
   const float* R;
@@ -44,11 +46,12 @@
   return ((w >> (8 * (idx & 3))) & 0xffu) != 0;
 }
 
-template <int KRES>
+template <int KRES, bool HOISTED = false>
 __global__ __launch_bounds__(512) void ipa_module_persistent_kernel(const ModuleArgs a) {
   extern __shared__ __attribute__((aligned(16))) float lds[];
   constexpr int K = KRES, NTILE = K / TI, DT = K / 128;
   static_assert(KRES == 128 || KRES == 256, "patch-resident module: K = 128 or 256");
+  static_assert(!HOISTED || KRES == 128, "the hoisted pair bias is a K = 128 form");
   const int M = a.B * K;
   if (a.stagger_ticks > 0 && a.stagger_classes > 1) {
     const unsigned long long t0 = __builtin_amdgcn_s_memrealtime();
@@ -115,8 +118,13 @@
 #pragma unroll 1
       for (int tile = 0; tile < NTILE; ++tile) {
         if (needed != nullptr && !module_tile_needed(needed, b * NTILE + tile)) continue;
-        ipa_attn_tile<8, (KRES > 128), true>(lds, b, tile, static_cast<unsigned>((b * a.NL + l) * NTILE + tile), a.proj, a.pair, a.R, a.t, small,
-                                             small + 512, a.feat, K / 128, a.stamps, a.esc, nullptr, nullptr, a.ctx_of_row);
+        if constexpr (HOISTED)
+          ipa_attn_tile<8, false, true, false, true>(lds, b, tile, static_cast<unsigned>((b * a.NL + l) * NTILE + tile), a.proj, a.pair, a.R, a.t,
+                                                     small, small + 512, a.feat, 1, a.stamps, a.esc, nullptr, nullptr, a.ctx_of_row,
+                                                     a.pbias + 64 + static_cast<size_t>(l) * a.pbias_stride, a.pbias + l);
+        else
+          ipa_attn_tile<8, (KRES > 128), true>(lds, b, tile, static_cast<unsigned>((b * a.NL + l) * NTILE + tile), a.proj, a.pair, a.R, a.t, small,
+                                               small + 512, a.feat, K / 128, a.stamps, a.esc, nullptr, nullptr, a.ctx_of_row);
         asm volatile("s_waitcnt vmcnt(0)" ::: "memory");
         __syncthreads();
       }
@@ -179,7 +187,8 @@
 
 int launch_ipa_module_persistent(const diffab_dims* d, float* xa, float* xb, const float* R, const float* t, float* ws, const void* planes,
                                  const float* pair_planes, hipStream_t st, const float* emb_X, const MlpChainSet* emb,
-                                 const MlpChainSet* heads, const int* ctx_of_row, int n_ctx, const unsigned char* last_layer_tiles) {
+                                 const MlpChainSet* heads, const int* ctx_of_row, int n_ctx, const unsigned char* last_layer_tiles,
+                                 const float* pair_bias) {
   DIFFAB_REQUIRE(ipa_module_persistent_supported(d) && xa && xb && R && t && ws && planes && pair_planes, DIFFAB_ERR_ARG,
                  "ipa_module_persistent: unsupported operands");
   DIFFAB_REQUIRE((reinterpret_cast<uintptr_t>(last_layer_tiles) & 3) == 0, DIFFAB_ERR_ARG,
@@ -192,6 +201,9 @@
   a.feat = ws + rows * ANP;
   a.pair = pair_planes + 64;
   a.esc = pair_row_scales(d, pair_planes, n_ctx);
+  DIFFAB_REQUIRE(pair_bias == nullptr || pair_hoist_supported(d), DIFFAB_ERR_ARG, "ipa_module_persistent: the hoisted pair bias is a K = 128 form");
+  a.pbias = pair_bias;
+  a.pbias_stride = pair_bias ? static_cast<size_t>(pair_bias_layer(d, pair_bias, 1, n_ctx) - pair_bias_layer(d, pair_bias, 0, n_ctx)) : 0;
   a.ctx_of_row = ctx_of_row;
   a.last_layer_tiles = last_layer_tiles;
   a.R = R;
@@ -217,15 +229,16 @@
   int dev = 0, ncu = 256;
   if (hipGetDevice(&dev) == hipSuccess) (void)hipDeviceGetAttribute(&ncu, hipDeviceAttributeMultiprocessorCount, dev);
   const int grid = d->B < ncu ? d->B : ncu;
-#define MODULE_LAUNCH(K_)                                                                                                       \
+#define MODULE_LAUNCH(...)                                                                                                      \
   do {                                                                                                                            \
-    DIFFAB_HIP_CHECK(hipFuncSetAttribute(reinterpret_cast<const void*>(ipa_module_persistent_kernel<K_>),                         \
+    DIFFAB_HIP_CHECK(hipFuncSetAttribute(reinterpret_cast<const void*>(ipa_module_persistent_kernel<__VA_ARGS__>),                \
                                          hipFuncAttributeMaxDynamicSharedMemorySize, static_cast<int>(kModuleLdsBytes)));        \
     timer_begin(st);                                                                                                              \
-    hipLaunchKernelGGL((ipa_module_persistent_kernel<K_>), dim3(grid), dim3(512), kModuleLdsBytes, st, a);                        \
+    hipLaunchKernelGGL((ipa_module_persistent_kernel<__VA_ARGS__>), dim3(grid), dim3(512), kModuleLdsBytes, st, a);               \
     timer_end(st);                                                                                                                \
   } while (0)
-  if (d->K == 128) MODULE_LAUNCH(128);
+  if (pair_bias != nullptr) MODULE_LAUNCH(128, true);
+  else if (d->K == 128) MODULE_LAUNCH(128);
   else MODULE_LAUNCH(256);
 #undef MODULE_LAUNCH
   DIFFAB_LAUNCH_CHECK();
diff --git a/diffab-pytorch_amd/diffab_pytorch/_hip.py b/diffab-pytorch_amd/diffab_pytorch/_hip.py
--- a/diffab-pytorch_amd/diffab_pytorch/_hip.py
+++ b/diffab-pytorch_amd/diffab_pytorch/_hip.py
@@ -18,6 +18,7 @@
 FLAG_MULTI_LAUNCH = 1024
 FLAG_SKIP_UNUSED_ROWS = 256
 FLAG_ALL_ROWS = 8192
+FLAG_INLINE_PAIR_BIAS = 16384
 FLAG_KEEP_STRUCTURE = 2048
 FLAG_KEEP_SEQUENCE = 4096
 
@@ -110,6 +111,8 @@
     "diffab_debug_set_module_stagger": (C.c_int, [_i32, _i32]),
     "diffab_debug_set_module_stamps": (C.c_int, [_fp]),
     "diffab_debug_row_tiles": (C.c_int, [_fp, _i32, _i32, _fp, _fp]),
+    "diffab_debug_pair_hoist_floats": (_sz, [_PD, _i32]),
+    "diffab_debug_pair_hoist": (C.c_int, [_PD, _fp, C.POINTER(DenoiserWeights), _fp, _fp, _fp, _fp]),
     "diffab_set_stream_guard": (C.c_int, [C.c_int]),
     "diffab_debug_linear128": (C.c_int, [_fp, _fp, _fp, _fp, C.c_int64, C.c_int32, C.c_int32, _fp, C.c_size_t, _fp]),
     "diffab_debug_gemm_tn": (C.c_int, [_fp, _fp, _fp, _fp, C.c_int64, C.c_int32, C.c_int32, C.c_int32, _fp]),
diff --git a/include/diffab_hip.h b/include/diffab_hip.h
--- a/include/diffab_hip.h
+++ b/include/diffab_hip.h
@@ -25,6 +25,7 @@
 #define DIFFAB_FLAG_PERSISTENT_MODULE 512u
 #define DIFFAB_FLAG_MULTI_LAUNCH 1024u
 #define DIFFAB_FLAG_ALL_ROWS 8192u
+#define DIFFAB_FLAG_INLINE_PAIR_BIAS 16384u
 #define DIFFAB_FLAG_SKIP_UNUSED_ROWS 256u
 #define DIFFAB_FLAG_KEEP_STRUCTURE 2048u
 #define DIFFAB_FLAG_KEEP_SEQUENCE 4096u
@@ -141,6 +142,10 @@
 
 size_t diffab_denoise_workspace_bytes(const diffab_dims* d);
 size_t diffab_sample_workspace_bytes(const diffab_dims* d);
+
+size_t diffab_debug_pair_hoist_floats(const diffab_dims* d, int32_t which);
+int diffab_debug_pair_hoist(const diffab_dims* d, const float* pair_ctx, const diffab_denoiser_weights* w, float* planes_inline,
+                            float* planes_hoisted, float* bias, void* stream);
 size_t diffab_sample_shared_workspace_bytes(const diffab_dims* d, int32_t n_ctx);
 int diffab_ipa_layer_fwd(const diffab_dims* d, const diffab_ipa_layer_weights* w, const float* x ,
                          const float* e , const float* R , const float* t ,
```

New measurement: 14.37 million. 0.977x the previous value.
